# rakhimovv/lvt

Hardware: AMD Instinct MI355X
Metric: video-clips/sec/node (VQVAE+DSFVT train step, BAIR 64x64x16) (higher is better)
Workload: dtype f32

## Files before the change

include/lvt_hip.h:

```cpp
#ifndef LVT_HIP_H
#define LVT_HIP_H
#include <stddef.h>
#include <stdint.h>
#ifdef __cplusplus
extern "C" {
#endif

#define LVT_OK            0
#define LVT_EINVAL      (-1)
#define LVT_EWORKSPACE  (-2)
#define LVT_ELAUNCH     (-3)
#define LVT_ENODEVICE   (-4)

const char *lvt_last_error(void);
int lvt_version(void);
int lvt_device_info(char *name, int name_len, int *cus, int *clock_khz, long long *hbm_bytes);

#define LVT_MATH_F32   (1 << 16)
#define LVT_MATH_F16X2 (1 << 18)
typedef struct { const float *a; const float *b; float *c; } lvt_amax_io;
int lvt_amax(const float *x, long long n, float *out, void *stream);
typedef struct { const float *x; long long n; float *out; } lvt_amax_entry;
int lvt_amax_multi(const lvt_amax_entry *entries, int n, void *stream);
int lvt_amax_merge(const float *a, const float *b, float *out, void *stream);
#define LVT_VQ_COARSE  (1 << 17)
#define LVT_VQ_GENERIC (1 << 22)

#define LVT_EPI_BIAS        1
#define LVT_EPI_RESIDUAL    2
#define LVT_EPI_RELU        4
#define LVT_EPI_TANH        8
#define LVT_EPI_MASK       16
#define LVT_EPI_ACCUM      32
#define LVT_EPI_PLANES     64
#define LVT_CAUSAL_KMAX   (1 << 8)
#define LVT_CAUSAL_KMIN   (1 << 9)
#define LVT_CAUSAL_TILE   (1 << 10)

typedef struct {
    int M, N, K;
    int ta, tb;
    const float *A; long long lda; int a_kb; long long a_skb;
    const float *B; long long ldb; int b_kb; long long b_skb;
    float *C;       long long ldc;
    int batch_outer, batch_inner;
    long long sA_o, sA_i, sB_o, sB_i, sC_o, sC_i;
    float alpha;
    int flags;
    const float *bias;
    const float *res;  long long ldr;
    const float *mask; long long ldm;
    int splits;
    float *a_colsum;
    long long c_plane;
    const float *a_amax, *b_amax;
    const float *a_amax2, *b_amax2;
    float *c_amax;
} lvt_gemm_desc;
size_t lvt_gemm_workspace_bytes(const lvt_gemm_desc *d);
int lvt_gemm_f32(const lvt_gemm_desc *d, void *workspace, size_t workspace_bytes, void *stream);

int lvt_vq_argmax_scores(const float *scores, long long rows, int K, long long ld, const float *codebook, int D,
                         long long *idx, void *stream);

typedef struct {
    int M, N, K;
    const void *A; long long lda; int a_planes; int a_kb; long long a_skb;
    const void *B; long long ldb;
    float *C; long long ldc;
    int batch_outer, batch_inner;
    long long sA_o, sA_i, sB_o, sB_i, sC_o, sC_i;
    float alpha;
    int flags;
    const float *bias;
    const float *res;  long long ldr;
    const float *mask; long long ldm;
    const float *a_amax, *b_amax;
    float *c_amax;
    void *Cp; long long ldcp; const float *cp_amax;
} lvt_gemm_p2_desc;
int lvt_gemm_p2_f32(const lvt_gemm_p2_desc *d, void *stream);
typedef struct { const float *src; void *dst; int rows, cols; long long ld_src, ld_dst; int transpose; const float *amax;
                 int batch; long long bs_src, bs_dst; } lvt_p2_pack_entry;
int lvt_p2_pack_multi(const lvt_p2_pack_entry *entries, int n, void *stream);

int lvt_gemm_smallm_f32(int M, int N, int K, int tb, const float *A, long long lda, const float *B,
                        long long ldb, float *C, long long ldc, int batch, long long sB, long long sC,
                        float alpha, int flags, const float *bias, const float *res, long long ldr,
                        const int *pos, long long c_pos, long long r_pos, void *stream);
size_t lvt_gemm_smallm_splitk_workspace_bytes(int M, int N, int splits);
int lvt_gemm_smallm_splitk_f32(int M, int N, int K, int splits, const float *A, long long lda, const float *B,
                               long long ldb, float *C, long long ldc, float alpha, int flags, const float *bias,
                               const float *res, long long ldr, const int *pos, long long c_pos, long long r_pos,
                               void *workspace, size_t workspace_bytes, void *stream);
int lvt_gemm_smallm_partial_f32(int M, int N, int K, int splits, const float *A, long long lda, const float *B,
                                long long ldb, void *workspace, size_t workspace_bytes, void *stream);
int lvt_splitsum_layernorm_fwd(const float *partials, int splits, int rows, int d, const float *bias, const float *res,
                               long long ldr, float *x_out, float eps, const float *w, const float *b, float *y,
                               void *stream);

typedef struct {
    int N, Ti, Hi, Wi, Ci;
    int To, Ho, Wo, Co;
    int Kt, Kh, Kw;
    int st, sh, sw;
    int pt, ph, pw;
} lvt_conv_geom;
int lvt_conv3d_pack_weight(const lvt_conv_geom *g, const float *w, int Ci_real, int Co_real,
                           float *wp, void *stream);
typedef struct { const float *w; float *dst; int kind, taps, Ci, Co, Ci_real, Co_real; } lvt_pack_entry;
int lvt_conv3d_pack_weights_multi(const lvt_pack_entry *entries, int n, void *stream);
#define LVT_CONV_WEIGHT_IMAGE (1 << 21)
typedef struct { const float *wp; int rows, cols; const float *amax; } lvt_weight_image_entry;
size_t lvt_conv3d_weight_image_bytes(int rows, int cols);
int lvt_conv3d_weight_images(const lvt_weight_image_entry *entries, int n, void *stream);
int lvt_conv3d_pack_weight_t(const lvt_conv_geom *g, const float *w, int Ci_real, int Co_real,
                             float *wt, void *stream);
// ... 21 lines not shown
#define LVT_WGRAD_DB_OF_X (1 << 20)
int lvt_conv3d_bwd_weight(const lvt_conv_geom *g, const float *x, const float *dy, float *dw, float *db,
                          int Ci_real, int Co_real, int flags, const lvt_amax_io *ax, void *workspace,
                          size_t workspace_bytes, void *stream);
int lvt_convt4_fwd(const float *x, const float *w, const float *bias, int N, int Hi, int Wi, int Ci, int Cr,
                   int act_tanh, float *y, int flags, const lvt_amax_io *ax, void *stream);
size_t lvt_colsum_workspace_bytes(long long M, int N);
int lvt_colsum(const float *g, long long M, int N, long long ld, float *out, void *workspace,
               size_t workspace_bytes, void *stream);

size_t lvt_vq_nearest_workspace_bytes(long long rows, int num, int KC);
size_t lvt_vq_nearest_generic_workspace_bytes(int num, int D, int KC);
int lvt_vq_nearest(const float *z, long long rows, int ldz, int num, int D, int KC,
                   const float *codebooks, long long *idx, int P, int flags, void *workspace, size_t workspace_bytes,
                   void *stream);
int lvt_vq_gather(const long long *idx, const float *codebooks, long long rows, int num, int D, int KC,
                  int P, float *out, int ldo, void *stream);
size_t lvt_vq_ema_workspace_bytes(long long rows, int num, int D, int KC);
int lvt_vq_ema_accumulate(const long long *idx, const float *z, long long rows, int ldz, int num, int D,
                          int KC, int P, float *stats, void *workspace, size_t workspace_bytes,
                          void *stream);
int lvt_vq_ema_finalize(const float *stats, int num, int D, int KC, float decay, float eps,
                        float *running_size, float *running_sum, float *weight, void *stream);

int lvt_to_channels_last(const float *in, int B, int C, long long R, int ldo, int mode, const float *a,
                         const float *s, float *out, float *out_amax, void *stream);
int lvt_to_channels_first(const float *in, int B, int C, long long R, int ldi, int mode, const float *a,
                          const float *s, float lo, float hi, float *out, void *stream);

size_t lvt_reduce_workspace_bytes(void);
int lvt_mse_fwd(const float *a, const float *b, long long n, double denom, float scale, float *out,
                void *workspace, size_t workspace_bytes, void *stream);
int lvt_mse_bwd(const float *a, const float *b, long long n, double denom, float scale,
                const float *gout_dev, const float *add, int tanh_of_a, float *out, float *out_amax, void *stream);
int lvt_l1_fwd(const float *a, const float *b, long long n, double denom, float scale, float *out,
               void *workspace, size_t workspace_bytes, void *stream);
int lvt_l1_bwd(const float *a, const float *b, long long n, double denom, float scale,
               const float *gout_dev, const float *add, int tanh_of_a, float *out, float *out_amax, void *stream);
int lvt_tanh_bwd(const float *g, const float *y, long long n, float *out, float *out_amax, void *stream);
int lvt_axpy(const float *x, const float *add, long long n, const float *alpha_dev, float alpha,
             float *out, void *stream);
int lvt_add_periodic(float *x, const float *table, long long rows, int P, int d, void *stream);

int lvt_layernorm_fwd(const float *x, long long rows, int d, float eps, const float *w, const float *b,
                      float *y, float *mean, float *rstd, float *y_amax, const float *w_amax, const float *b_amax,
                      void *stream);
int lvt_layernorm_fwd_p2(const float *x, long long rows, int d, float eps, const float *w, const float *b,
                         float *y, void *yp, float *mean, float *rstd, float *y_amax, const float *w_amax,
                         const float *b_amax, void *stream);
size_t lvt_layernorm_bwd_workspace_bytes(int d);
int lvt_layernorm_bwd(const float *dy, const float *x, const float *mean, const float *rstd,
                      const float *w, long long rows, int d, const float *add, float *dx, float *dw,
                      float *db, float *dx_amax, void *workspace, size_t workspace_bytes, void *stream);

int lvt_attn_softmax_fwd(float *scores, int B, int H, int S, float temper, const float *dt,
                         const float *dh, const float *dw, int bt, int bh, int bw, int masked, float fill,
                         void *stream);
int lvt_attn_softmax_bwd(const float *P, float *dP, int B, int H, int S, float temper, int bt, int bh,
                         int bw, float *G, float *ddt, float *ddh, float *ddw, void *stream);

int lvt_attn_fwd(const float *q, const float *k, const float *v, int B, int H, int S, int da, float temper,
                 const float *dt, const float *dh, const float *dw, int bt, int bh, int bw, int masked, float fill,
                 float *P, float *o, void *stream);

int lvt_attn_planes_supported(int S, int da, int bt, int bh, int bw);
int lvt_attn_fwd_planes(const void *qkv_planes, long long plane_stride, long long operand_stride, int B, int H, int S, int da,
                        float temper, const float *dt, const float *dh, const float *dw, int bt, int bh, int bw, int masked,
                        float fill, float *P, float *o, float *o_amax, void *stream);
size_t lvt_attn_bwd_planes_workspace_bytes(int B, int H, int S, int bt, int bh, int bw);
int lvt_attn_bwd_planes(const void *qkv_planes, long long plane_stride, long long operand_stride, const void *do_planes,
                        const float *P, const float *o, int B, int H, int S, int da, float temper, int bt, int bh, int bw,
                        int masked, float *dq, float *dk, float *dv, float *ddt, float *ddh, float *ddw, float *d_amax,
                        void *workspace, size_t workspace_bytes, void *stream);

int lvt_attn_flash_supported(int S, int da, int bt, int bh, int bw);
int lvt_attn_fwd_flash(const float *q, const float *k, const float *v, long long ld, int B, int H, int S, int da,
                       float temper, const float *dt, const float *dh, const float *dw, int bt, int bh, int bw,
                       int masked, float fill, float *o, float *stats, float *o_amax, void *stream);
size_t lvt_attn_bwd_flash_workspace_bytes(int B, int H, int S, int bt, int bh, int bw);
int lvt_attn_bwd_flash(const float *q, const float *k, const float *v, const float *d_o, long long ld, const float *stats,
                       const float *o, int B, int H, int S, int da, float temper, const float *dt, const float *dh, const float *dw,
                       int bt, int bh, int bw, int masked, float fill, float *dq, float *dk, float *dv, float *ddt,
                       float *ddh, float *ddw, float *d_amax, void *workspace, size_t workspace_bytes, void *stream);

int lvt_attn_decode(const float *q, long long ldq, const float *Kc, const float *Vc, int B, int H, int S, int da, int qi,
                    float temper, const float *dt, const float *dh, const float *dw, int bt, int bh, int bw,
                    float *o, const int *pos, long long q_pos, void *stream);

int lvt_decode_gather_codes(const long long *codes, const long long *nb, const int *pos, int rows, int S1, int taps,
                            long long *out, void *stream);
int lvt_decode_commit(const long long *drawn, int rows, int S1, long long *codes, int *pos, void *stream);

int lvt_sample_categorical(const float *logits, long long rows, int V, float temp, const float *u,
                           long long *out, long long out_stride, float *probs, const int *pos, long long u_pos,
                           void *stream);

int lvt_embbag_fwd(const long long *idx, long long bstride, int P, long long rows, int nslots,
                   const int *slot_off, const int *tab_row, const float *table, int D, const float *bias,
                   const float *btable, const long long *bindex, float *out, void *stream);
#define LVT_ONEHOT_DENSE (1 << 19)
size_t lvt_onehot_tn_workspace_bytes(int nslots, int V, int N, long long rows);
int lvt_onehot_tn_is_gather(int nslots, int V, int N, long long ldb, const float *dout, int flags);
int lvt_onehot_tn_gemm(const long long *idx, int nslots, int V, const int *slot_off, long long bstride,
                       long long pstride, int P, long long rows, const float *dout, long long ldb, int N,
                       float *out, int flags, const float *dout_amax, void *workspace, size_t workspace_bytes,
                       void *stream);
int lvt_permute3(const float *in, long long s0, long long s1, long long s2, int n0, int n1, int n2,
                 float *out, void *stream);

int lvt_row_gather(const float *x, const long long *perm, long long B, int S, int d, float *out, void *stream);

int lvt_slice_context(const long long *video, int B, int T, int nc, int H, int W, const int *abc, int st, int sh,
                      int sw, int kt, int kh, int kw, int n_prime, long long pad_value, long long *ctx,
                      long long *slice, long long *slice_idx, unsigned char *ignore, void *stream);

size_t lvt_xent_workspace_bytes(void);
int lvt_xent_fwd(const float *logits, const long long *target, long long tstride_b, long long tstride_pos,
                 int P, long long rows, int V, long long ignore, float scale, float *row_loss, float *lse,
                 float *loss, float *count, void *workspace, size_t workspace_bytes, void *stream);
int lvt_xent_bwd(const float *logits, const long long *target, long long tstride_b, long long tstride_pos,
                 int P, long long rows, int V, long long ignore, const float *lse, const float *count,
                 const float *gout, float scale, float *dlogits, float *dl_amax, void *stream);

typedef struct {
    float *p; const float *g; float *s0; float *s1;
    long long n; float lr; float wd;
} lvt_opt_entry;
int lvt_adam_step(const lvt_opt_entry *entries, int n, float beta1, float beta2, float eps, int step,
                  void *stream);
int lvt_rmsprop_step(const lvt_opt_entry *entries, int n, float alpha, float eps, float momentum,
                     void *stream);

#ifdef __cplusplus
}
#endif
#endif
```

lvt_amd/csrc/attention_flash.hip:

```cpp
#include "attn_common.h"

namespace {

template <int I> struct IC { static constexpr int value = I; };
template <int N, int I = 0, class F> __device__ __forceinline__ void static_for(F &&f) {
    if constexpr (I < N) { f(IC<I>{}); static_for<N, I + 1>(f); }
}

typedef _Float16 f16x8 __attribute__((ext_vector_type(8)));
typedef _Float16 f16x2v __attribute__((ext_vector_type(2)));
typedef float f32x2 __attribute__((ext_vector_type(2)));
typedef float f32x4v __attribute__((ext_vector_type(4)));
typedef short s16x4 __attribute__((ext_vector_type(4)));
typedef __attribute__((address_space(3))) s16x4 lds_s16x4;
typedef unsigned u32x4 __attribute__((ext_vector_type(4)));

#define FA_LD 144
#define FA_PL (64 * FA_LD)
#define FA_SLOT (2 * FA_PL)
#define FA_EMIN 30
#define FA_EMAX 254
#define FA_LOG2E 1.4426950408889634f

typedef unsigned u32x2 __attribute__((ext_vector_type(2)));

__device__ __forceinline__ float fa_u2f(unsigned u) { return __uint_as_float(u); }
__device__ __forceinline__ float fa_exp_field(int e) { return e <= 0 ? 0.f : fa_u2f((unsigned)e << 23); }
__device__ __forceinline__ int fa_clamp_e(int e) { return e < FA_EMIN ? FA_EMIN : (e > FA_EMAX ? FA_EMAX : e); }
__device__ __forceinline__ int fa_ebits(float nonneg) { return fa_clamp_e((int)((__float_as_uint(nonneg) >> 23) & 0xffu)); }
template <int CTRL> __device__ __forceinline__ float fa_dpp_max(float v) {
    const int o = __builtin_amdgcn_update_dpp(0, __builtin_bit_cast(int, v), CTRL, 0xf, 0xf, false);
    return fmaxf(v, __builtin_bit_cast(float, o));
}
__device__ __forceinline__ float fa_row16_max(float v) {
    v = fa_dpp_max<0xB1>(v);
    v = fa_dpp_max<0x4E>(v);
    v = fa_dpp_max<0x141>(v);
    v = fa_dpp_max<0x140>(v);
    return v;
}
__device__ __forceinline__ float fa_kg_max(float v) {
    u32x2 r = __builtin_amdgcn_permlane16_swap(__float_as_uint(v), __float_as_uint(v), false, false);
    v = fmaxf(fa_u2f(r[0]), fa_u2f(r[1]));
    r = __builtin_amdgcn_permlane32_swap(__float_as_uint(v), __float_as_uint(v), false, false);
    return fmaxf(fa_u2f(r[0]), fa_u2f(r[1]));
}
__device__ __forceinline__ float fa_kg_sum(float v) {
    u32x2 r = __builtin_amdgcn_permlane16_swap(__float_as_uint(v), __float_as_uint(v), false, false);
    v = fa_u2f(r[0]) + fa_u2f(r[1]);
    r = __builtin_amdgcn_permlane32_swap(__float_as_uint(v), __float_as_uint(v), false, false);
    return fa_u2f(r[0]) + fa_u2f(r[1]);
}
__device__ __forceinline__ float fa_max4(const f32x4v a) { return fmaxf(fmaxf(a[0], a[1]), fmaxf(a[2], a[3])); }
__device__ __forceinline__ float fa_absmax4(const float4 a) { return fmaxf(fmaxf(fabsf(a.x), fabsf(a.y)), fmaxf(fabsf(a.z), fabsf(a.w))); }

__device__ __forceinline__ float fa_mix_lo(unsigned h, float c) {
    float r;
    asm("v_fma_mix_f32 %0, %1, %2, %3 op_sel:[0,0,0] op_sel_hi:[1,0,0]" : "=v"(r) : "v"(h), "v"(-1.f), "v"(c));
    return r;
}
__device__ __forceinline__ float fa_mix_hi(unsigned h, float c) {
    float r;
    asm("v_fma_mix_f32 %0, %1, %2, %3 op_sel:[1,0,0] op_sel_hi:[1,0,0]" : "=v"(r) : "v"(h), "v"(-1.f), "v"(c));
    return r;
}
__device__ __forceinline__ void fa_split_pair(float a, float b, float s, unsigned &ph, unsigned &pl) {
    const f32x2 t = f32x2{a, b} * s;
    ph = __builtin_bit_cast(unsigned, __builtin_convertvector(t, f16x2v));
    const f32x2 r = {fa_mix_lo(ph, t.x), fa_mix_hi(ph, t.y)};
    pl = __builtin_bit_cast(unsigned, __builtin_convertvector(r, f16x2v));
}
__device__ __forceinline__ void fa_split_pair1(float a, float b, unsigned &ph, unsigned &pl) {
    const f32x2 t = {a, b};
    ph = __builtin_bit_cast(unsigned, __builtin_convertvector(t, f16x2v));
    const f32x2 r = {fa_mix_lo(ph, a), fa_mix_hi(ph, b)};
    pl = __builtin_bit_cast(unsigned, __builtin_convertvector(r, f16x2v));
}
__device__ __forceinline__ void fa_split8(const float (&v)[8], f16x8 &h, f16x8 &l) {
    u32x4 uh, ul;
    unsigned a, b;
    fa_split_pair1(v[0], v[1], a, b); uh[0] = a; ul[0] = b;
    fa_split_pair1(v[2], v[3], a, b); uh[1] = a; ul[1] = b;
// ... 8 lines not shown
}

__device__ __forceinline__ int fa_row_scale(const float4 a, const float4 b) {
    return fa_ebits(fa_row16_max(fmaxf(fa_absmax4(a), fa_absmax4(b))));
}
__device__ __forceinline__ void fa_row_store(const float4 a, const float4 b, int eb, unsigned short *slot, float *rs_inv, int row, int c) {
    const float s = fa_u2f((unsigned)(268 - eb) << 23);
    uint2 h0, l0, h1, l1;
    fa_split_pair(a.x, a.y, s, h0.x, l0.x); fa_split_pair(a.z, a.w, s, h0.y, l0.y);
    fa_split_pair(b.x, b.y, s, h1.x, l1.x); fa_split_pair(b.z, b.w, s, h1.y, l1.y);
    unsigned short *d = slot + row * FA_LD + 4 * c;
    *reinterpret_cast<uint2 *>(d) = h0;
    *reinterpret_cast<uint2 *>(d + 64) = h1;
    *reinterpret_cast<uint2 *>(d + FA_PL) = l0;
    *reinterpret_cast<uint2 *>(d + FA_PL + 64) = l1;
    rs_inv[c == 0 ? row : 64 + c] = fa_u2f((unsigned)(eb - 14) << 23);
}
struct G4 { float4 v[4]; };
__device__ __forceinline__ void fa_load(G4 &g, const float *__restrict__ x, const float *__restrict__ y, long long ld, int tid) {
    const int r = tid >> 4, c = tid & 15;
    const float *px = x + (long long)r * ld + 4 * c, *py = y + (long long)r * ld + 4 * c;
    g.v[0] = *reinterpret_cast<const float4 *>(px);
    g.v[1] = *reinterpret_cast<const float4 *>(px + 64);
    g.v[2] = *reinterpret_cast<const float4 *>(py);
    g.v[3] = *reinterpret_cast<const float4 *>(py + 64);
}
__device__ __forceinline__ void fa_park(const G4 &g, unsigned short *slot, float *rs_inv, int tid) {
    const int r = tid >> 4, c = tid & 15;
#pragma unroll
    for (int half = 0; half < 2; ++half)
        fa_row_store(g.v[2 * half], g.v[2 * half + 1], fa_row_scale(g.v[2 * half], g.v[2 * half + 1]), slot, rs_inv, 32 * half + r, c);
}
struct G8 { float4 v[8]; };
__device__ __forceinline__ void fa_load8(G8 &g, const float *__restrict__ x, const float *__restrict__ y, long long ld, int tid) {
    const int r = tid >> 4, c = tid & 15;
    const float *px = x + (long long)r * ld + 4 * c, *py = y + (long long)r * ld + 4 * c;
    g.v[0] = *reinterpret_cast<const float4 *>(px);
    g.v[1] = *reinterpret_cast<const float4 *>(px + 64);
    g.v[2] = *reinterpret_cast<const float4 *>(px + 16 * ld);
    g.v[3] = *reinterpret_cast<const float4 *>(px + 16 * ld + 64);
    g.v[4] = *reinterpret_cast<const float4 *>(py);
    g.v[5] = *reinterpret_cast<const float4 *>(py + 64);
    g.v[6] = *reinterpret_cast<const float4 *>(py + 16 * ld);
    g.v[7] = *reinterpret_cast<const float4 *>(py + 16 * ld + 64);
}
__device__ __forceinline__ void fa_park8(const G8 &g, unsigned short *slot, float *rs_inv, int tid) {
    const int r = tid >> 4, c = tid & 15;
#pragma unroll
    for (int p = 0; p < 4; ++p)
        fa_row_store(g.v[2 * p], g.v[2 * p + 1], fa_row_scale(g.v[2 * p], g.v[2 * p + 1]), slot, rs_inv, 16 * p + r, c);
}
__device__ __forceinline__ void fa_bfrags_request(const float *__restrict__ row, int kg, float4 (&v)[8]) {
#pragma unroll
    for (int s = 0; s < 4; ++s) {
        v[2 * s] = *reinterpret_cast<const float4 *>(row + 32 * s + 8 * kg);
        v[2 * s + 1] = *reinterpret_cast<const float4 *>(row + 32 * s + 8 * kg + 4);
    }
}
__device__ __forceinline__ void fa_bfrags_split(const float4 (&v)[8], f16x8 (&fr)[4][2], float &inv) {
    float m = 0.f;
#pragma unroll
    for (int e = 0; e < 8; ++e) m = fmaxf(m, fa_absmax4(v[e]));
    m = fa_kg_max(m);
    const int eb = fa_ebits(m);
    const float sc = fa_u2f((unsigned)(268 - eb) << 23);
    inv = fa_u2f((unsigned)(eb - 14) << 23);
#pragma unroll
    for (int s = 0; s < 4; ++s) {
        u32x4 uh, ul;
        unsigned a, b;
        fa_split_pair(v[2 * s].x, v[2 * s].y, sc, a, b); uh[0] = a; ul[0] = b;
        fa_split_pair(v[2 * s].z, v[2 * s].w, sc, a, b); uh[1] = a; ul[1] = b;
        fa_split_pair(v[2 * s + 1].x, v[2 * s + 1].y, sc, a, b); uh[2] = a; ul[2] = b;
        fa_split_pair(v[2 * s + 1].z, v[2 * s + 1].w, sc, a, b); uh[3] = a; ul[3] = b;
        fr[s][0] = __builtin_bit_cast(f16x8, uh);
        fr[s][1] = __builtin_bit_cast(f16x8, ul);
    }
}
__device__ __forceinline__ void fa_load_bfrags(const float *__restrict__ row, int kg, f16x8 (&fr)[4][2], float &inv) {
    float4 v[8];
    fa_bfrags_request(row, kg, v);
    fa_bfrags_split(v, fr, inv);
}
__device__ __forceinline__ f16x8 fa_rowfrag(const unsigned short *slot, int pl, int row, int s, int kg) {
    return *reinterpret_cast<const f16x8 *>(slot + pl * FA_PL + row * FA_LD + 32 * s + 8 * kg);
}
__device__ __forceinline__ f16x8 fa_trfrag(const unsigned short *slot, int pl, int rb, int dtile, int c16, int kg) {
    const unsigned short *p = slot + pl * FA_PL + (rb + 4 * kg + (c16 >> 2)) * FA_LD + 16 * dtile + 4 * (c16 & 3);
    const s16x4 lo = __builtin_amdgcn_ds_read_tr16_b64_v4i16((lds_s16x4 *)(p));
    const s16x4 hi = __builtin_amdgcn_ds_read_tr16_b64_v4i16((lds_s16x4 *)(p + 16 * FA_LD));
    union { struct { s16x4 a, b; } s; f16x8 v; } u;
    u.s.a = lo; u.s.b = hi;
    return u.v;
}

struct FaSmem {
    unsigned short ring[2][FA_SLOT];
    float rs_inv[2][80];
    float dhs[32];
};
template <int NR> struct FaSmemA {
    unsigned short ring[2][FA_SLOT];
    float rs_inv[2][80];
    float dhs[32];
    float red[16];
    float R[128 * 4 * NR];
};
struct FaSmem3 {
    unsigned short ring[3][FA_SLOT];
    float rs_inv[3][80];
    float dhs[32];
};

__device__ __forceinline__ int fa_pair(unsigned x) { return (int)(((x >> 4) << 3) | (x & 7)); }
__device__ __forceinline__ int fa_half(unsigned x) { return (int)((x >> 3) & 1); }
__device__ __forceinline__ int fa_pair4(unsigned x) { return (int)(((x >> 5) << 3) | (x & 7)); }
__device__ __forceinline__ int fa_quarter(unsigned x) { return (int)((x >> 3) & 3); }
__device__ __forceinline__ int fa_opaque(int x) { asm volatile("" : "+s"(x)); return x; }

template <int BH, int BW> struct Geo16 {
    static_assert(BW == 16 || BW == 8, "16-wide tiles: BW is 8 or 16");
    static constexpr int HP = BW == 16 ? BH : BH / 2;
    static __device__ __forceinline__ int hj(int hslot, int kg) { return BW == 16 ? hslot : 2 * hslot + (kg >> 1); }
    static __device__ __forceinline__ int wj(int r, int kg) { return BW == 16 ? 4 * kg + r : 4 * (kg & 1) + r; }
};
template <int BT, int BH, int BW> struct BankIdx {
    static constexpr int NT = 2 * BT - 1, NH = 2 * BH - 1, NW = 2 * BW - 1, NB = NT + NH + NW;
};

struct FaArgs {
    const float *q, *k, *v, *d_o;
    long long ld;
    int H;
    float c1, fill2;
    float inv_temper;
    const float *dt, *dh, *dw;
    float *o, *m, *l;
    float *dq, *dk, *dv, *delta, *scal, *bank_partial;
};

template <int BT, int BH, int BW, int MASKED, int NCH>
__device__ __forceinline__ float fa_fwd_body(const FaArgs &A, FaSmem &sm, int bh_, int qhalf) {
    using GE = Geo16<BH, BW>;
    constexpr int HP = GE::HP;
    static_assert(BT * BH * BW == AT_S, "256 tokens");
    const int tid = threadIdx.x, lane = tid & 63, wave = tid >> 6;
    const int c16 = lane & 15, kg = lane >> 4;
    const int b = bh_ / A.H, h = bh_ % A.H;
    const long long row0 = (long long)b * AT_S;
    const int il = wave * 16 + c16, i = qhalf * 128 + il;
    const float *kbase = A.k + row0 * A.ld + h * AT_D, *vbase = A.v + row0 * A.ld + h * AT_D;
    constexpr int NIT = NCH;

    if (tid < 2 * BH - 1) sm.dhs[tid] = A.dh[h * (2 * BH - 1) + tid] * FA_LOG2E;
    G4 g0, g1;
#define FA_G(t) ((((t) & 1) == 0) ? g0 : g1)
    auto load_item = [&](int t, G4 &gg) { fa_load(gg, kbase + (long long)(32 * t) * A.ld, vbase + (long long)(32 * t) * A.ld, A.ld, tid); };
    load_item(0, g0);
    if (NIT > 1) load_item(1, g1);
    f16x8 qb[4][2];
    float qinv;
    fa_load_bfrags(A.q + (row0 + i) * A.ld + h * AT_D, kg, qb, qinv);
    const int wi = i % BW, hi = (i / BW) % BH, ti = i / (BW * BH);
    float bt_[BT], bw_[4];
#pragma unroll
    for (int x = 0; x < BT; ++x) bt_[x] = A.dt[h * (2 * BT - 1) + ti - x + BT - 1] * FA_LOG2E;
#pragma unroll
    for (int r = 0; r < 4; ++r) bw_[r] = A.dw[h * (2 * BW - 1) + wi - GE::wj(r, kg) + BW - 1] * FA_LOG2E;
    const float *dhl = sm.dhs + (hi + BH - 1 - (BW == 16 ? 0 : (kg >> 1)));
    constexpr int HSTEP = BW == 16 ? 1 : 2;
    const float qc = qinv * A.c1;
    fa_park(g0, sm.ring[0], sm.rs_inv[0], tid);
    __syncthreads();

    f32x4v oacc[AT_D / 16];
#pragma unroll
    for (int d = 0; d < AT_D / 16; ++d) oacc[d] = f32x4v{0.f, 0.f, 0.f, 0.f};
    float m_run = -3.0e38f, lsum = 0.f;
    float vmax_run = fa_u2f((unsigned)(FA_EMIN - 14) << 23);

    static_for<NIT>([&](auto tc) {
        constexpr int t = decltype(tc)::value;
        const unsigned short *cur = sm.ring[t & 1];
        const float *cinv = sm.rs_inv[t & 1];
        if constexpr (t + 2 < NIT) load_item(t + 2, FA_G(t));
        f32x4v st[2] = {f32x4v{0.f, 0.f, 0.f, 0.f}, f32x4v{0.f, 0.f, 0.f, 0.f}};
#pragma unroll
        for (int s = 0; s < 4; ++s) {
            f16x8 a[2][2];
#pragma unroll
            for (int kt = 0; kt < 2; ++kt)
#pragma unroll
                for (int pl = 0; pl < 2; ++pl) a[kt][pl] = fa_rowfrag(cur, pl, 16 * kt + c16, s, kg);
#pragma unroll
            for (int kt = 0; kt < 2; ++kt) st[kt] = fa_mfma(a[kt][1], qb[s][0], st[kt]);
#pragma unroll
            for (int kt = 0; kt < 2; ++kt) st[kt] = fa_mfma(a[kt][0], qb[s][1], st[kt]);
#pragma unroll
            for (int kt = 0; kt < 2; ++kt) st[kt] = fa_mfma(a[kt][0], qb[s][0], st[kt]);
        }
        if constexpr (t + 1 < NIT) fa_park(FA_G(t + 1), sm.ring[(t + 1) & 1], sm.rs_inv[(t + 1) & 1], tid);
        float x[8];
        f32x4v vinv[2];
#pragma unroll
        for (int kt = 0; kt < 2; ++kt) {
            const int T = 2 * t + kt;
            const f32x4v kinv = *reinterpret_cast<const f32x4v *>(cinv + 16 * kt + 4 * kg);
            vinv[kt] = *reinterpret_cast<const f32x4v *>(cinv + 32 + 16 * kt + 4 * kg);
            const float bth = bt_[T / HP] + dhl[-HSTEP * (T % HP)];
#pragma unroll
            for (int r = 0; r < 4; ++r) {
                float v = fa_score(st[kt][r], kinv[r] * qc, bth + bw_[r]);
                if (MASKED && 16 * T + 4 * kg + r > i) v = A.fill2;
                x[4 * kt + r] = v;
            }
        }
        float cmax = fmaxf(fmaxf(fmaxf(x[0], x[1]), fmaxf(x[2], x[3])), fmaxf(fmaxf(x[4], x[5]), fmaxf(x[6], x[7])));
        cmax = fa_kg_max(cmax);
        const float vmax_c = fa_kg_max(fmaxf(fa_max4(vinv[0]), fa_max4(vinv[1])));
        const float m_new = fmaxf(m_run, cmax);
        const float alpha = __builtin_amdgcn_exp2f(m_run - m_new);
        m_run = m_new;
        const float vmax_new = fmaxf(vmax_run, vmax_c);
        const float fo = alpha * (vmax_run * __builtin_amdgcn_rcpf(vmax_new));
        vmax_run = vmax_new;
        const float srun = 32768.f * __builtin_amdgcn_rcpf(vmax_new);
        float psum = 0.f, pw[8];
#pragma unroll
        for (int kt = 0; kt < 2; ++kt)
#pragma unroll
            for (int r = 0; r < 4; ++r) {
                const float p = __builtin_amdgcn_exp2f(x[4 * kt + r] - m_new);
                psum += p;
                pw[4 * kt + r] = p * (vinv[kt][r] * srun);
            }
        lsum = lsum * alpha + psum;
        f16x8 pbh, pbl;
        fa_split8(pw, pbh, pbl);
#pragma unroll
        for (int d = 0; d < AT_D / 16; ++d) oacc[d] *= fo;
#pragma unroll
        for (int dp = 0; dp < AT_D / 32; ++dp) {
            f16x8 a[2][2];
#pragma unroll
            for (int dd = 0; dd < 2; ++dd)
#pragma unroll
                for (int pl = 0; pl < 2; ++pl) a[dd][pl] = fa_trfrag(cur, pl, 32, 2 * dp + dd, c16, kg);
#pragma unroll
            for (int dd = 0; dd < 2; ++dd) oacc[2 * dp + dd] = fa_mfma(a[dd][1], pbh, oacc[2 * dp + dd]);
#pragma unroll
            for (int dd = 0; dd < 2; ++dd) oacc[2 * dp + dd] = fa_mfma(a[dd][0], pbl, oacc[2 * dp + dd]);
#pragma unroll
            for (int dd = 0; dd < 2; ++dd) oacc[2 * dp + dd] = fa_mfma(a[dd][0], pbh, oacc[2 * dp + dd]);
        }
        __syncthreads();
    });
#undef FA_G
    const float linv = 1.f / fa_kg_sum(lsum);
    const float osc = (vmax_run * (1.f / 32768.f)) * linv;
    float am = 0.f;
    {
        float *orow = A.o + (row0 + i) * A.ld + h * AT_D + 4 * kg;
#pragma unroll
        for (int d = 0; d < AT_D / 16; ++d) {
            const f32x4v ov = oacc[d] * osc;
            *reinterpret_cast<f32x4v *>(orow + 16 * d) = ov;
            am = fmaxf(am, fmaxf(fmaxf(fabsf(ov[0]), fabsf(ov[1])), fmaxf(fabsf(ov[2]), fabsf(ov[3]))));
        }
    }
    if (kg == 0) {
        const long long si = ((long long)b * A.H + h) * AT_S + i;
        A.m[si] = m_run;
        A.l[si] = linv;
    }
    return am;
}

template <int BT, int BH, int BW, int MASKED>
__global__ __launch_bounds__(512, 1) void lvt_attn_fwd_flash_kernel(const FaArgs A, float *__restrict__ o_amax) {
    __shared__ __attribute__((aligned(16))) FaSmem sm;
    if (threadIdx.x >= 256) __builtin_amdgcn_s_setprio(1);
    float am;
    if (MASKED) {
        am = fa_fwd_body<BT, BH, BW, MASKED, 8>(A, sm, blockIdx.x, 1);
        __syncthreads();
        am = fmaxf(am, fa_fwd_body<BT, BH, BW, MASKED, 4>(A, sm, fa_opaque(blockIdx.x), 0));
    } else {
        am = fa_fwd_body<BT, BH, BW, MASKED, 8>(A, sm, fa_pair(blockIdx.x), fa_half(blockIdx.x));
    }
    if (o_amax) {
        __syncthreads();
        lvt_block_amax_commit(am, o_amax, reinterpret_cast<float *>(sm.ring[0]));
    }
}

template <int BT, int BH, int BW, int MASKED, int NCH, int ONEP>
__device__ __forceinline__ float fa_bwd_a_body(const FaArgs &A, FaSmemA<BT + Geo16<BH, BW>::HP + 4> &sm, int bh_, int qhalf) {
    using GE = Geo16<BH, BW>;
    using BI = BankIdx<BT, BH, BW>;
    constexpr int HP = GE::HP;
    constexpr int NR = BT + HP + 4;
    static_assert(BT * BH * BW == AT_S, "256 tokens");
    const int tid = threadIdx.x, lane = tid & 63, wave = tid >> 6;
    const int c16 = lane & 15, kg = lane >> 4;
    const int b = bh_ / A.H, h = bh_ % A.H;
    const long long row0 = (long long)b * AT_S;
    const int il = wave * 16 + c16, i = qhalf * 128 + il;
    const float *kbase = A.k + row0 * A.ld + h * AT_D, *vbase = A.v + row0 * A.ld + h * AT_D;
    constexpr int NIT = ONEP ? NCH : 2 * NCH;

    if (tid < 2 * BH - 1) sm.dhs[tid] = A.dh[h * (2 * BH - 1) + tid] * FA_LOG2E;
    float *mine = sm.R + (il * 4 + kg) * NR;
#pragma unroll
    for (int x = 0; x < NR; ++x) mine[x] = 0.f;
    G4 g0;
    auto load_item = [&](int t, G4 &gg) {
        const int c = t < NCH ? t : t - NCH;
        fa_load(gg, kbase + (long long)(32 * c) * A.ld, vbase + (long long)(32 * c) * A.ld, A.ld, tid);
    };
    load_item(0, g0);
    f16x8 qb[4][2], dob[4][2];
    float qinv, doinv;
    float4 qraw[8], doraw[8], oraw[ONEP ? 8 : 1];
    fa_bfrags_request(A.q + (row0 + i) * A.ld + h * AT_D, kg, qraw);
    fa_bfrags_request(A.d_o + (row0 + i) * A.ld + h * AT_D, kg, doraw);
    if constexpr (ONEP) fa_bfrags_request(A.o + (row0 + i) * A.ld + h * AT_D, kg, oraw);
    fa_bfrags_split(qraw, qb, qinv);
    fa_bfrags_split(doraw, dob, doinv);
    float delta_early = 0.f;
    if constexpr (ONEP) {
        float a0 = 0.f, a1 = 0.f;
#pragma unroll
        for (int s_ = 0; s_ < 4; ++s_) {
            const float4 o0 = oraw[2 * s_], o1 = oraw[2 * s_ + 1], d0 = doraw[2 * s_], d1 = doraw[2 * s_ + 1];
            a0 = fmaf(o0.x, d0.x, a0); a0 = fmaf(o0.y, d0.y, a0); a0 = fmaf(o0.z, d0.z, a0); a0 = fmaf(o0.w, d0.w, a0);
            a1 = fmaf(o1.x, d1.x, a1); a1 = fmaf(o1.y, d1.y, a1); a1 = fmaf(o1.z, d1.z, a1); a1 = fmaf(o1.w, d1.w, a1);
        }
        delta_early = fa_kg_sum(a0 + a1);
    }
    const long long si = ((long long)b * A.H + h) * AT_S + i;
    const float m_i = A.m[si], linv = A.l[si];
    const int wi = i % BW, hi = (i / BW) % BH, ti = i / (BW * BH);
    float bt_[BT];
    f32x4v bw4;
#pragma unroll
    for (int x = 0; x < BT; ++x) bt_[x] = A.dt[h * (2 * BT - 1) + ti - x + BT - 1] * FA_LOG2E;
#pragma unroll
    for (int r = 0; r < 4; ++r) bw4[r] = A.dw[h * (2 * BW - 1) + wi - GE::wj(r, kg) + BW - 1] * FA_LOG2E;
    const float *dhl = sm.dhs + (hi + BH - 1 - (BW == 16 ? 0 : (kg >> 1)));
    constexpr int HSTEP = BW == 16 ? 1 : 2;
    const float qc = qinv * A.c1;
    fa_park(g0, sm.ring[0], sm.rs_inv[0], tid);
    load_item(1, g0);
    __syncthreads();

    float delta = 0.f, gmax = 0.f;
    float kmax = fa_u2f((unsigned)(FA_EMIN - 14) << 23);
    float sgf = 0.f, kmr = 0.f, dl = 0.f;
    int ebG = FA_EMIN;
    if constexpr (ONEP) { delta = delta_early; dl = delta * linv; }
    f32x4v qacc[AT_D / 16];
#pragma unroll
    for (int d = 0; d < AT_D / 16; ++d) qacc[d] = f32x4v{0.f, 0.f, 0.f, 0.f};
    constexpr bool CORR = ONEP;
    f32x4v cacc[CORR ? AT_D / 16 : 1];
#pragma unroll
    for (int d = 0; d < (CORR ? AT_D / 16 : 1); ++d) cacc[d] = f32x4v{0.f, 0.f, 0.f, 0.f};
    int ebC = 16;
    float rst[BT], rsw[4];
#pragma unroll
    for (int x = 0; x < BT; ++x) rst[x] = 0.f;
#pragma unroll
    for (int r = 0; r < 4; ++r) rsw[r] = 0.f;

    static_for<NIT>([&](auto tc) {
        constexpr int t = decltype(tc)::value;
        constexpr int c = t < NCH ? t : t - NCH;
        constexpr bool PASS2 = ONEP || t >= NCH;
        const unsigned short *cur = sm.ring[t & 1];
        const float *cinv = sm.rs_inv[t & 1];
        constexpr bool PARK = t + 1 < NIT;
        unsigned short *nslot = sm.ring[(t + 1) & 1];
        float *ninv = sm.rs_inv[(t + 1) & 1];
        if constexpr (!ONEP && t == NCH) {
            delta = fa_kg_sum(delta) * linv;
            gmax = fa_kg_max(gmax);
            kmax = fa_kg_max(kmax);
            const float G = gmax + fabsf(delta);
            ebG = fa_ebits(G);
            sgf = fa_u2f((unsigned)(268 - ebG) << 23);
            kmr = __builtin_amdgcn_rcpf(kmax);
            dl = delta * linv;
            float r0 = doinv, r1 = G * qinv;
#pragma unroll
            for (int dd = 32; dd > 0; dd >>= 1) { r0 = fmaxf(r0, __shfl_xor(r0, dd, 64)); r1 = fmaxf(r1, __shfl_xor(r1, dd, 64)); }
            if (lane == 0) { sm.red[wave] = r0; sm.red[8 + wave] = r1; }
        }
        f32x4v st[2] = {f32x4v{0.f, 0.f, 0.f, 0.f}, f32x4v{0.f, 0.f, 0.f, 0.f}};
        f32x4v dp[2] = {f32x4v{0.f, 0.f, 0.f, 0.f}, f32x4v{0.f, 0.f, 0.f, 0.f}};
        int eb0 = 0, eb1 = 0;
        static_for<4>([&](auto sc_) {
            constexpr int s = decltype(sc_)::value;
            f16x8 a[2][2], av[2][2];
#pragma unroll
            for (int kt = 0; kt < 2; ++kt)
#pragma unroll
                for (int pl = 0; pl < 2; ++pl) {
                    a[kt][pl] = fa_rowfrag(cur, pl, 16 * kt + c16, s, kg);
                    av[kt][pl] = fa_rowfrag(cur, pl, 32 + 16 * kt + c16, s, kg);
                }
#pragma unroll
            for (int kt = 0; kt < 2; ++kt) { st[kt] = fa_mfma(a[kt][1], qb[s][0], st[kt]); dp[kt] = fa_mfma(av[kt][1], dob[s][0], dp[kt]); }
#pragma unroll
            for (int kt = 0; kt < 2; ++kt) { st[kt] = fa_mfma(a[kt][0], qb[s][1], st[kt]); dp[kt] = fa_mfma(av[kt][0], dob[s][1], dp[kt]); }
#pragma unroll
            for (int kt = 0; kt < 2; ++kt) { st[kt] = fa_mfma(a[kt][0], qb[s][0], st[kt]); dp[kt] = fa_mfma(av[kt][0], dob[s][0], dp[kt]); }
            if constexpr (PARK) {
                if constexpr (s == 0) eb0 = fa_row_scale(g0.v[0], g0.v[1]);
                if constexpr (s == 1) fa_row_store(g0.v[0], g0.v[1], eb0, nslot, ninv, tid >> 4, tid & 15);
                if constexpr (s == 2) eb1 = fa_row_scale(g0.v[2], g0.v[3]);
                if constexpr (s == 3) fa_row_store(g0.v[2], g0.v[3], eb1, nslot, ninv, 32 + (tid >> 4), tid & 15);
                __builtin_amdgcn_sched_group_barrier(0x100, 8, 0);
#pragma unroll
                for (int e = 0; e < 12; ++e) {
                    __builtin_amdgcn_sched_group_barrier(0x008, 1, 0);
                    __builtin_amdgcn_sched_group_barrier(0x002, (s & 1) ? 3 : 2, 0);
                }
                __builtin_amdgcn_sched_barrier(0);
            }
        });
        if constexpr (t + 2 < NIT) load_item(t + 2, g0);
        float w[8];
        u32x4 pku = {0u, 0u, 0u, 0u};
        if constexpr (CORR) {
            const f32x4v k0 = *reinterpret_cast<const f32x4v *>(cinv + 4 * kg), k1 = *reinterpret_cast<const f32x4v *>(cinv + 16 + 4 * kg);
            const int ebN = max(ebC, (int)(__float_as_uint(fa_kg_max(fmaxf(fa_max4(k0), fa_max4(k1)))) >> 23));
            if (__builtin_amdgcn_ballot_w64(ebN != ebC) != 0) {
                const float f = fa_exp_field(127 + ebC - ebN);
#pragma unroll
                for (int d = 0; d < AT_D / 16; ++d) cacc[d] = cacc[d] * f;
                ebC = ebN;
            }
        }
        const float scc = CORR ? fa_u2f((unsigned)(268 - ebC) << 23) * linv : 0.f;
#pragma unroll
        for (int kt = 0; kt < 2; ++kt) {
            const int T = 2 * c + kt;
            const f32x4v kinv = *reinterpret_cast<const f32x4v *>(cinv + 16 * kt + 4 * kg);
            const f32x4v vinv = *reinterpret_cast<const f32x4v *>(cinv + 32 + 16 * kt + 4 * kg);
            const float bth = bt_[T / HP] + dhl[-HSTEP * (T % HP)];
            if constexpr (!PASS2) kmax = fmaxf(kmax, fa_max4(kinv));
            const f32x4v qk = kinv * qc, bm = bw4 + bth;
            const f32x4v dv = vinv * (PASS2 ? doinv * linv : doinv), kw = kinv * kmr;
            float gt = 0.f;
            const f32x4v ks = kinv * scc;
            f32x4v pkv = {0.f, 0.f, 0.f, 0.f};
#pragma unroll
            for (int r = 0; r < 4; ++r) {
                float x = fa_score(st[kt][r], qk[r], bm[r]);
                if (MASKED && 16 * T + 4 * kg + r > i) x = A.fill2;
                const float ex = __builtin_amdgcn_exp2f(x - m_i);
                if constexpr (!PASS2) {
                    const float dpv = dp[kt][r] * dv[r];
                    delta = fmaf(ex, dpv, delta);
                    gmax = fmaxf(gmax, fabsf(dpv));
                } else {
                    const float g = ex * fmaf(dp[kt][r], dv[r], -dl);
                    gt += g;
                    rsw[r] += g;
                    if constexpr (ONEP) { w[4 * kt + r] = g * kinv[r]; gmax = fmaxf(gmax, fabsf(g)); if constexpr (CORR) pkv[r] = ex * ks[r]; }
                    else w[4 * kt + r] = (g * sgf) * kw[r];
                }
            }
            if constexpr (PASS2) { rst[T / HP] += gt; mine[BT + T % HP] += gt; }
            if constexpr (CORR) {
                pku[2 * kt] = __builtin_bit_cast(unsigned, __builtin_convertvector(f32x2{pkv[0], pkv[1]}, f16x2v));
                pku[2 * kt + 1] = __builtin_bit_cast(unsigned, __builtin_convertvector(f32x2{pkv[2], pkv[3]}, f16x2v));
            }
        }
        if constexpr (PASS2) {
            if constexpr (ONEP) {
                float tm = 0.f;
#pragma unroll
                for (int e = 0; e < 8; ++e) tm = fmaxf(tm, fabsf(w[e]));
                const int ebN = max(ebG, fa_ebits(fa_kg_max(tm)));
                if (__builtin_amdgcn_ballot_w64(ebN != ebG) != 0) {
                    const float f = fa_exp_field(127 + ebG - ebN);
#pragma unroll
                    for (int d = 0; d < AT_D / 16; ++d) qacc[d] = qacc[d] * f;
                    ebG = ebN;
                }
                const float sct = fa_u2f((unsigned)(268 - ebG) << 23);
#pragma unroll
                for (int e = 0; e < 8; ++e) w[e] *= sct;
            }
            f16x8 wbh, wbl;
            fa_split8(w, wbh, wbl);
            const f16x8 pcb = __builtin_bit_cast(f16x8, pku);
#pragma unroll
            for (int dq_ = 0; dq_ < AT_D / 32; ++dq_) {
                f16x8 a[2][2];
#pragma unroll
                for (int dd = 0; dd < 2; ++dd)
#pragma unroll
                    for (int pl = 0; pl < 2; ++pl) a[dd][pl] = fa_trfrag(cur, pl, 0, 2 * dq_ + dd, c16, kg);
#pragma unroll
                for (int dd = 0; dd < 2; ++dd) qacc[2 * dq_ + dd] = fa_mfma(a[dd][1], wbh, qacc[2 * dq_ + dd]);
#pragma unroll
                for (int dd = 0; dd < 2; ++dd) qacc[2 * dq_ + dd] = fa_mfma(a[dd][0], wbl, qacc[2 * dq_ + dd]);
// ... 5 lines not shown
                }
            }
        }
        __syncthreads();
    });
    if constexpr (ONEP) {
        float r0 = doinv, r1 = fa_kg_max(gmax) * qinv;
#pragma unroll
        for (int dd = 32; dd > 0; dd >>= 1) { r0 = fmaxf(r0, __shfl_xor(r0, dd, 64)); r1 = fmaxf(r1, __shfl_xor(r1, dd, 64)); }
        if (lane == 0) { sm.red[wave] = r0; sm.red[8 + wave] = r1; }
        __syncthreads();
    }
    const float f1 = ONEP ? 1.f : kmax, f2 = fa_exp_field(ebG - 14) * A.inv_temper;
    float epsc = 0.f;
    if constexpr (CORR) {
        const float eps = fa_kg_sum((rsw[0] + rsw[1]) + (rsw[2] + rsw[3]));
        delta += eps;
        epsc = (eps * fa_exp_field(ebC - 14)) * A.inv_temper;
    }
    float am = 0.f;
    {
        float *qrow = A.dq + (row0 + i) * A.ld + h * AT_D + 4 * kg;
#pragma unroll
        for (int d = 0; d < AT_D / 16; ++d) {
            f32x4v ov = (qacc[d] * f1) * f2;
            if constexpr (CORR) ov = ov - cacc[d] * epsc;
            *reinterpret_cast<f32x4v *>(qrow + 16 * d) = ov;
            am = fmaxf(am, fmaxf(fmaxf(fabsf(ov[0]), fabsf(ov[1])), fmaxf(fabsf(ov[2]), fabsf(ov[3]))));
        }
    }
    if (kg == 0) A.delta[si] = delta;
    if (tid == 0) {
        float r0 = sm.red[0], r1 = sm.red[8];
#pragma unroll
        for (int x = 1; x < 8; ++x) { r0 = fmaxf(r0, sm.red[x]); r1 = fmaxf(r1, sm.red[8 + x]); }
        A.scal[(bh_ * 2 + qhalf) * 2] = r0;
        A.scal[(bh_ * 2 + qhalf) * 2 + 1] = r1;
    }
    float *R = sm.R;
    float *R2 = reinterpret_cast<float *>(sm.ring[0]);
#pragma unroll
    for (int x = 0; x < BT; ++x) mine[x] = rst[x];
#pragma unroll
    for (int r = 0; r < 4; ++r) mine[BT + HP + r] = rsw[r];
    __syncthreads();
    {
        const int e = tid & 63, part = tid >> 6;
        if (e < BI::NB) {
            float acc = 0.f;
            for (int q = 16 * part; q < 16 * part + 16; ++q) {
                const int iq = qhalf * 128 + q;
                const int wq = iq % BW, hq = (iq / BW) % BH, tq = iq / (BW * BH);
                const float *r = R + (q * 4) * NR;
                if (e < BI::NT) {
                    const int tj = tq - e + BT - 1;
                    if (tj >= 0 && tj < BT) acc += (r[tj] + r[NR + tj]) + (r[2 * NR + tj] + r[3 * NR + tj]);
                } else if (e < BI::NT + BI::NH) {
                    const int hj = hq - (e - BI::NT) + BH - 1;
                    if (hj >= 0 && hj < BH) {
                        if (BW == 16) acc += (r[BT + hj] + r[NR + BT + hj]) + (r[2 * NR + BT + hj] + r[3 * NR + BT + hj]);
                        else acc += r[(2 * (hj & 1)) * NR + BT + (hj >> 1)] + r[(2 * (hj & 1) + 1) * NR + BT + (hj >> 1)];
                    }
                } else {
                    const int wj = wq - (e - BI::NT - BI::NH) + BW - 1;
                    if (wj >= 0 && wj < BW) {
                        if (BW == 16) acc += r[(wj >> 2) * NR + BT + HP + (wj & 3)];
                        else acc += r[(wj >> 2) * NR + BT + HP + (wj & 3)] + r[((wj >> 2) + 2) * NR + BT + HP + (wj & 3)];
                    }
                }
            }
            R2[part * BI::NB + e] = acc;
        }
    }
    __syncthreads();
    if (tid < BI::NB) {
        float acc = 0.f;
#pragma unroll
        for (int part = 0; part < 8; ++part) acc += R2[part * BI::NB + tid];
        A.bank_partial[((long long)bh_ * 2 + qhalf) * BI::NB + tid] = acc;
    }
    return am;
}

template <int BT, int BH, int BW, int MASKED, int ONEP>
__global__ __launch_bounds__(512, 1) void lvt_attn_bwd_flash_a_kernel(const FaArgs A, float *__restrict__ d_amax) {
    __shared__ __attribute__((aligned(16))) FaSmemA<BT + Geo16<BH, BW>::HP + 4> sm;
    if (threadIdx.x >= 256) __builtin_amdgcn_s_setprio(1);
    float am;
    if (MASKED) {
        am = fa_bwd_a_body<BT, BH, BW, MASKED, 8, ONEP>(A, sm, blockIdx.x, 1);
        __syncthreads();
        am = fmaxf(am, fa_bwd_a_body<BT, BH, BW, MASKED, 4, ONEP>(A, sm, fa_opaque(blockIdx.x), 0));
    } else {
        am = fa_bwd_a_body<BT, BH, BW, MASKED, 8, ONEP>(A, sm, fa_pair(blockIdx.x), fa_half(blockIdx.x));
    }
    if (d_amax) {
        __syncthreads();
        lvt_block_amax_commit(am, d_amax, reinterpret_cast<float *>(sm.ring[0]));
    }
}

struct FaSmemB {
    unsigned short ring[2][FA_SLOT];
    unsigned short vres[2][FA_SLOT];
    float rs_inv[2][80];
    float vinv[2][80];
    float dhs[32];
};

template <int BT, int BH, int BW, int MASKED, int C0, int NCH>
__device__ __forceinline__ float fa_bwd_b_body(const FaArgs &A, FaSmemB &sm, int bh_, int khalf) {
    using GE = Geo16<BH, BW>;
    constexpr int HP = GE::HP;
    const int tid = threadIdx.x, lane = tid & 63, wave = tid >> 6;
    const int c16 = lane & 15, kg = lane >> 4;
    const int b = bh_ / A.H, h = bh_ % A.H;
    const long long row0 = (long long)b * AT_S;
    const int jl = wave * 16 + c16, j = khalf * 128 + jl;
    const float *qbase = A.q + row0 * A.ld + h * AT_D, *dobase = A.d_o + row0 * A.ld + h * AT_D;
    const long long sb = ((long long)b * A.H + h) * AT_S;
    constexpr int NIT = NCH;

    if (tid < 2 * BH - 1) sm.dhs[tid] = A.dh[h * (2 * BH - 1) + tid] * FA_LOG2E;
    G4 g0;
    auto load_item = [&](int t, G4 &gg) {
        fa_load(gg, qbase + (long long)(32 * (C0 + t)) * A.ld, dobase + (long long)(32 * (C0 + t)) * A.ld, A.ld, tid);
    };
    {
        const float *rows = A.v + (row0 + khalf * 128) * A.ld + h * AT_D;
        G4 a, bq;
        fa_load(a, rows, rows + 32 * A.ld, A.ld, tid);
        fa_load(bq, rows + 64 * A.ld, rows + 96 * A.ld, A.ld, tid);
        fa_park(a, sm.vres[0], sm.vinv[0], tid);
        fa_park(bq, sm.vres[1], sm.vinv[1], tid);
    }
    f16x8 kb[4][2];
    float kinv;
    load_item(0, g0);
    fa_load_bfrags(A.k + (row0 + j) * A.ld + h * AT_D, kg, kb, kinv);
    const float *sc = A.scal + (long long)bh_ * 4;
    const float domax = fmaxf(sc[0], sc[2]), umax = fmaxf(sc[1], sc[3]);
    const float srun = 32768.f * __builtin_amdgcn_rcpf(domax);
    const int zb = fa_ebits(umax);
    const float zrun = fa_u2f((unsigned)(268 - zb) << 23);
    const unsigned short *vs = sm.vres[jl >> 6];
    const int wj = j % BW, hj = (j / BW) % BH, tj = j / (BW * BH);
    float bt_[BT];
    f32x4v bw4;
#pragma unroll
    for (int x = 0; x < BT; ++x) bt_[x] = A.dt[h * (2 * BT - 1) + x - tj + BT - 1] * FA_LOG2E;
#pragma unroll
    for (int r = 0; r < 4; ++r) bw4[r] = A.dw[h * (2 * BW - 1) + GE::wj(r, kg) - wj + BW - 1] * FA_LOG2E;
    const float *dhl = sm.dhs + (BH - 1 - hj + (BW == 16 ? 0 : (kg >> 1)));
    constexpr int HSTEP = BW == 16 ? 1 : 2;
    const float kc = kinv * A.c1;
    fa_park(g0, sm.ring[0], sm.rs_inv[0], tid);
    if (NIT > 1) load_item(1, g0);
    __syncthreads();
    const float vinv = sm.vinv[jl >> 6][jl & 63];

    f32x4v accv[AT_D / 16], acck[AT_D / 16];
#pragma unroll
    for (int d = 0; d < AT_D / 16; ++d) { accv[d] = f32x4v{0.f, 0.f, 0.f, 0.f}; acck[d] = f32x4v{0.f, 0.f, 0.f, 0.f}; }

    static_for<NIT>([&](auto tc) {
        constexpr int t = decltype(tc)::value;
        constexpr int c = C0 + t;
        constexpr bool PARK = t + 1 < NIT;
        const unsigned short *cur = sm.ring[t & 1];
        const float *cinv = sm.rs_inv[t & 1];
        unsigned short *nslot = sm.ring[(t + 1) & 1];
        float *ninv = sm.rs_inv[(t + 1) & 1];
        f32x4v m4[2], l4[2], d4[2];
#pragma unroll
        for (int qt = 0; qt < 2; ++qt) {
            const long long o = sb + 32 * c + 16 * qt + 4 * kg;
            m4[qt] = *reinterpret_cast<const f32x4v *>(A.m + o);
            l4[qt] = *reinterpret_cast<const f32x4v *>(A.l + o);
            d4[qt] = *reinterpret_cast<const f32x4v *>(A.delta + o);
        }
        f32x4v st[2] = {f32x4v{0.f, 0.f, 0.f, 0.f}, f32x4v{0.f, 0.f, 0.f, 0.f}};
        f32x4v dp[2] = {f32x4v{0.f, 0.f, 0.f, 0.f}, f32x4v{0.f, 0.f, 0.f, 0.f}};
        int eb0 = 0, eb1 = 0;
        f16x8 aq[2][2][2], ad[2][2], vb[2];
        auto load_s = [&](int s_, int bf) {
#pragma unroll
            for (int qt = 0; qt < 2; ++qt)
#pragma unroll
                for (int pl = 0; pl < 2; ++pl) aq[bf][qt][pl] = fa_rowfrag(cur, pl, 16 * qt + c16, s_, kg);
        };
        auto load_p = [&](int s_) {
#pragma unroll
            for (int pl = 0; pl < 2; ++pl) vb[pl] = fa_rowfrag(vs, pl, jl & 63, s_, kg);
#pragma unroll
            for (int qt = 0; qt < 2; ++qt)
#pragma unroll
                for (int pl = 0; pl < 2; ++pl) ad[qt][pl] = fa_rowfrag(cur, pl, 32 + 16 * qt + c16, s_, kg);
        };
        load_s(0, 0);
        static_for<4>([&](auto sc_) {
            constexpr int s = decltype(sc_)::value, bf = s & 1;
            load_p(s);
#pragma unroll
            for (int qt = 0; qt < 2; ++qt) st[qt] = fa_mfma(aq[bf][qt][1], kb[s][0], st[qt]);
#pragma unroll
            for (int qt = 0; qt < 2; ++qt) st[qt] = fa_mfma(aq[bf][qt][0], kb[s][1], st[qt]);
#pragma unroll
            for (int qt = 0; qt < 2; ++qt) st[qt] = fa_mfma(aq[bf][qt][0], kb[s][0], st[qt]);
            if constexpr (s < 3) load_s(s + 1, bf ^ 1);
#pragma unroll
            for (int qt = 0; qt < 2; ++qt) dp[qt] = fa_mfma(ad[qt][1], vb[0], dp[qt]);
#pragma unroll
            for (int qt = 0; qt < 2; ++qt) dp[qt] = fa_mfma(ad[qt][0], vb[1], dp[qt]);
#pragma unroll
            for (int qt = 0; qt < 2; ++qt) dp[qt] = fa_mfma(ad[qt][0], vb[0], dp[qt]);
            if constexpr (PARK) {
                if constexpr (s == 0) eb0 = fa_row_scale(g0.v[0], g0.v[1]);
                if constexpr (s == 1) fa_row_store(g0.v[0], g0.v[1], eb0, nslot, ninv, tid >> 4, tid & 15);
                if constexpr (s == 2) eb1 = fa_row_scale(g0.v[2], g0.v[3]);
                if constexpr (s == 3) fa_row_store(g0.v[2], g0.v[3], eb1, nslot, ninv, 32 + (tid >> 4), tid & 15);
            }
            __builtin_amdgcn_sched_group_barrier(0x100, 6, 0);
#pragma unroll
            for (int e = 0; e < 6; ++e) {
                __builtin_amdgcn_sched_group_barrier(0x008, 1, 0);
                if (PARK) __builtin_amdgcn_sched_group_barrier(0x002, (s & 1) ? 3 : 2, 0);
            }
            if constexpr (s < 3) __builtin_amdgcn_sched_group_barrier(0x100, 4, 0);
#pragma unroll
            for (int e = 0; e < 6; ++e) {
                __builtin_amdgcn_sched_group_barrier(0x008, 1, 0);
                if (PARK) __builtin_amdgcn_sched_group_barrier(0x002, (s & 1) ? 3 : 2, 0);
            }
            __builtin_amdgcn_sched_barrier(0);
        });
        if constexpr (t + 2 < NIT) load_item(t + 2, g0);
        float pw[8], u[8];
#pragma unroll
        for (int qt = 0; qt < 2; ++qt) {
            const int T = 2 * c + qt;
            const f32x4v qinv = *reinterpret_cast<const f32x4v *>(cinv + 16 * qt + 4 * kg);
            const f32x4v doinv = *reinterpret_cast<const f32x4v *>(cinv + 32 + 16 * qt + 4 * kg);
            const float bth = bt_[T / HP] + dhl[HSTEP * (T % HP)];
            const f32x4v qk = qinv * kc, bm = bw4 + bth;
            const f32x4v lds = l4[qt] * (doinv * srun);
            const f32x4v qzl = l4[qt] * qinv;
            const f32x4v dvq = (doinv * vinv) * qzl, dq_ = d4[qt] * qzl;
#pragma unroll
            for (int r = 0; r < 4; ++r) {
                float x = fa_score(st[qt][r], qk[r], bm[r]);
                if (MASKED && j > 16 * T + 4 * kg + r) x = A.fill2;
                const float ex = __builtin_amdgcn_exp2f(x - m4[qt][r]);
                pw[4 * qt + r] = ex * lds[r];
                u[4 * qt + r] = (ex * fmaf(dp[qt][r], dvq[r], -dq_[r])) * zrun;
            }
        }
        f16x8 pbh, pbl, ubh, ubl;
        fa_split8(pw, pbh, pbl);
        fa_split8(u, ubh, ubl);
        f16x8 ao[2][2], aqt[2];
        auto load_o = [&](int d_, int bf) {
#pragma unroll
            for (int pl = 0; pl < 2; ++pl) ao[bf][pl] = fa_trfrag(cur, pl, 32, d_, c16, kg);
        };
        load_o(0, 0);
        static_for<AT_D / 16>([&](auto dc) {
            constexpr int d = decltype(dc)::value, bf = d & 1;
#pragma unroll
            for (int pl = 0; pl < 2; ++pl) aqt[pl] = fa_trfrag(cur, pl, 0, d, c16, kg);
            accv[d] = fa_mfma(ao[bf][1], pbh, accv[d]);
            accv[d] = fa_mfma(ao[bf][0], pbl, accv[d]);
            accv[d] = fa_mfma(ao[bf][0], pbh, accv[d]);
            if constexpr (d + 1 < AT_D / 16) load_o(d + 1, bf ^ 1);
            acck[d] = fa_mfma(aqt[1], ubh, acck[d]);
            acck[d] = fa_mfma(aqt[0], ubl, acck[d]);
            acck[d] = fa_mfma(aqt[0], ubh, acck[d]);
            __builtin_amdgcn_sched_group_barrier(0x100, 4, 0);
            __builtin_amdgcn_sched_group_barrier(0x008, 3, 0);
            if constexpr (d + 1 < AT_D / 16) __builtin_amdgcn_sched_group_barrier(0x100, 4, 0);
            __builtin_amdgcn_sched_group_barrier(0x008, 3, 0);
            __builtin_amdgcn_sched_barrier(0);
        });
        __syncthreads();
    });
    const float fvs = domax * (1.f / 32768.f), fks = fa_exp_field(zb - 14) * A.inv_temper;
    float am = 0.f;
    {
        float *vrow = A.dv + (row0 + j) * A.ld + h * AT_D + 4 * kg, *krow = A.dk + (row0 + j) * A.ld + h * AT_D + 4 * kg;
#pragma unroll
        for (int d = 0; d < AT_D / 16; ++d) {
            const f32x4v ov = accv[d] * fvs, ok = acck[d] * fks;
            *reinterpret_cast<f32x4v *>(vrow + 16 * d) = ov;
            *reinterpret_cast<f32x4v *>(krow + 16 * d) = ok;
#pragma unroll
            for (int e = 0; e < 4; ++e) am = fmaxf(am, fmaxf(fabsf(ov[e]), fabsf(ok[e])));
        }
    }
    return am;
}

template <int BT, int BH, int BW, int MASKED>
__global__ __launch_bounds__(512, 1) void lvt_attn_bwd_flash_b_kernel(const FaArgs A, float *__restrict__ d_amax) {
    __shared__ __attribute__((aligned(16))) FaSmemB sm;
    if (threadIdx.x >= 256) __builtin_amdgcn_s_setprio(1);
    float am;
    if (MASKED) {
        if (fa_half(blockIdx.x) == 0) am = fa_bwd_b_body<BT, BH, BW, MASKED, 0, 8>(A, sm, fa_pair(blockIdx.x), 0);
        else am = fa_bwd_b_body<BT, BH, BW, MASKED, 4, 4>(A, sm, fa_pair(blockIdx.x), 1);
    } else {
        am = fa_bwd_b_body<BT, BH, BW, MASKED, 0, 8>(A, sm, fa_pair(blockIdx.x), fa_half(blockIdx.x));
    }
    if (d_amax) {
        __syncthreads();
        lvt_block_amax_commit(am, d_amax, reinterpret_cast<float *>(sm.ring[0]));
    }
}

__global__ __launch_bounds__(256) void lvt_attn_flash_bank_reduce_kernel(const float *__restrict__ partial, int B, int H, int NB, int nt,
                                                                         int nh, float *__restrict__ ddt, float *__restrict__ ddh,
                                                                         float *__restrict__ ddw) {
    const int idx = blockIdx.x * 4 + (threadIdx.x >> 6), lane = threadIdx.x & 63;
    if (idx >= H * NB) return;
    const int h = idx / NB, e = idx % NB;
    float s = 0.f;
    for (int jj = lane; jj < 2 * B; jj += 64) s += partial[(((long long)(jj >> 1) * H + h) * 2 + (jj & 1)) * NB + e];
#pragma unroll
    for (int m = 32; m >= 1; m >>= 1) s += __shfl_xor(s, m, 64);
    if (lane) return;
    const int nw = NB - nt - nh;
    if (e < nt) ddt[h * nt + e] = nt == 1 ? 0.f : s;
    else if (e < nt + nh) ddh[h * nh + e - nt] = nh == 1 ? 0.f : s;
    else ddw[h * nw + e - nt - nh] = nw == 1 ? 0.f : s;
}

}

extern "C" int lvt_attn_flash_supported(int S, int da, int bt, int bh, int bw) {
    return S == AT_S && da == AT_D && ((bt == 1 && bh == 16 && bw == 16) || (bt == 4 && bh == 8 && bw == 8)) ? 1 : 0;
}

#define LVT_FA_GEOMS(X) X(1, 16, 16) X(4, 8, 8)

extern "C" int lvt_attn_fwd_flash(const float *q, const float *k, const float *v, long long ld, int B, int H, int S, int da,
                                  float temper, const float *dt, const float *dh, const float *dw, int bt, int bh, int bw,
                                  int masked, float fill, float *o, float *stats, float *o_amax, void *stream) {
    LVT_REQUIRE(q && k && v && dt && dh && dw && o && stats && B > 0 && H > 0, "attn_fwd_flash: bad args");
    LVT_REQUIRE((B * H) % 8 == 0, "attn_fwd_flash: B * H = %d must be a multiple of 8 (workgroup pairing per XCD)", B * H);
    LVT_REQUIRE(lvt_attn_flash_supported(S, da, bt, bh, bw), "attn_fwd_flash: S=%d da=%d block (%d,%d,%d) has no instantiation", S, da, bt, bh, bw);
    LVT_REQUIRE(lvt_aligned16(q) && lvt_aligned16(k) && lvt_aligned16(v) && lvt_aligned16(o) && lvt_aligned16(stats) && ld % 4 == 0 &&
                ld >= (long long)H * da, "attn_fwd_flash: alignment / row stride");
    FaArgs A = {};
    A.q = q; A.k = k; A.v = v; A.ld = ld; A.H = H; A.inv_temper = 1.f / temper; A.c1 = FA_LOG2E / temper; A.fill2 = fill * FA_LOG2E;
    A.dt = dt; A.dh = dh; A.dw = dw; A.o = o; A.m = stats; A.l = stats + (size_t)B * H * S;
    const dim3 grid((unsigned)(B * H * (masked ? 1 : 2))), blk(512);
    hipStream_t s = (hipStream_t)stream;
#define LVT_X(BT, BH, BW)                                                                                       \
    if (bt == BT && bh == BH && bw == BW) {                                                                     \
        if (masked) hipLaunchKernelGGL((lvt_attn_fwd_flash_kernel<BT, BH, BW, 1>), grid, blk, 0, s, A, o_amax); \
        else hipLaunchKernelGGL((lvt_attn_fwd_flash_kernel<BT, BH, BW, 0>), grid, blk, 0, s, A, o_amax);        \
    }
    LVT_FA_GEOMS(LVT_X)
#undef LVT_X
    LVT_CHECK_LAUNCH("lvt_attn_fwd_flash_kernel");
    return LVT_OK;
}

extern "C" size_t lvt_attn_bwd_flash_workspace_bytes(int B, int H, int S, int bt, int bh, int bw) {
    const size_t nb = (size_t)(2 * bt - 1) + (2 * bh - 1) + (2 * bw - 1);
    return (size_t)B * H * S * sizeof(float) + (size_t)B * H * 4 * sizeof(float) + (size_t)B * H * 2 * nb * sizeof(float);
}

extern "C" int lvt_attn_bwd_flash(const float *q, const float *k, const float *v, const float *d_o, long long ld, const float *stats,
                                  const float *o, int B, int H, int S, int da, float temper, const float *dt, const float *dh, const float *dw,
                                  int bt, int bh, int bw, int masked, float fill, float *dq, float *dk, float *dv, float *ddt,
                                  float *ddh, float *ddw, float *d_amax, void *workspace, size_t workspace_bytes, void *stream) {
    LVT_REQUIRE(q && k && v && d_o && stats && dt && dh && dw && dq && dk && dv && ddt && ddh && ddw && B > 0 && H > 0, "attn_bwd_flash: bad args");
    LVT_REQUIRE((B * H) % 8 == 0, "attn_bwd_flash: B * H = %d must be a multiple of 8 (workgroup pairing per XCD)", B * H);
    LVT_REQUIRE(lvt_attn_flash_supported(S, da, bt, bh, bw), "attn_bwd_flash: S=%d da=%d block (%d,%d,%d) has no instantiation", S, da, bt, bh, bw);
    LVT_REQUIRE(lvt_aligned16(q) && lvt_aligned16(k) && lvt_aligned16(v) && lvt_aligned16(d_o) && lvt_aligned16(stats) && lvt_aligned16(dq) &&
                lvt_aligned16(dk) && lvt_aligned16(dv) && ld % 4 == 0 && ld >= (long long)H * da, "attn_bwd_flash: alignment / row stride");
    if (!workspace || workspace_bytes < lvt_attn_bwd_flash_workspace_bytes(B, H, S, bt, bh, bw) || !lvt_aligned16(workspace)) {
        lvt_set_error("attn_bwd_flash: workspace too small or misaligned");
        return LVT_EWORKSPACE;
    }
    FaArgs A = {};
    A.q = q; A.k = k; A.v = v; A.d_o = d_o; A.ld = ld; A.H = H; A.inv_temper = 1.f / temper; A.c1 = FA_LOG2E / temper; A.fill2 = fill * FA_LOG2E;
    A.dt = dt; A.dh = dh; A.dw = dw; A.m = const_cast<float *>(stats); A.l = const_cast<float *>(stats) + (size_t)B * H * S;
    A.dq = dq; A.dk = dk; A.dv = dv;
    LVT_REQUIRE(!o || lvt_aligned16(o), "attn_bwd_flash: o must be 16-byte aligned");
    const bool onep = o != nullptr;
    A.o = const_cast<float *>(o);
    A.delta = (float *)workspace;
    A.scal = A.delta + (size_t)B * H * S;
    A.bank_partial = A.scal + (size_t)B * H * 4;
    const int nt = 2 * bt - 1, nh = 2 * bh - 1, nw = 2 * bw - 1, nb = nt + nh + nw;
    const dim3 grid((unsigned)(B * H * (masked ? 1 : 2))), blk(512);
    const dim3 gridb((unsigned)(B * H * 2));
    hipStream_t s = (hipStream_t)stream;
#define LVT_X(BT, BH, BW)                                                                                         \
    if (bt == BT && bh == BH && bw == BW) {                                                                       \
        if (masked && onep) hipLaunchKernelGGL((lvt_attn_bwd_flash_a_kernel<BT, BH, BW, 1, 1>), grid, blk, 0, s, A, d_amax); \
        else if (masked) hipLaunchKernelGGL((lvt_attn_bwd_flash_a_kernel<BT, BH, BW, 1, 0>), grid, blk, 0, s, A, d_amax);    \
        else if (onep) hipLaunchKernelGGL((lvt_attn_bwd_flash_a_kernel<BT, BH, BW, 0, 1>), grid, blk, 0, s, A, d_amax);      \
        else hipLaunchKernelGGL((lvt_attn_bwd_flash_a_kernel<BT, BH, BW, 0, 0>), grid, blk, 0, s, A, d_amax);                \
    }
    LVT_FA_GEOMS(LVT_X)
#undef LVT_X
    LVT_CHECK_LAUNCH("lvt_attn_bwd_flash_a_kernel");
#define LVT_X(BT, BH, BW)                                                                                         \
    if (bt == BT && bh == BH && bw == BW) {                                                                       \
        if (masked) hipLaunchKernelGGL((lvt_attn_bwd_flash_b_kernel<BT, BH, BW, 1>), gridb, blk, 0, s, A, d_amax); \
        else hipLaunchKernelGGL((lvt_attn_bwd_flash_b_kernel<BT, BH, BW, 0>), grid, blk, 0, s, A, d_amax);        \
    }
    LVT_FA_GEOMS(LVT_X)
#undef LVT_X
    LVT_CHECK_LAUNCH("lvt_attn_bwd_flash_b_kernel");
    hipLaunchKernelGGL(lvt_attn_flash_bank_reduce_kernel, dim3((unsigned)lvt_cdiv((long long)H * nb, 4)), dim3(256), 0, s,
                       A.bank_partial, B, H, nb, nt, nh, ddt, ddh, ddw);
    LVT_CHECK_LAUNCH("lvt_attn_flash_bank_reduce_kernel");
    return LVT_OK;
}
```

lvt_amd/csrc/epilogue_fast.h:

```cpp
#pragma once
#include "lvt_common.h"

typedef float lvt_f32x16 __attribute__((ext_vector_type(16)));

template <int TM, int TN>
__device__ __forceinline__ void lvt_f16x2_finish(lvt_f32x16 (&acc)[TM][TN], lvt_f32x16 (&acx)[TM][TN], int unscale) {
    if (unscale >= -100 && unscale <= 120) {
        const float s = __uint_as_float((unsigned)(unscale + 127) << 23), sx = __uint_as_float((unsigned)(unscale + 116) << 23);
#pragma unroll
        for (int i = 0; i < TM; ++i)
#pragma unroll
            for (int j = 0; j < TN; ++j) acc[i][j] = acx[i][j] * sx + acc[i][j] * s;
    } else {
#pragma unroll
        for (int i = 0; i < TM; ++i)
#pragma unroll
            for (int j = 0; j < TN; ++j)
#pragma unroll
                for (int r = 0; r < 16; ++r) acc[i][j][r] = ldexpf(fmaf(acx[i][j][r], 1.f / 2048.f, acc[i][j][r]), unscale);
    }
}

struct LvtEpi {
    int M, N;
// ... 25 lines not shown
    for (int i = 0; i < TM; ++i) {
        const int row0 = m_w + i * 32 + r0;
#pragma unroll
        for (int u = 0; u < 8; ++u) orow_all[i][u] = rm(row0 + 4 * u);
    }
    auto request = [&](int i) {
        const int row0 = m_w + i * 32 + r0;
        if (f_res) {
            const float *rp = e.res + e.coff + col;
#pragma unroll
            for (int u = 0; u < 8; ++u)
                rv_all[i][u] = (colok && row0 + 4 * u < e.M) ? *reinterpret_cast<const float4 *>(rp + orow_all[i][u] * e.ldr) : make_float4(0.f, 0.f, 0.f, 0.f);
        }
        if (f_mask) {
            const float *mp = e.mask + e.coff + col;
#pragma unroll
            for (int u = 0; u < 8; ++u)
                mv_all[i][u] = (colok && row0 + 4 * u < e.M) ? *reinterpret_cast<const float4 *>(mp + orow_all[i][u] * e.ldm) : make_float4(0.f, 0.f, 0.f, 0.f);
        }
    };
#pragma unroll
    for (int i = 0; i < TM; ++i) request(i);
#pragma unroll
    for (int i = 0; i < TM; ++i) {
#pragma unroll
        for (int j = 0; j < TN; ++j)
#pragma unroll
            for (int r = 0; r < 16; ++r) wave_tile[((r & 3) + 8 * (r >> 2) + 4 * half) * SW + 32 * j + l31] = acc[i][j][r];
        const int row0 = m_w + i * 32 + r0;
        const long long (&orow)[8] = orow_all[i];
        const float4 (&rv)[8] = rv_all[i];
        const float4 (&mv)[8] = mv_all[i];
        float *cp = e.C + e.coff + col;
#pragma unroll
        for (int u = 0; u < 8; ++u) {
            float4 v = *reinterpret_cast<const float4 *>(&wave_tile[(r0 + 4 * u) * SW + 4 * c4]);
            v.x *= e.alpha; v.y *= e.alpha; v.z *= e.alpha; v.w *= e.alpha;
            if (f_bias) { v.x += bias4.x; v.y += bias4.y; v.z += bias4.z; v.w += bias4.w; }
            if (f_res) { v.x += rv[u].x; v.y += rv[u].y; v.z += rv[u].z; v.w += rv[u].w; }
            if (f_relu) { v.x = fmaxf(v.x, 0.f); v.y = fmaxf(v.y, 0.f); v.z = fmaxf(v.z, 0.f); v.w = fmaxf(v.w, 0.f); }
            if (f_mask) { v.x = mv[u].x > 0.f ? v.x : 0.f; v.y = mv[u].y > 0.f ? v.y : 0.f; v.z = mv[u].z > 0.f ? v.z : 0.f; v.w = mv[u].w > 0.f ? v.w : 0.f; }
            if (colok && row0 + 4 * u < e.M) {
                am = fmaxf(am, fmaxf(fmaxf(lvt_absf(v.x), lvt_absf(v.y)), fmaxf(lvt_absf(v.z), lvt_absf(v.w))));
                *reinterpret_cast<float4 *>(cp + orow[u] * e.ldc) = v;
            }
        }
    }
    return am;
}

template <int TM, int TN, class RM = LvtRowIdentity>
__device__ __forceinline__ float lvt_epi_fast_dispatch(const LvtEpi &e, lvt_f32x16 (&acc)[TM][TN], float *wave_tile, int m_w, int n_w, int lane,
                                                       const RM rm = RM()) {
#define LVT_EPI_CASE(F) case (F): return lvt_epi_fast_wave<(F), TM, TN, RM>(e, acc, wave_tile, m_w, n_w, lane, rm)
    switch (e.flags & (LVT_EPI_BIAS | LVT_EPI_RESIDUAL | LVT_EPI_RELU | LVT_EPI_MASK)) {
    LVT_EPI_CASE(0);
    LVT_EPI_CASE(LVT_EPI_BIAS);
    LVT_EPI_CASE(LVT_EPI_BIAS | LVT_EPI_RELU);
    LVT_EPI_CASE(LVT_EPI_BIAS | LVT_EPI_RESIDUAL);
    LVT_EPI_CASE(LVT_EPI_BIAS | LVT_EPI_RESIDUAL | LVT_EPI_RELU);
    LVT_EPI_CASE(LVT_EPI_RESIDUAL);
    LVT_EPI_CASE(LVT_EPI_MASK);
    LVT_EPI_CASE(LVT_EPI_RESIDUAL | LVT_EPI_MASK);
    default: return lvt_epi_fast_wave<-1, TM, TN, RM>(e, acc, wave_tile, m_w, n_w, lane, rm);
    }
#undef LVT_EPI_CASE
}

__device__ __forceinline__ unsigned lvt_amax_peek(const float *dst) {
    return (dst && threadIdx.x == 0) ? __hip_atomic_load(reinterpret_cast<const unsigned *>(dst), __ATOMIC_RELAXED, __HIP_MEMORY_SCOPE_AGENT) : 0u;
}
__device__ __forceinline__ void lvt_block_amax_commit_seen(float m, float *dst, float *scratch, unsigned seen) {
#pragma unroll
    for (int d = 32; d > 0; d >>= 1) m = fmaxf(m, __shfl_xor(m, d, 64));
    const int nw = (blockDim.x + 63) >> 6;
    if ((threadIdx.x & 63) == 0) scratch[threadIdx.x >> 6] = m;
    __syncthreads();
    if (threadIdx.x == 0) {
        for (int w = 1; w < nw; ++w) m = fmaxf(m, scratch[w]);
        const unsigned bits = __float_as_uint(m);
        if (bits > seen) atomicMax(reinterpret_cast<unsigned *>(dst), bits);
    }
}
```

lvt_amd/csrc/gemm_engine.hip:

```cpp
#include "lvt_common.h"
#include "epilogue_fast.h"
#include <string.h>
#include <stdlib.h>
#include <stdint.h>
#include <type_traits>

typedef float f32x16 __attribute__((ext_vector_type(16)));

#define BK 32
#define NTHREADS 256

enum { A_KPLAIN = 0, A_MPLAIN = 1, A_CONV_K = 2, A_CONVT_K = 3, A_CONV_M = 4, A_ONEHOT_M = 5, A_PATCH = 6, A_PATCHT = 7 };
enum { B_KPLAIN = 0, B_NPLAIN = 1, B_CONVT_W = 2 };

struct KParams {
    int M, N, K;
    const float *A; long long lda; int a_kb; long long a_skb;
    const float *B; long long ldb; int b_kb; long long b_skb;
    float *C; long long ldc; long long c_plane;
    int batch_inner;
    long long sA_o, sA_i, sB_o, sB_i, sC_o, sC_i;
    float alpha; int flags;
    const float *bias; const float *res; long long ldr; const float *mask; long long ldm;
    int splits; int k_per_split; float *partial; long long partial_stride;
// ... 1378 lines not shown
    };

    f32x16 acc[TM][TN], acx[TM][TN];
#pragma unroll
    for (int i = 0; i < TM; ++i)
#pragma unroll
        for (int j = 0; j < TN; ++j)
#pragma unroll
            for (int r = 0; r < 16; ++r) { acc[i][j][r] = 0.f; acx[i][j][r] = 0.f; }

    int fa[TM], fb[TN];
#pragma unroll
    for (int i = 0; i < TM; ++i) fa[i] = hrow<BM>(wm * (TM * 32) + i * 32 + l31) + 8 * half;
#pragma unroll
    for (int j = 0; j < TN; ++j) fb[j] = 2 * PSA + hrow<BN>(wn * (TN * 32) + j * 32 + l31) + 8 * half;

    auto tile = [&](const unsigned short *cur, unsigned short *nxt, auto do_store, auto do_fetch) {
#pragma unroll
        for (int ks = 0; ks < BK; ks += 16) {
            f16x8 a[2][TM], b[2][TN];
#pragma unroll
            for (int q = 0; q < 2; ++q) {
#pragma unroll
                for (int i = 0; i < TM; ++i) a[q][i] = *reinterpret_cast<const f16x8 *>(cur + fa[i] + q * PSA + ks);
#pragma unroll
                for (int j = 0; j < TN; ++j) b[q][j] = *reinterpret_cast<const f16x8 *>(cur + fb[j] + q * PSB + ks);
            }
#pragma unroll
            for (int i = 0; i < TM; ++i)
#pragma unroll
                for (int j = 0; j < TN; ++j)
                    acx[i][j] = __builtin_amdgcn_mfma_f32_32x32x16_f16(a[0][i], b[1][j], acx[i][j], 0, 0, 0);
#pragma unroll
            for (int i = 0; i < TM; ++i)
#pragma unroll
                for (int j = 0; j < TN; ++j)
                    acc[i][j] = __builtin_amdgcn_mfma_f32_32x32x16_f16(a[0][i], b[0][j], acc[i][j], 0, 0, 0);
#pragma unroll
            for (int i = 0; i < TM; ++i)
#pragma unroll
                for (int j = 0; j < TN; ++j)
                    acx[i][j] = __builtin_amdgcn_mfma_f32_32x32x16_f16(a[1][i], b[0][j], acx[i][j], 0, 0, 0);
            if (ks == 0) {
                if constexpr (decltype(do_store)::value) store(nxt);
                if constexpr (decltype(do_fetch)::value) fetch();
            }
        }
    };
    typedef std::integral_constant<bool, true> yes_t;
    typedef std::integral_constant<bool, false> no_t;

    const int ntiles = kbeg < kend ? (kend - kbeg) / BK : 0;
    if (ntiles > 0) {
        fetch();
        store(S0);
        if (ntiles > 1) fetch();
    }
    __syncthreads();
    int kt = 0;
    for (; kt + 2 < ntiles; ++kt) {
        tile(S0 + (kt & 1) * STAGE, S0 + ((kt + 1) & 1) * STAGE, yes_t(), yes_t());
        __syncthreads();
    }
    if (kt + 1 < ntiles) {
        tile(S0 + (kt & 1) * STAGE, S0 + ((kt + 1) & 1) * STAGE, yes_t(), no_t());
        __syncthreads();
        ++kt;
    }
    if (kt < ntiles) tile(S0 + (kt & 1) * STAGE, nullptr, no_t(), no_t());
    __syncthreads();
    lvt_f16x2_finish<TM, TN>(acc, acx, unscale);

    if (TA && sum_on) {
        float *scratch = lds;
        *reinterpret_cast<float4 *>(&scratch[(kk0 * 64 + mq) * 4]) = colacc;
        __syncthreads();
        if (tid < BM) {
            float s_ = 0.f;
            for (int r = 0; r < 8; ++r) s_ += scratch[(r * 64 + tid / 4) * 4 + (tid & 3)];
            if (m0 + tid < p.M) p.colsum_partial[((long long)tc.split * gridDim.y + tc.z) * p.M + m0 + tid] = s_;
        }
        __syncthreads();
    }
    if (p.vec_epi && !(p.flags & (LVT_EPI_PLANES | LVT_EPI_ACCUM | LVT_EPI_TANH))) {
        LvtEpi e;
        e.M = p.M; e.N = p.N;
        float *wave_tile = lds + wave * (32 * TN * 32);
        if (p.splits > 1) {
            e.C = p.partial; e.ldc = p.N; e.coff = tc.split * p.partial_stride + (long long)tc.z * p.M * p.N; e.alpha = 1.f; e.flags = 0;
            e.bias = nullptr; e.res = nullptr; e.ldr = 0; e.mask = nullptr; e.ldm = 0;
            (void)lvt_epi_fast_wave<0, TM, TN>(e, acc, wave_tile, m0 + wm * (TM * 32), n0 + wn * (TN * 32), lane);
            return;
        }
        const unsigned seen = lvt_amax_peek(p.c_amax);
        e.C = p.C; e.ldc = p.ldc; e.coff = tc.coff; e.alpha = p.alpha; e.flags = p.flags;
        e.bias = p.bias; e.res = p.res; e.ldr = p.ldr; e.mask = p.mask; e.ldm = p.ldm;
        const float am_w = lvt_epi_fast_dispatch<TM, TN>(e, acc, wave_tile, m0 + wm * (TM * 32), n0 + wn * (TN * 32), lane);
        if (p.c_amax) lvt_block_amax_commit_seen(am_w, p.c_amax, lds + TURN_FLOATS, seen);
        return;
    }
    if (p.vec_epi) lvt_epilogue_vec<AMODE, BM, BN, WM, WN>(p, acc, lds, m0, n0, wm, wn, lane, 0, tc.coff, tc.z, tc.split);
    else lvt_epilogue<AMODE, BM, BN, WM, WN>(p, acc, m0, n0, wm, wn, l31, half, 0, tc.coff, tc.z, tc.split);
}

__global__ void lvt_reduce_splits_kernel(const float *__restrict__ partial, long long n4, long long stride,
                                         int splits, float *__restrict__ out, int accumulate) {
    long long i = (long long)blockIdx.x * blockDim.x + threadIdx.x;
    const long long step = (long long)gridDim.x * blockDim.x;
    for (; i < n4; i += step) {
        float4 s0 = ldg4(partial + i * 4), s1 = zero4(), s2 = zero4(), s3 = zero4();
        int k = 1;
        for (; k + 3 < splits; k += 4) {
            const float4 t0 = ldg4(partial + k * stride + i * 4), t1 = ldg4(partial + (k + 1) * stride + i * 4);
            const float4 t2 = ldg4(partial + (k + 2) * stride + i * 4), t3 = ldg4(partial + (k + 3) * stride + i * 4);
            s0.x += t0.x; s0.y += t0.y; s0.z += t0.z; s0.w += t0.w;
            s1.x += t1.x; s1.y += t1.y; s1.z += t1.z; s1.w += t1.w;
            s2.x += t2.x; s2.y += t2.y; s2.z += t2.z; s2.w += t2.w;
            s3.x += t3.x; s3.y += t3.y; s3.z += t3.z; s3.w += t3.w;
        }
        for (; k < splits; ++k) {
            const float4 t = ldg4(partial + k * stride + i * 4);
            s0.x += t.x; s0.y += t.y; s0.z += t.z; s0.w += t.w;
        }
        float4 s;
        s.x = (s0.x + s1.x) + (s2.x + s3.x); s.y = (s0.y + s1.y) + (s2.y + s3.y);
        s.z = (s0.z + s1.z) + (s2.z + s3.z); s.w = (s0.w + s1.w) + (s2.w + s3.w);
        float4 *o = reinterpret_cast<float4 *>(out + i * 4);
        if (accumulate) { const float4 c = *o; s.x += c.x; s.y += c.y; s.z += c.z; s.w += c.w; }
        *o = s;
    }
}

__global__ void lvt_pack_weight_kernel(const float *__restrict__ w, float *__restrict__ wp, int taps, int Ci,
                                       int Co, int Ci_real, int Co_real) {
    const long long total = (long long)taps * Ci * Co;
    for (long long i = (long long)blockIdx.x * blockDim.x + threadIdx.x; i < total;
         i += (long long)gridDim.x * blockDim.x) {
        const int co = i % Co; long long t = i / Co;
        const int ci = t % Ci; const int tap = t / Ci;
        float v = 0.f;
        if (co < Co_real && ci < Ci_real) v = w[((long long)co * Ci_real + ci) * taps + tap];
        wp[i] = v;
    }
}
__global__ void lvt_pack_weight_t_kernel(const float *__restrict__ w, float *__restrict__ wt, int taps, int Ci,
                                         int Co, int Ci_real, int Co_real) {
    const long long total = (long long)taps * Co * Ci;
    for (long long i = (long long)blockIdx.x * blockDim.x + threadIdx.x; i < total;
         i += (long long)gridDim.x * blockDim.x) {
        const int ci = i % Ci; long long t = i / Ci;
        const int co = t % Co; const int tr = t / Co;
        float v = 0.f;
        if (co < Co_real && ci < Ci_real) v = w[((long long)co * Ci_real + ci) * taps + (taps - 1 - tr)];
        wt[i] = v;
    }
}
__global__ void lvt_pack_weight_phases_kernel(const float *__restrict__ w, float *__restrict__ wph, int Ci, int Co,
                                              int Ci_real, int Co_real) {
    const long long total = 16LL * Co * Ci;
    for (long long i = (long long)blockIdx.x * blockDim.x + threadIdx.x; i < total; i += (long long)gridDim.x * blockDim.x) {
        const int ci = i % Ci; long long t = i / Ci;
        const int co = t % Co; const int pt = t / Co;
        const int ph = pt >> 2, tap = pt & 3;
        const int ky = 3 - (ph >> 1) - 2 * (tap >> 1), kx = 3 - (ph & 1) - 2 * (tap & 1);
        float v = 0.f;
        if (co < Co_real && ci < Ci_real) v = w[(((long long)co * Ci_real + ci) * 4 + ky) * 4 + kx];
// ... 150 lines not shown

template <int TA, int TB>
static int launch_wide(const KParams &p, int zcount, hipStream_t s) {
    const long long ntm = lvt_cdiv(p.M, 256), ntn = lvt_cdiv(p.N, 128);
    if (ntm * ntn > 0x7fffffffLL || zcount > 65535 || p.splits > 65535) {
        lvt_set_error("gemm: grid too large (%lld tiles, z=%d, splits=%d)", ntm * ntn, zcount, p.splits);
        return LVT_EINVAL;
    }
    dim3 grid((unsigned)(ntm * ntn), (unsigned)zcount, (unsigned)(p.splits > 1 ? p.splits : 1));
    KParams pv = p;
    {
        auto al16 = [](const void *q) { return ((uintptr_t)q & 15) == 0; };
        bool ok = p.N % 4 == 0;
        if (p.splits > 1) ok = ok && al16(p.partial) && p.partial_stride % 4 == 0 && ((long long)p.M * p.N) % 4 == 0;
        else {
            ok = ok && al16(p.C) && p.ldc % 4 == 0 && p.sC_o % 4 == 0 && p.sC_i % 4 == 0;
            if (p.flags & LVT_EPI_BIAS) ok = ok && al16(p.bias);
            if (p.flags & LVT_EPI_RESIDUAL) ok = ok && al16(p.res) && p.ldr % 4 == 0;
            if (p.flags & LVT_EPI_MASK) ok = ok && al16(p.mask) && p.ldm % 4 == 0;
        }
        pv.vec_epi = ok ? 1 : 0;
    }
    if ((p.flags & LVT_EPI_PLANES) && !pv.vec_epi) {
        lvt_set_error("gemm: LVT_EPI_PLANES needs 16-byte aligned bias / res / mask and ldr, ldm %% 4 == 0");
        return LVT_EINVAL;
    }
    hipLaunchKernelGGL((lvt_gemm_wide_kernel<TA, TB>), grid, dim3(WIDE_THREADS), 0, s, pv);
    LVT_CHECK_LAUNCH("lvt_gemm_wide_kernel");
    return LVT_OK;
}

static int choose_splits(long long tiles, int K, int min_k) {
    int s = (int)((2 * LVT_NUM_CU) / (tiles > 0 ? tiles : 1));
    const int maxs = K / min_k > 0 ? K / min_k : 1;
    if (s > maxs) s = maxs;
    if (s < 1) s = 1;
    return s;
}

static void kparams_from_desc(const lvt_gemm_desc *d, KParams &p) {
    memset(&p, 0, sizeof(p));
    p.M = d->M; p.N = d->N; p.K = d->K;
    p.A = d->A; p.lda = d->lda; p.a_kb = d->a_kb > 0 ? d->a_kb : d->K; p.a_skb = d->a_skb;
    p.B = d->B; p.ldb = d->ldb; p.b_kb = d->b_kb > 0 ? d->b_kb : d->K; p.b_skb = d->b_skb;
    p.C = d->C; p.ldc = d->ldc; p.c_plane = d->c_plane;
    p.batch_inner = d->batch_inner > 0 ? d->batch_inner : 1;
    p.sA_o = d->sA_o; p.sA_i = d->sA_i; p.sB_o = d->sB_o; p.sB_i = d->sB_i; p.sC_o = d->sC_o; p.sC_i = d->sC_i;
    p.alpha = d->alpha; p.flags = d->flags; p.bias = d->bias; p.res = d->res; p.ldr = d->ldr;
    p.mask = d->mask; p.ldm = d->ldm;
    p.splits = d->splits > 1 ? d->splits : 1;
    p.a_amax = d->a_amax; p.b_amax = d->b_amax; p.c_amax = d->c_amax;
    p.a_amax2 = d->a_amax2; p.b_amax2 = d->b_amax2;
}

static int gemm_batch(const lvt_gemm_desc *d) {
    return (d->batch_outer > 0 ? d->batch_outer : 1) * (d->batch_inner > 0 ? d->batch_inner : 1);
}

extern "C" size_t lvt_gemm_workspace_bytes(const lvt_gemm_desc *d) {
    if (!d || d->splits <= 1) return 0;
    return (size_t)d->splits * gemm_batch(d) * ((size_t)d->M * d->N + (d->a_colsum ? (size_t)d->M : 0)) * sizeof(float);
}

extern "C" int lvt_gemm_f32(const lvt_gemm_desc *d, void *workspace, size_t workspace_bytes, void *stream) {
    LVT_REQUIRE(d && d->A && d->B && d->C, "gemm: null pointer");
    LVT_REQUIRE(d->M > 0 && d->N > 0 && d->K > 0, "gemm: bad shape %d %d %d", d->M, d->N, d->K);
    LVT_REQUIRE(d->K % 4 == 0, "gemm: K=%d must be a multiple of 4", d->K);
    LVT_REQUIRE(d->lda % 4 == 0 && d->ldb % 4 == 0, "gemm: lda/ldb must be multiples of 4");
    LVT_REQUIRE(lvt_aligned16(d->A) && lvt_aligned16(d->B), "gemm: A/B must be 16-byte aligned");
    LVT_REQUIRE(d->ta == 0 || d->M % 4 == 0, "gemm: ta=1 needs M %% 4 == 0");
    LVT_REQUIRE(d->tb == 0 || d->N % 4 == 0, "gemm: tb=1 needs N %% 4 == 0");
    LVT_REQUIRE(d->a_kb <= 0 || (d->a_kb % 4 == 0 && d->a_skb % 4 == 0), "gemm: a_kb/a_skb %% 4");
    LVT_REQUIRE(d->b_kb <= 0 || (d->b_kb % 4 == 0 && d->b_skb % 4 == 0), "gemm: b_kb/b_skb %% 4");
    LVT_REQUIRE(!(d->ta == 1 && d->tb == 0), "gemm: (ta=1, tb=0) is not instantiated");
    LVT_REQUIRE(!(d->flags & LVT_EPI_BIAS) || d->bias, "gemm: BIAS flag without bias");
    LVT_REQUIRE(!(d->flags & LVT_EPI_RESIDUAL) || d->res, "gemm: RESIDUAL flag without res");
    LVT_REQUIRE(!(d->flags & LVT_EPI_MASK) || d->mask, "gemm: MASK flag without mask");
    LVT_REQUIRE(math_of(d->flags) != 2 || (d->a_amax && d->b_amax), "gemm: LVT_MATH_F16X2 needs a_amax and b_amax");
    LVT_REQUIRE(!d->c_amax || d->splits <= 1, "gemm: c_amax is not produced by split-K launches");
    if (d->flags & LVT_EPI_PLANES)
        LVT_REQUIRE(d->splits <= 1 && !(d->flags & LVT_EPI_ACCUM) && d->N % 4 == 0 && d->ldc % 4 == 0 && d->c_plane % 4 == 0 &&
                    d->sC_o % 4 == 0 && d->sC_i % 4 == 0 && lvt_aligned16(d->C) && !(d->flags & LVT_MATH_F32),
                    "gemm: PLANES needs the bf16x3 arithmetic, no split-K / ACCUM, N, ldc, c_plane, sC %% 4 == 0 and an aligned C");
    hipStream_t s = (hipStream_t)stream;
    KParams p; kparams_from_desc(d, p);
    const int zc = gemm_batch(d);
    if (p.splits > 1) {
        LVT_REQUIRE((d->flags & ~(LVT_EPI_ACCUM | LVT_MATH_F32 | LVT_MATH_F16X2)) == 0 && d->alpha == 1.0f, "gemm: split-K allows only ACCUM");
        LVT_REQUIRE(d->ldc == d->N && (zc == 1 || (d->sC_i == (long long)d->M * d->N)),
                    "gemm: split-K needs a dense C (ldc == N)");
        LVT_REQUIRE(((long long)d->M * d->N) % 4 == 0 && lvt_aligned16(d->C), "gemm: split-K C alignment");
        const size_t need = lvt_gemm_workspace_bytes(d);
        if (workspace_bytes < need || !workspace) {
            lvt_set_error("gemm: workspace %zu < %zu", workspace_bytes, need);
            return LVT_EWORKSPACE;
        }
        p.k_per_split = (int)(lvt_cdiv(lvt_cdiv(p.K, p.splits), BK) * BK);
        p.partial = (float *)workspace;
        p.partial_stride = (long long)zc * d->M * d->N;
        if (d->a_colsum) {
            LVT_REQUIRE(d->ta == 1 && d->M % 4 == 0, "gemm: a_colsum needs ta == 1 and M %% 4 == 0");
            p.colsum_partial = p.partial + (long long)p.splits * p.partial_stride;
        }
    } else {
        LVT_REQUIRE(!d->a_colsum, "gemm: a_colsum needs splits > 1");
    }
    int rc;
    const long long a_span = d->ta ? (long long)d->K * d->lda : (long long)d->M * d->lda + (long long)(d->K / p.a_kb) * d->a_skb;
    const long long b_span = d->tb ? (long long)d->K * d->ldb : (long long)d->N * d->ldb + (long long)(d->K / p.b_kb) * d->b_skb;
    const bool wide = math_of(d->flags) == 2 && d->M > 128 && d->K % BK == 0 && p.a_kb % BK == 0 &&
                      p.b_kb % BK == 0 && a_span < (1LL << 30) && b_span < (1LL << 30) &&
                      !(d->flags & (LVT_CAUSAL_KMAX | LVT_CAUSAL_KMIN | LVT_CAUSAL_TILE));
    if (wide && d->ta == 0 && d->tb == 0) rc = launch_wide<0, 0>(p, zc, s);
    else if (wide && d->ta == 0 && d->tb == 1) rc = launch_wide<0, 1>(p, zc, s);
    else if (wide) rc = launch_wide<1, 1>(p, zc, s);
    else if (d->ta == 0 && d->tb == 0) rc = launch_tile<A_KPLAIN, B_KPLAIN, 128, 128, 2, 2>(p, zc, s);
    else if (d->ta == 0 && d->tb == 1) rc = launch_tile<A_KPLAIN, B_NPLAIN, 128, 128, 2, 2>(p, zc, s);
    else rc = launch_tile<A_MPLAIN, B_NPLAIN, 128, 128, 2, 2>(p, zc, s);
    if (rc != LVT_OK) return rc;
    if (p.splits > 1) {
        const long long n4 = p.partial_stride / 4;
        const int blocks = (int)(lvt_cdiv(n4, 256) < 2048 ? lvt_cdiv(n4, 256) : 2048);
        hipLaunchKernelGGL(lvt_reduce_splits_kernel, dim3(blocks), dim3(256), 0, s, p.partial, n4,
                           p.partial_stride, p.splits, d->C, (d->flags & LVT_EPI_ACCUM) ? 1 : 0);
        LVT_CHECK_LAUNCH("lvt_reduce_splits_kernel");
        if (p.colsum_partial) {
            hipLaunchKernelGGL(lvt_reduce_splits_kernel, dim3((unsigned)lvt_cdiv((long long)zc * d->M / 4, 256)), dim3(256), 0, s,
                               (const float *)p.colsum_partial, (long long)zc * d->M / 4, (long long)zc * d->M, p.splits,
                               d->a_colsum, 0);
            LVT_CHECK_LAUNCH("lvt_reduce_splits_kernel");
        }
    }
    return LVT_OK;
}

struct PackTable { const float *w[64]; float *dst[64]; int kind[64], taps[64], Ci[64], Co[64], Ci_real[64], Co_real[64]; };
__global__ void lvt_pack_weights_multi_kernel(const PackTable t) {
    const int e = blockIdx.y;
    const float *__restrict__ w = t.w[e];
    float *__restrict__ dst = t.dst[e];
    const int kind = t.kind[e], taps = t.taps[e], Ci = t.Ci[e], Co = t.Co[e], Ci_real = t.Ci_real[e], Co_real = t.Co_real[e];
    const long long total = (long long)(kind >= 2 ? 16 : taps) * Ci * Co;
    for (long long i = (long long)blockIdx.x * blockDim.x + threadIdx.x; i < total; i += (long long)gridDim.x * blockDim.x) {
        int co, ci, tap;
        if (kind == 0 || kind == 3) { co = i % Co; const long long q = i / Co; ci = q % Ci; tap = (int)(q / Ci); }
        else { ci = i % Ci; const long long q = i / Ci; co = q % Co; tap = (int)(q / Co); }
        int src_tap = tap;
        if (kind == 1) src_tap = taps - 1 - tap;
        else if (kind == 2) { const int ph = tap >> 2, tp = tap & 3; src_tap = (3 - (ph >> 1) - 2 * (tp >> 1)) * 4 + 3 - (ph & 1) - 2 * (tp & 1); }
        else if (kind == 3) { const int cls = tap >> 2, tp = tap & 3; src_tap = (2 * (tp >> 1) + (cls >> 1)) * 4 + 2 * (tp & 1) + (cls & 1); }
        float v = 0.f;
        if (co < Co_real && ci < Ci_real) v = w[((long long)co * Ci_real + ci) * (kind >= 2 ? 16 : taps) + src_tap];
        dst[i] = v;
    }
}
extern "C" int lvt_conv3d_pack_weights_multi(const lvt_pack_entry *entries, int n, void *stream) {
    LVT_REQUIRE(entries && n > 0, "pack_weights_multi: bad args");
    for (int base = 0; base < n; base += 64) {
        const int cnt = n - base < 64 ? n - base : 64;
        PackTable t;
        long long biggest = 0;
        for (int i = 0; i < cnt; ++i) {
            const lvt_pack_entry &e = entries[base + i];
            LVT_REQUIRE(e.w && e.dst && e.kind >= 0 && e.kind <= 3 && e.taps > 0 && e.Ci > 0 && e.Co > 0 && e.Ci_real <= e.Ci &&
                            e.Co_real <= e.Co && (e.kind < 2 || e.taps == 16), "pack_weights_multi: bad entry %d", base + i);
            t.w[i] = e.w; t.dst[i] = e.dst; t.kind[i] = e.kind; t.taps[i] = e.taps; t.Ci[i] = e.Ci; t.Co[i] = e.Co;
            t.Ci_real[i] = e.Ci_real; t.Co_real[i] = e.Co_real;
            const long long total = (long long)e.taps * e.Ci * e.Co;
            if (total > biggest) biggest = total;
        }
        const unsigned bx = (unsigned)(lvt_cdiv(biggest, 256) < 1024 ? lvt_cdiv(biggest, 256) : 1024);
        hipLaunchKernelGGL(lvt_pack_weights_multi_kernel, dim3(bx, (unsigned)cnt), dim3(256), 0, (hipStream_t)stream, t);
        LVT_CHECK_LAUNCH("lvt_pack_weights_multi_kernel");
    }
    return LVT_OK;
}

struct WImgTable { const float *wp[64]; char *img[64]; const float *amax[64]; int rows[64], cols[64]; };
__global__ __launch_bounds__(256) void lvt_weight_images_kernel(const WImgTable t) {
    const int e = blockIdx.y;
    const float *__restrict__ wp = t.wp[e];
    const int rows = t.rows[e], cols = t.cols[e];
    const int ntn = cols / 128, ntiles = (rows / 32) * ntn;
    int unscale = 0;
    const float sb = lvt_f16_scale(t.amax[e], unscale);
    const int n = threadIdx.x & 127, q0 = threadIdx.x >> 7;
    for (int tile = blockIdx.x; tile < ntiles; tile += gridDim.x) {
        const int kt = tile / ntn, nt = tile - kt * ntn;
        unsigned short *img = reinterpret_cast<unsigned short *>(t.img[e] + (long long)tile * PT_BIMG_BYTES);
        const float *src = wp + (long long)(kt * 32) * cols + nt * 128 + n;
#pragma unroll
        for (int kq = q0; kq < 8; kq += 2) {
            const float4 v = make_float4(src[(long long)(4 * kq) * cols], src[(long long)(4 * kq + 1) * cols],
                                         src[(long long)(4 * kq + 2) * cols], src[(long long)(4 * kq + 3) * cols]);
            store_split2_k<128>(img, n, 4 * kq, v, sb);
// ... 464 lines not shown
```

lvt_amd/csrc/lvt_core.hip:

```cpp
#include "lvt_common.h"
#include <string.h>

static thread_local char g_err[512] = "";

void lvt_set_error(const char *fmt, ...) {
    va_list ap;
    va_start(ap, fmt);
    vsnprintf(g_err, sizeof(g_err), fmt, ap);
    va_end(ap);
}

extern "C" const char *lvt_last_error(void) { return g_err; }
extern "C" int lvt_version(void) { return 620; }

extern "C" int lvt_device_info(char *name, int name_len, int *cus, int *clock_khz, long long *hbm_bytes) {
    int n = 0;
    if (hipGetDeviceCount(&n) != hipSuccess || n == 0) {
        lvt_set_error("no HIP device visible");
        return LVT_ENODEVICE;
    }
    int dev = 0;
    (void)hipGetDevice(&dev);
    hipDeviceProp_t prop;
    if (hipGetDeviceProperties(&prop, dev) != hipSuccess) {
        lvt_set_error("hipGetDeviceProperties failed");
        return LVT_ENODEVICE;
    }
    if (name && name_len > 0) {
        snprintf(name, name_len, "%s (%s)", prop.name, prop.gcnArchName);
    }
    if (cus) *cus = prop.multiProcessorCount;
    if (clock_khz) *clock_khz = prop.clockRate;
    if (hbm_bytes) *hbm_bytes = (long long)prop.totalGlobalMem;
    return LVT_OK;
}
```

lvt_amd/hip/binding.py:

```python
import ctypes as C
import os

import torch

_HERE = os.path.dirname(os.path.abspath(__file__))
_LIB_PATH = os.environ.get("LVT_HIP_LIB") or os.path.join(os.path.dirname(_HERE), "liblvt_hip.so")

EPI_BIAS, EPI_RESIDUAL, EPI_RELU, EPI_TANH, EPI_MASK, EPI_ACCUM, EPI_PLANES = 1, 2, 4, 8, 16, 32, 64
CAUSAL_KMAX, CAUSAL_KMIN, CAUSAL_TILE = 1 << 8, 1 << 9, 1 << 10
ABI_VERSION = 620
MATH_F32 = 1 << 16
MATH_F16X2 = 1 << 18
ONEHOT_DENSE = 1 << 19
WGRAD_DB_OF_X = 1 << 20
CONV_WEIGHT_IMAGE = 1 << 21


class LvtError(RuntimeError):
    pass


class GemmDesc(C.Structure):
    _fields_ = [
        ("M", C.c_int), ("N", C.c_int), ("K", C.c_int), ("ta", C.c_int), ("tb", C.c_int),
        ("A", C.c_void_p), ("lda", C.c_longlong), ("a_kb", C.c_int), ("a_skb", C.c_longlong),
        ("B", C.c_void_p), ("ldb", C.c_longlong), ("b_kb", C.c_int), ("b_skb", C.c_longlong),
        ("C", C.c_void_p), ("ldc", C.c_longlong),
        ("batch_outer", C.c_int), ("batch_inner", C.c_int),
        ("sA_o", C.c_longlong), ("sA_i", C.c_longlong), ("sB_o", C.c_longlong), ("sB_i", C.c_longlong),
        ("sC_o", C.c_longlong), ("sC_i", C.c_longlong),
        ("alpha", C.c_float), ("flags", C.c_int),
        ("bias", C.c_void_p), ("res", C.c_void_p), ("ldr", C.c_longlong),
        ("mask", C.c_void_p), ("ldm", C.c_longlong), ("splits", C.c_int),
        ("a_colsum", C.c_void_p), ("c_plane", C.c_longlong),
        ("a_amax", C.c_void_p), ("b_amax", C.c_void_p), ("a_amax2", C.c_void_p), ("b_amax2", C.c_void_p), ("c_amax", C.c_void_p),
    ]


class GemmP2Desc(C.Structure):
    _fields_ = [
        ("M", C.c_int), ("N", C.c_int), ("K", C.c_int),
        ("A", C.c_void_p), ("lda", C.c_longlong), ("a_planes", C.c_int), ("a_kb", C.c_int), ("a_skb", C.c_longlong),
        ("B", C.c_void_p), ("ldb", C.c_longlong),
        ("C", C.c_void_p), ("ldc", C.c_longlong),
        ("batch_outer", C.c_int), ("batch_inner", C.c_int),
        ("sA_o", C.c_longlong), ("sA_i", C.c_longlong), ("sB_o", C.c_longlong), ("sB_i", C.c_longlong),
        ("sC_o", C.c_longlong), ("sC_i", C.c_longlong),
        ("alpha", C.c_float), ("flags", C.c_int),
        ("bias", C.c_void_p), ("res", C.c_void_p), ("ldr", C.c_longlong),
        ("mask", C.c_void_p), ("ldm", C.c_longlong),
        ("a_amax", C.c_void_p), ("b_amax", C.c_void_p), ("c_amax", C.c_void_p),
        ("Cp", C.c_void_p), ("ldcp", C.c_longlong), ("cp_amax", C.c_void_p),
    ]


class P2PackEntry(C.Structure):
    _fields_ = [("src", C.c_void_p), ("dst", C.c_void_p), ("rows", C.c_int), ("cols", C.c_int), ("ld_src", C.c_longlong),
                ("ld_dst", C.c_longlong), ("transpose", C.c_int), ("amax", C.c_void_p),
                ("batch", C.c_int), ("bs_src", C.c_longlong), ("bs_dst", C.c_longlong)]


class AmaxEntry(C.Structure):
    _fields_ = [("x", C.c_void_p), ("n", C.c_longlong), ("out", C.c_void_p)]


class PackEntry(C.Structure):
    _fields_ = [("w", C.c_void_p), ("dst", C.c_void_p), ("kind", C.c_int), ("taps", C.c_int), ("Ci", C.c_int), ("Co", C.c_int),
                ("Ci_real", C.c_int), ("Co_real", C.c_int)]


class WeightImageEntry(C.Structure):
    _fields_ = [("wp", C.c_void_p), ("rows", C.c_int), ("cols", C.c_int), ("amax", C.c_void_p)]


class AmaxIO(C.Structure):
    _fields_ = [("a", C.c_void_p), ("b", C.c_void_p), ("c", C.c_void_p)]


class OptEntry(C.Structure):
    _fields_ = [("p", C.c_void_p), ("g", C.c_void_p), ("s0", C.c_void_p), ("s1", C.c_void_p),
                ("n", C.c_longlong), ("lr", C.c_float), ("wd", C.c_float)]


class ConvGeom(C.Structure):
    _fields_ = [(n, C.c_int) for n in
                ("N", "Ti", "Hi", "Wi", "Ci", "To", "Ho", "Wo", "Co", "Kt", "Kh", "Kw",
                 "st", "sh", "sw", "pt", "ph", "pw")]

    def key(self):
        return tuple(getattr(self, n) for n, _ in self._fields_)


_lib = None


def _declare(lib):
    vp, ci, cll, cf, sz = C.c_void_p, C.c_int, C.c_longlong, C.c_float, C.c_size_t
    P = C.POINTER
    sigs = {
        "lvt_last_error": (C.c_char_p, []),
        "lvt_version": (ci, []),
        "lvt_device_info": (ci, [C.c_char_p, ci, P(ci), P(ci), P(cll)]),
        "lvt_gemm_workspace_bytes": (sz, [P(GemmDesc)]),
        "lvt_gemm_f32": (ci, [P(GemmDesc), vp, sz, vp]),
        "lvt_vq_argmax_scores": (ci, [vp, cll, ci, cll, vp, ci, vp, vp]),
        "lvt_gemm_p2_f32": (ci, [P(GemmP2Desc), vp]),
        "lvt_p2_pack_multi": (ci, [P(P2PackEntry), ci, vp]),
        "lvt_layernorm_fwd_p2": (ci, [vp, cll, ci, cf, vp, vp, vp, vp, vp, vp, vp, vp, vp, vp]),
        "lvt_gemm_smallm_f32": (ci, [ci, ci, ci, ci, vp, cll, vp, cll, vp, cll, ci, cll, cll, cf, ci, vp, vp, cll, vp, cll, cll, vp]),
        "lvt_gemm_smallm_splitk_workspace_bytes": (sz, [ci, ci, ci]),
        "lvt_gemm_smallm_splitk_f32": (ci, [ci, ci, ci, ci, vp, cll, vp, cll, vp, cll, cf, ci, vp, vp, cll, vp, cll, cll, vp, sz, vp]),
        "lvt_gemm_smallm_partial_f32": (ci, [ci, ci, ci, ci, vp, cll, vp, cll, vp, sz, vp]),
        "lvt_splitsum_layernorm_fwd": (ci, [vp, ci, ci, ci, vp, vp, cll, vp, cf, vp, vp, vp, vp]),
        "lvt_conv3d_pack_weight": (ci, [P(ConvGeom), vp, ci, ci, vp, vp]),
        "lvt_conv3d_pack_weight_t": (ci, [P(ConvGeom), vp, ci, ci, vp, vp]),
        "lvt_conv3d_uses_patch_kernel": (ci, [P(ConvGeom), ci]),
        "lvt_conv3d_fwd_uses_parity_kernel": (ci, [P(ConvGeom), ci]),
        "lvt_conv3d_pack_weight_parity": (ci, [P(ConvGeom), vp, ci, ci, vp, vp]),
        "lvt_amax": (ci, [vp, cll, vp, vp]),
        "lvt_amax_multi": (ci, [P(AmaxEntry), ci, vp]),
        "lvt_conv3d_pack_weights_multi": (ci, [P(PackEntry), ci, vp]),
        "lvt_conv3d_weight_image_bytes": (sz, [ci, ci]),
        "lvt_conv3d_weight_images": (ci, [P(WeightImageEntry), ci, vp]),
        "lvt_amax_merge": (ci, [vp, vp, vp, vp]),
        "lvt_conv3d_fwd_parity": (ci, [P(ConvGeom), vp, vp, vp, vp, vp, vp, ci, P(AmaxIO), vp]),
        "lvt_conv3d_fwd": (ci, [P(ConvGeom), vp, vp, vp, vp, vp, vp, ci, P(AmaxIO), vp]),
        "lvt_conv3d_bwd_data_uses_phase_kernel": (ci, [P(ConvGeom), ci]),
        "lvt_conv3d_pack_weight_phases": (ci, [P(ConvGeom), vp, ci, ci, vp, vp]),
        "lvt_conv3d_bwd_data_phases": (ci, [P(ConvGeom), vp, vp, vp, vp, vp, vp, ci, P(AmaxIO), vp]),
        "lvt_conv3d_bwd_data": (ci, [P(ConvGeom), vp, vp, vp, vp, vp, vp, ci, P(AmaxIO), vp]),
        "lvt_conv3d_bwd_weight_workspace_bytes": (sz, [P(ConvGeom)]),
        "lvt_conv3d_bwd_weight_fuses_bias": (ci, [P(ConvGeom), ci]),
        "lvt_conv3d_bwd_weight": (ci, [P(ConvGeom), vp, vp, vp, vp, ci, ci, ci, P(AmaxIO), vp, sz, vp]),
        "lvt_convt4_fwd": (ci, [vp, vp, vp, ci, ci, ci, ci, ci, ci, vp, ci, vp, vp]),
        "lvt_colsum_workspace_bytes": (sz, [cll, ci]),
        "lvt_colsum": (ci, [vp, cll, ci, cll, vp, vp, sz, vp]),
        "lvt_vq_nearest_workspace_bytes": (sz, [cll, ci, ci]),
        "lvt_vq_nearest_generic_workspace_bytes": (sz, [ci, ci, ci]),
        "lvt_vq_nearest": (ci, [vp, cll, ci, ci, ci, ci, vp, vp, ci, ci, vp, sz, vp]),
        "lvt_vq_gather": (ci, [vp, vp, cll, ci, ci, ci, ci, vp, ci, vp]),
        "lvt_vq_ema_workspace_bytes": (sz, [cll, ci, ci, ci]),
        "lvt_vq_ema_accumulate": (ci, [vp, vp, cll, ci, ci, ci, ci, ci, vp, vp, sz, vp]),
        "lvt_vq_ema_finalize": (ci, [vp, ci, ci, ci, cf, cf, vp, vp, vp, vp]),
        "lvt_to_channels_last": (ci, [vp, ci, ci, cll, ci, ci, vp, vp, vp, vp, vp]),
        "lvt_to_channels_first": (ci, [vp, ci, ci, cll, ci, ci, vp, vp, cf, cf, vp, vp]),
        "lvt_reduce_workspace_bytes": (sz, []),
        "lvt_mse_fwd": (ci, [vp, vp, cll, C.c_double, cf, vp, vp, sz, vp]),
        "lvt_mse_bwd": (ci, [vp, vp, cll, C.c_double, cf, vp, vp, ci, vp, vp, vp]),
        "lvt_l1_fwd": (ci, [vp, vp, cll, C.c_double, cf, vp, vp, sz, vp]),
        "lvt_l1_bwd": (ci, [vp, vp, cll, C.c_double, cf, vp, vp, ci, vp, vp, vp]),
        "lvt_tanh_bwd": (ci, [vp, vp, cll, vp, vp, vp]),
        "lvt_axpy": (ci, [vp, vp, cll, vp, cf, vp, vp]),
        "lvt_add_periodic": (ci, [vp, vp, cll, ci, ci, vp]),
        "lvt_layernorm_fwd": (ci, [vp, cll, ci, cf, vp, vp, vp, vp, vp, vp, vp, vp, vp]),
        "lvt_layernorm_bwd_workspace_bytes": (sz, [ci]),
        "lvt_layernorm_bwd": (ci, [vp, vp, vp, vp, vp, cll, ci, vp, vp, vp, vp, vp, vp, sz, vp]),
        "lvt_attn_softmax_fwd": (ci, [vp, ci, ci, ci, cf, vp, vp, vp, ci, ci, ci, ci, cf, vp]),
        "lvt_attn_softmax_bwd": (ci, [vp, vp, ci, ci, ci, cf, ci, ci, ci, vp, vp, vp, vp, vp]),
        "lvt_attn_fwd": (ci, [vp, vp, vp, ci, ci, ci, ci, cf, vp, vp, vp, ci, ci, ci, ci, cf, vp, vp, vp]),
        "lvt_attn_planes_supported": (ci, [ci, ci, ci, ci, ci]),
        "lvt_attn_fwd_planes": (ci, [vp, cll, cll, ci, ci, ci, ci, cf, vp, vp, vp, ci, ci, ci, ci, cf, vp, vp, vp, vp]),
        "lvt_attn_bwd_planes_workspace_bytes": (sz, [ci, ci, ci, ci, ci, ci]),
        "lvt_attn_bwd_planes": (ci, [vp, cll, cll, vp, vp, vp, ci, ci, ci, ci, cf, ci, ci, ci, ci, vp, vp, vp, vp, vp, vp, vp, vp, sz, vp]),
        "lvt_attn_flash_supported": (ci, [ci, ci, ci, ci, ci]),
        "lvt_attn_fwd_flash": (ci, [vp, vp, vp, cll, ci, ci, ci, ci, cf, vp, vp, vp, ci, ci, ci, ci, cf, vp, vp, vp, vp]),
        "lvt_attn_bwd_flash_workspace_bytes": (sz, [ci, ci, ci, ci, ci, ci]),
        "lvt_attn_bwd_flash": (ci, [vp, vp, vp, vp, cll, vp, vp, ci, ci, ci, ci, cf, vp, vp, vp, ci, ci, ci, ci, cf, vp, vp, vp, vp,
                                    vp, vp, vp, vp, sz, vp]),
        "lvt_attn_decode": (ci, [vp, cll, vp, vp, ci, ci, ci, ci, ci, cf, vp, vp, vp, ci, ci, ci, vp, vp, cll, vp]),
        "lvt_decode_gather_codes": (ci, [vp, vp, vp, ci, ci, ci, vp, vp]),
        "lvt_decode_commit": (ci, [vp, ci, ci, vp, vp, vp]),
        "lvt_sample_categorical": (ci, [vp, cll, ci, cf, vp, vp, cll, vp, vp, cll, vp]),
        "lvt_embbag_fwd": (ci, [vp, cll, ci, cll, ci, P(ci), P(ci), vp, ci, vp, vp, vp, vp, vp]),
        "lvt_onehot_tn_workspace_bytes": (sz, [ci, ci, ci, cll]),
        "lvt_onehot_tn_is_gather": (ci, [ci, ci, ci, cll, vp, ci]),
        "lvt_onehot_tn_gemm": (ci, [vp, ci, ci, P(ci), cll, cll, ci, cll, vp, cll, ci, vp, ci, vp, vp, sz, vp]),
        "lvt_permute3": (ci, [vp, cll, cll, cll, ci, ci, ci, vp, vp]),
        "lvt_row_gather": (ci, [vp, vp, cll, ci, ci, vp, vp]),
        "lvt_slice_context": (ci, [vp, ci, ci, ci, ci, ci, vp, ci, ci, ci, ci, ci, ci, ci, cll, vp, vp, vp, vp, vp]),
        "lvt_xent_workspace_bytes": (sz, []),
        "lvt_xent_fwd": (ci, [vp, vp, cll, cll, ci, cll, ci, cll, cf, vp, vp, vp, vp, vp, sz, vp]),
        "lvt_xent_bwd": (ci, [vp, vp, cll, cll, ci, cll, ci, cll, vp, vp, vp, cf, vp, vp, vp]),
        "lvt_adam_step": (ci, [P(OptEntry), ci, cf, cf, cf, ci, vp]),
        "lvt_rmsprop_step": (ci, [P(OptEntry), ci, cf, cf, cf, vp]),
    }
    for name, (res, args) in sigs.items():
        fn = getattr(lib, name)
        fn.restype = res
        fn.argtypes = args
    return sigs


def available():
    return os.path.exists(_LIB_PATH)


def lib():
    global _lib
    if _lib is None:
        if not os.path.exists(_LIB_PATH):
            raise LvtError("liblvt_hip.so not found at %s -- run `python -c 'import __graft_entry__ as g; "
                           "g.build()'` (or `make -C lvt_amd/csrc`); there is no CPU fallback" % _LIB_PATH)
        handle = C.CDLL(_LIB_PATH)
        handle.lvt_version.restype = C.c_int
        if handle.lvt_version() != ABI_VERSION:
            raise LvtError("liblvt_hip.so at %s has ABI version %d, this package binds version %d -- rebuild it "
                           "(`make -C lvt_amd/csrc`)" % (_LIB_PATH, handle.lvt_version(), ABI_VERSION))
        handle._lvt_sigs = _declare(handle)
        _lib = handle
    return _lib


MATH_MODES = ("f32", "bf16x3", "f16x2")
_math_mode = os.environ.get("LVT_MATH", "f16x2")
if _math_mode not in MATH_MODES:
    raise LvtError("LVT_MATH must be one of %s (got %r)" % (MATH_MODES, _math_mode))


def set_math_mode(mode):
    global _math_mode
    if mode not in MATH_MODES:
        raise LvtError("math mode must be one of %s (got %r)" % (MATH_MODES, mode))
    _math_mode = mode


def get_math_mode():
    return _math_mode


def math_flag():
    return MATH_F32 if _math_mode == "f32" else (MATH_F16X2 if _math_mode == "f16x2" else 0)


def f16x2():
    return _math_mode == "f16x2"


_amax_pool, _amax_pos, _epoch = None, 0, 0


def bump_epoch():
    global _epoch
    _epoch += 1


def amax_slot(device):
    global _amax_pool, _amax_pos
    if _amax_pool is None or _amax_pos >= _amax_pool.numel() or _amax_pool.device != device:
        _amax_pool, _amax_pos = torch.zeros(4096, dtype=torch.float32, device=device), 0
    s = _amax_pool[_amax_pos:_amax_pos + 1]
    _amax_pos += 1
# ... 214 lines not shown
```

lvt_amd/hip/gemm.py:

```python
import ctypes as C
import os

import torch

from . import binding as L


def gemm(A, B, C_out, M, N, K, ta=0, tb=0, lda=None, ldb=None, ldc=None, a_kb=0, a_skb=0, b_kb=0,
         b_skb=0, batch_outer=1, batch_inner=1, sA=(0, 0), sB=(0, 0), sC=(0, 0), alpha=1.0, flags=0,
         bias=None, res=None, ldr=0, mask=None, ldm=0, splits=1, a_colsum=None, c_plane=0, a_also=None, b_also=None):
    L.require(A, B, C_out, bias, res, mask)
    d = L.GemmDesc()
    d.M, d.N, d.K, d.ta, d.tb = M, N, K, ta, tb
    d.A, d.lda, d.a_kb, d.a_skb = A.data_ptr(), (lda if lda is not None else (K if ta == 0 else M)), a_kb, a_skb
    d.B, d.ldb, d.b_kb, d.b_skb = B.data_ptr(), (ldb if ldb is not None else (K if tb == 0 else N)), b_kb, b_skb
    d.C, d.ldc = C_out.data_ptr(), (ldc if ldc is not None else N)
    d.batch_outer, d.batch_inner = batch_outer, batch_inner
    d.sA_o, d.sA_i = sA
    d.sB_o, d.sB_i = sB
    d.sC_o, d.sC_i = sC
    d.alpha, d.flags = alpha, flags | L.math_flag()
    d.bias = bias.data_ptr() if bias is not None else None
    d.res = res.data_ptr() if res is not None else None
    d.ldr = ldr if res is not None and ldr else d.ldc
    d.mask = mask.data_ptr() if mask is not None else None
    d.ldm = ldm if mask is not None and ldm else d.ldc
    d.splits = splits
    d.a_colsum = a_colsum.data_ptr() if a_colsum is not None else None
    d.c_plane = c_plane
    if L.f16x2():
        d.a_amax, d.b_amax = L.amax_of(A).data_ptr(), L.amax_of(B).data_ptr()
        d.a_amax2 = L.amax_of(a_also).data_ptr() if a_also is not None else None
        d.b_amax2 = L.amax_of(b_also).data_ptr() if b_also is not None else None
        if splits <= 1 and C_out.dtype == torch.float32:
            d.c_amax = L.new_amax(C_out).data_ptr()
    lib = L.lib()
    ws, nws = None, 0
    if splits > 1:
        nws = lib.lvt_gemm_workspace_bytes(C.byref(d))
        ws = L.workspace(nws, A.device, "gemm")
    t0 = L.TIMER.begin() if L.TIMER is not None else None
    L.check(lib.lvt_gemm_f32(C.byref(d), L.ptr(ws), nws, L.stream_ptr()), "lvt_gemm_f32")
    if t0 is not None:
        causal = 0.75 if flags & (L.CAUSAL_KMAX | L.CAUSAL_KMIN | L.CAUSAL_TILE) and M == 256 and N % 128 == 0 else 1.0
        L.TIMER.end("gemm_%s%s" % ("nt"[ta], "tn"[tb]), 2.0 * M * N * K * batch_outer * batch_inner * causal, t0)
    return C_out


class P2Image:
    __slots__ = ("data", "amax")

    def __init__(self, data, amax):
        self.data, self.amax = data, amax


def p2_mode(force=None):
    if not L.f16x2():
        return "off"
    if force is not None:
        return "full" if force else "off"
    env = os.environ.get("LVT_P2", "")
    if env == "qkv":
        return "qkv"
    return "full" if env not in ("", "0") else "off"


def p2_supported(force=None):
    return p2_mode(force) == "full"


def p2_pack(specs):
    arr = (L.P2PackEntry * len(specs))()
    for e, sp in zip(arr, specs):
        src, transpose, dst, amax = sp[:4]
        if src.dim() != 2 or dst.dim() != 2 or src.stride(1) != 1 or dst.stride(1) != 1 or not src.is_cuda:
            raise L.LvtError("p2_pack: 2-D device views with unit column stride expected")
        e.src, e.dst, e.rows, e.cols = src.data_ptr(), dst.data_ptr(), src.shape[0], src.shape[1]
        e.ld_src, e.ld_dst, e.transpose, e.amax = src.stride(0), dst.stride(0), int(bool(transpose)), amax.data_ptr()
        e.batch, e.bs_src, e.bs_dst = sp[4:7] if len(sp) > 4 else (1, 0, 0)
    L.check(L.lib().lvt_p2_pack_multi(arr, len(specs), L.stream_ptr()), "lvt_p2_pack_multi")


def gemm_p2(A, Bimg, C_out, M, N, K, lda=None, a_kb=0, a_skb=0, ldb=None, ldc=None, batch_outer=1, batch_inner=1, sA=(0, 0),
            sB=(0, 0), sC=(0, 0), alpha=1.0, flags=0, bias=None, res=None, ldr=0, mask=None, ldm=0, out_image=None, out_bound=None):
    a_img = isinstance(A, P2Image)
    At = A.data if a_img else A
    L.require(C_out, bias, res, mask)
    d = L.GemmP2Desc()
    d.M, d.N, d.K = M, N, K
    d.A, d.lda, d.a_planes, d.a_kb, d.a_skb = At.data_ptr(), (lda if lda is not None else K), int(a_img), a_kb, a_skb
    d.B, d.ldb = Bimg.data.data_ptr(), (ldb if ldb is not None else K)
    d.C, d.ldc = C_out.data_ptr(), (ldc if ldc is not None else N)
    d.batch_outer, d.batch_inner = batch_outer, batch_inner
    d.sA_o, d.sA_i = sA
    d.sB_o, d.sB_i = sB
    d.sC_o, d.sC_i = sC
    d.alpha, d.flags = alpha, flags | L.MATH_F16X2
    d.bias = bias.data_ptr() if bias is not None else None
    d.res = res.data_ptr() if res is not None else None
    d.ldr = ldr if res is not None and ldr else d.ldc
    d.mask = mask.data_ptr() if mask is not None else None
    d.ldm = ldm if mask is not None and ldm else d.ldc
    d.a_amax = (A.amax if a_img else L.amax_of(A)).data_ptr()
    d.b_amax = Bimg.amax.data_ptr()
    d.c_amax = L.new_amax(C_out).data_ptr()
    img = None
    if out_image is not None:
        d.Cp, d.ldcp, d.cp_amax = out_image.data_ptr(), d.ldc, out_bound.data_ptr()
        img = P2Image(out_image, out_bound)
    t0 = L.TIMER.begin() if L.TIMER is not None else None
    L.check(L.lib().lvt_gemm_p2_f32(C.byref(d), L.stream_ptr()), "lvt_gemm_p2_f32")
    if t0 is not None:
        L.TIMER.end("gemm_p2a" if a_img else "gemm_p2", 2.0 * M * N * K * batch_outer * batch_inner, t0)
    return C_out, img


def _smallm_splits(N, K):
# ... 299 lines not shown
```

lvt_amd/hip/tx.py:

```python
import ctypes as C

import torch

from . import binding as L
from . import ew


def _iarr(vals):
    return (C.c_int * len(vals))(*[int(v) for v in vals])


def attn_softmax_fwd_(scores, temper, dt, dh, dw, block, masked, fill=-1e4):
    L.require(scores, dt, dh, dw)
    B, H, S, _ = scores.shape
    L.check(L.lib().lvt_attn_softmax_fwd(L.ptr(scores), B, H, S, temper, L.ptr(dt), L.ptr(dh), L.ptr(dw),
                                         block[0], block[1], block[2], 1 if masked else 0, fill, L.stream_ptr()),
            "lvt_attn_softmax_fwd")
    L.drop_amax(scores)
    return scores


def attn_fwd_supported(S, da):
    return S == 256 and da == 128


def attn_fwd(q, k, v, B, H, S, da, temper, dt, dh, dw, block, masked, fill=-1e4):
    L.require(q, k, v, dt, dh, dw)
    P = torch.empty(B, H, S, S, dtype=torch.float32, device=q.device)
    o = torch.empty(B * S, H * da, dtype=torch.float32, device=q.device)
    t0 = L.TIMER.begin() if L.TIMER is not None else None
    L.check(L.lib().lvt_attn_fwd(L.ptr(q), L.ptr(k), L.ptr(v), B, H, S, da, temper, L.ptr(dt), L.ptr(dh), L.ptr(dw),
                                 block[0], block[1], block[2], 1 if masked else 0, fill, L.ptr(P), L.ptr(o),
                                 L.stream_ptr()), "lvt_attn_fwd")
    if t0 is not None:
        L.TIMER.end("attn_fwd", 4.0 * B * H * S * S * da, t0)
    return P, o


def attn_planes_supported(S, da, block, bh_pairs=8):
    return bh_pairs % 8 == 0 and bool(L.lib().lvt_attn_planes_supported(S, da, block[0], block[1], block[2])) and L.get_math_mode() != "f32"


def attn_fwd_planes(qkvp, B, H, S, da, temper, dt, dh, dw, block, masked, fill=-1e4):
    L.require(qkvp, dt, dh, dw)
    M, hd = B * S, H * da
    P = torch.empty(B, H, S, S, dtype=torch.float32, device=qkvp.device)
    o = torch.empty(M, hd, dtype=torch.float32, device=qkvp.device)
    t0 = L.TIMER.begin() if L.TIMER is not None else None
    L.check(L.lib().lvt_attn_fwd_planes(L.ptr(qkvp), M * hd, 3 * M * hd, B, H, S, da, temper, L.ptr(dt), L.ptr(dh), L.ptr(dw),
                                        block[0], block[1], block[2], 1 if masked else 0, fill, L.ptr(P), L.ptr(o),
                                        L.out_amax(o), L.stream_ptr()), "lvt_attn_fwd_planes")
    if t0 is not None:
        L.TIMER.end("attn_fwd", 4.0 * B * H * S * S * da, t0)
    return P, o


def attn_bwd_planes(qkvp, dop, P, o, B, H, S, da, temper, block, masked):
    L.require(qkvp, dop, P, o)
    M, hd = B * S, H * da
    dev = P.device
    dqkv = torch.empty(3, M, hd, dtype=torch.float32, device=dev)
    ddt = torch.empty(H, 2 * block[0] - 1, dtype=torch.float32, device=dev)
    ddh = torch.empty(H, 2 * block[1] - 1, dtype=torch.float32, device=dev)
    ddw = torch.empty(H, 2 * block[2] - 1, dtype=torch.float32, device=dev)
    lib = L.lib()
    nws = lib.lvt_attn_bwd_planes_workspace_bytes(B, H, S, block[0], block[1], block[2])
    ws = L.workspace(nws, dev, "attn_bwd")
    t0 = L.TIMER.begin() if L.TIMER is not None else None
    L.check(lib.lvt_attn_bwd_planes(L.ptr(qkvp), M * hd, 3 * M * hd, L.ptr(dop), L.ptr(P), L.ptr(o), B, H, S, da, temper,
                                    block[0], block[1], block[2], 1 if masked else 0, L.ptr(dqkv[0]), L.ptr(dqkv[1]),
                                    L.ptr(dqkv[2]), L.ptr(ddt), L.ptr(ddh), L.ptr(ddw), L.out_amax(dqkv), L.ptr(ws), nws,
                                    L.stream_ptr()),
            "lvt_attn_bwd_planes")
    if t0 is not None:
        L.TIMER.end("attn_bwd", 8.0 * B * H * S * S * da, t0)
    return dqkv, ddt, ddh, ddw


def attn_flash_supported(S, da, block, bh_pairs=8):
    return (bh_pairs % 8 == 0 and L.get_math_mode() == "f16x2" and
            bool(L.lib().lvt_attn_flash_supported(S, da, block[0], block[1], block[2])))


def attn_fwd_flash(qkv, B, H, S, da, temper, dt, dh, dw, block, masked, fill=-1e4):
    L.require(qkv, dt, dh, dw)
    M, hd = B * S, H * da
    o = torch.empty(M, hd, dtype=torch.float32, device=qkv.device)
    stats = torch.empty(2, B * H * S, dtype=torch.float32, device=qkv.device)
    t0 = L.TIMER.begin() if L.TIMER is not None else None
    L.check(L.lib().lvt_attn_fwd_flash(L.ptr(qkv[0]), L.ptr(qkv[1]), L.ptr(qkv[2]), hd, B, H, S, da, temper, L.ptr(dt), L.ptr(dh),
                                       L.ptr(dw), block[0], block[1], block[2], 1 if masked else 0, fill, L.ptr(o), L.ptr(stats),
                                       L.out_amax(o), L.stream_ptr()), "lvt_attn_fwd_flash")
    if t0 is not None:
        L.TIMER.end("attn_fwd", 4.0 * B * H * S * S * da, t0)
    return o, stats


def attn_bwd_flash(qkv, do, stats, B, H, S, da, temper, dt, dh, dw, block, masked, fill=-1e4, o=None):
    L.require(qkv, do, stats, dt, dh, dw, o)
    M, hd = B * S, H * da
    dev = qkv.device
    dqkv = torch.empty(3, M, hd, dtype=torch.float32, device=dev)
    ddt = torch.empty(H, 2 * block[0] - 1, dtype=torch.float32, device=dev)
    ddh = torch.empty(H, 2 * block[1] - 1, dtype=torch.float32, device=dev)
    ddw = torch.empty(H, 2 * block[2] - 1, dtype=torch.float32, device=dev)
    lib = L.lib()
    nws = lib.lvt_attn_bwd_flash_workspace_bytes(B, H, S, block[0], block[1], block[2])
    ws = L.workspace(nws, dev, "attn_bwd")
    t0 = L.TIMER.begin() if L.TIMER is not None else None
    L.check(lib.lvt_attn_bwd_flash(L.ptr(qkv[0]), L.ptr(qkv[1]), L.ptr(qkv[2]), L.ptr(do), hd, L.ptr(stats), L.ptr(o), B, H, S, da, temper,
                                   L.ptr(dt), L.ptr(dh), L.ptr(dw), block[0], block[1], block[2], 1 if masked else 0, fill,
                                   L.ptr(dqkv[0]), L.ptr(dqkv[1]), L.ptr(dqkv[2]), L.ptr(ddt), L.ptr(ddh), L.ptr(ddw),
                                   L.out_amax(dqkv), L.ptr(ws), nws, L.stream_ptr()), "lvt_attn_bwd_flash")
    if t0 is not None:
        L.TIMER.end("attn_bwd", 8.0 * B * H * S * S * da, t0)
    return dqkv, ddt, ddh, ddw


def attn_softmax_bwd_(P, dP, temper, block):
    L.require(P, dP)
    B, H, S, _ = P.shape
    G = torch.empty(H, S, S, dtype=torch.float32, device=P.device)
    ddt = torch.empty(H, 2 * block[0] - 1, dtype=torch.float32, device=P.device)
    ddh = torch.empty(H, 2 * block[1] - 1, dtype=torch.float32, device=P.device)
    ddw = torch.empty(H, 2 * block[2] - 1, dtype=torch.float32, device=P.device)
    L.check(L.lib().lvt_attn_softmax_bwd(L.ptr(P), L.ptr(dP), B, H, S, temper, block[0], block[1], block[2], L.ptr(G),
                                         L.ptr(ddt), L.ptr(ddh), L.ptr(ddw), L.stream_ptr()), "lvt_attn_softmax_bwd")
    L.drop_amax(dP)
    return ddt, ddh, ddw


MAX_SLOTS = 32


def _embbag_once(idx, bstride, P, rows, slot_off, tab_row, table, D, bias, btable, bindex):
    out = torch.empty(rows, D, dtype=torch.float32, device=idx.device)
    L.check(L.lib().lvt_embbag_fwd(L.ptr(idx), bstride, P, rows, len(slot_off), _iarr(slot_off), _iarr(tab_row),
                                   L.ptr(table), D, L.ptr(bias), L.ptr(btable), L.ptr(bindex), L.ptr(out),
                                   L.stream_ptr()), "lvt_embbag_fwd")
    return out


def embbag_fwd(idx, bstride, P, rows, slot_off, tab_row, table, D, bias=None, btable=None, bindex=None):
    L.require(idx, table, bias, btable, bindex)
    out = _embbag_once(idx, bstride, P, rows, slot_off[:MAX_SLOTS], tab_row[:MAX_SLOTS], table, D, bias, btable, bindex)
    for s in range(MAX_SLOTS, len(slot_off), MAX_SLOTS):
        part = _embbag_once(idx, bstride, P, rows, slot_off[s:s + MAX_SLOTS], tab_row[s:s + MAX_SLOTS], table, D,
                            None, None, None)
        out = ew.axpy(part, add=out)
    return out


def _onehot_once(idx, V, slot_off, bstride, pstride, P, rows, dout, N, ldb, dense):
    lib = L.lib()
    ns = len(slot_off)
    out = torch.empty(ns * V, N, dtype=torch.float32, device=dout.device)
    nws = lib.lvt_onehot_tn_workspace_bytes(ns, V, N, rows)
    ws = L.workspace(nws, dout.device, "onehot")
    ldb = ldb if ldb is not None else N
    flags = L.math_flag() | (L.ONEHOT_DENSE if dense else 0)
    gather = bool(lib.lvt_onehot_tn_is_gather(ns, V, N, ldb, L.ptr(dout), flags))
    t0 = L.TIMER.begin() if L.TIMER is not None else None
    L.check(lib.lvt_onehot_tn_gemm(L.ptr(idx), ns, V, _iarr(slot_off), bstride, pstride, P, rows, L.ptr(dout), ldb, N,
                                   L.ptr(out), flags, L.ptr(L.amax_of(dout)) if (L.f16x2() and not gather) else None,
                                   L.ptr(ws), nws, L.stream_ptr()),
            "lvt_onehot_tn_gemm")
    if t0 is not None:
        if gather:
            L.TIMER.end("embbag_wgrad_gather", 0.0, t0)
        else:
            L.TIMER.end("gemm_onehot_tn", 2.0 * ns * V * N * rows, t0)
    return out


def onehot_tn_gemm(idx, V, slot_off, bstride, pstride, P, rows, dout, N, ldb=None, dense=False):
    L.require(idx, dout)
    if len(slot_off) <= MAX_SLOTS:
        return _onehot_once(idx, V, slot_off, bstride, pstride, P, rows, dout, N, ldb, dense)
# ... 77 lines not shown
```

lvt_amd/modeling/autoregressive/vt_attention.py:

```python
import math
import os

import numpy as np
import torch
from torch import nn
from torch.nn import init

from ...hip import binding as L
from ...hip import ew, tx
from ...hip import gemm as G


class PositionalEncoding(nn.Module):

    def __init__(self, d_model, num_dims=3, min_timescale=1.0, max_timescale=1.0e4):
        super().__init__()
        assert d_model >= num_dims * 2, "d_model should be >= then 2*num_dims"
        self.d_model, self.num_dims = d_model, num_dims
        self.num_timescales = d_model // (num_dims * 2)
        inc = np.log(max_timescale / min_timescale) / self.num_timescales
        self.register_buffer("inv_timescales",
                             min_timescale * torch.exp(torch.arange(self.num_timescales).float() * -inc))
        self._tables = {}

# ... 92 lines not shown
    for m, iq, i1 in layers:
        m._p2 = (iq, i1)


def linear_wgrad(dy, x, n_out, k_in, rows, want_bias=False):
    dw = torch.empty(n_out, k_in, dtype=torch.float32, device=dy.device)
    tiles = -(-n_out // 128) * -(-k_in // 128)
    splits = _splits(tiles, rows)
    if not want_bias:
        G.gemm(dy, x, dw, n_out, k_in, rows, ta=1, tb=1, lda=dy.shape[-1], ldb=x.shape[-1], splits=splits)
        return dw
    if splits < 2:
        G.gemm(dy, x, dw, n_out, k_in, rows, ta=1, tb=1, lda=dy.shape[-1], ldb=x.shape[-1], splits=splits)
        return dw, G.colsum(dy, rows, n_out)
    db = torch.empty(n_out, dtype=torch.float32, device=dy.device)
    G.gemm(dy, x, dw, n_out, k_in, rows, ta=1, tb=1, lda=dy.shape[-1], ldb=x.shape[-1], splits=splits, a_colsum=db)
    return dw, db


def linear_wgrad_pair(dy0, x0, dy1, x1, n_out, k_in, rows):
    es = dy0.element_size()
    da, dx = dy1.data_ptr() - dy0.data_ptr(), x1.data_ptr() - x0.data_ptr()
    if (da % (4 * es) or dx % (4 * es) or dy0.shape != dy1.shape or x0.shape != x1.shape or not
            (dy0.is_contiguous() and dy1.is_contiguous() and x0.is_contiguous() and x1.is_contiguous())):
        a, ab = linear_wgrad(dy0, x0, n_out, k_in, rows, want_bias=True)
        b, bb = linear_wgrad(dy1, x1, n_out, k_in, rows, want_bias=True)
        return torch.stack([a, b]), torch.stack([ab, bb])
    dw = torch.empty(2, n_out, k_in, dtype=torch.float32, device=dy0.device)
    db = torch.empty(2, n_out, dtype=torch.float32, device=dy0.device)
    tiles = 2 * -(-n_out // 128) * -(-k_in // 128)
    splits = _splits(tiles, rows)
    if splits < 2:
        a, ab = linear_wgrad(dy0, x0, n_out, k_in, rows, want_bias=True)
        b, bb = linear_wgrad(dy1, x1, n_out, k_in, rows, want_bias=True)
        return torch.stack([a, b]), torch.stack([ab, bb])
    G.gemm(dy0, x0, dw, n_out, k_in, rows, ta=1, tb=1, lda=n_out, ldb=k_in, batch_inner=2, sA=(0, da // es), sB=(0, dx // es),
           sC=(0, n_out * k_in), splits=splits, a_colsum=db, a_also=dy1, b_also=x1)
    return dw, db


FUSED_ATTENTION = True
PLANE_ATTENTION = None
FLASH_ATTENTION = None


def _use_flash(S, da, block, pairs):
    if os.environ.get("LVT_NO_FLASH_ATTENTION") or FLASH_ATTENTION is False:
        return False
    return tx.attn_flash_supported(S, da, block, pairs)


def _use_planes(S, da, block, pairs):
    if os.environ.get("LVT_NO_PLANE_ATTENTION") or PLANE_ATTENTION is False:
        return False
    return tx.attn_planes_supported(S, da, block, pairs)


class _BlockLocalAttentionFn(torch.autograd.Function):
    @staticmethod
    def forward(ctx, x, block, masked, dt, dh, dw, ln_w, ln_b, w_q, w_k, w_v, proj_w, f0w, f0b, f1w, f1b, f3w, f3b,
                wqkv, p2=None):
        L.require(x)
        M, d = x.shape
        S = block[0] * block[1] * block[2]
        b = M // S
        na, _, da = w_q.shape
        hd = na * da
        temper = math.sqrt(da)
        dev = x.device
        flash = FUSED_ATTENTION and _use_flash(S, da, block, b * na)
        planes = FUSED_ATTENTION and not flash and _use_planes(S, da, block, b * na)
        p2 = p2 if (p2 is not None and not planes and L.f16x2()) else None
        p2_full = p2 is not None and p2[1] is not None
        if p2_full:
            xn, xn_img, mean1, rstd1 = ew.layernorm_fwd_p2(x, ln_w, ln_b)
        else:
            xn, mean1, rstd1 = ew.layernorm_fwd(x, ln_w, ln_b)
        if planes:
            qkv = torch.empty(3, 3, M, hd, dtype=torch.bfloat16, device=dev)
            G.gemm(xn, wqkv, qkv, M, da, d, ta=0, tb=1, lda=d, ldb=da, ldc=hd, batch_outer=3, batch_inner=na,
                   sB=(na * d * da, d * da), sC=(3 * M * hd, da), flags=L.EPI_PLANES, c_plane=M * hd)
            P, o = tx.attn_fwd_planes(qkv, b, na, S, da, temper, dt, dh, dw, block, masked)
        else:
            qkv = torch.empty(3, M, hd, dtype=torch.float32, device=dev)
            if p2 is not None:
                G.gemm_p2(G.P2Image(xn_img, L.amax_of(xn)) if p2_full else xn, p2[0], qkv, M, hd, d, lda=d, ldb=d, ldc=hd,
                          batch_outer=3, batch_inner=1, sB=(hd * d, 0), sC=(M * hd, 0))
                if p2_full:
                    del xn_img
            else:
                G.gemm(xn, wqkv, qkv, M, da, d, ta=0, tb=1, lda=d, ldb=da, ldc=hd, batch_outer=3, batch_inner=na,
                       sB=(na * d * da, d * da), sC=(M * hd, da))
            q, k, v = qkv[0], qkv[1], qkv[2]
        if planes:
            pass
        elif flash:
            o, P = tx.attn_fwd_flash(qkv, b, na, S, da, temper, dt, dh, dw, block, masked)
        elif FUSED_ATTENTION and tx.attn_fwd_supported(S, da):
            P, o = tx.attn_fwd(q, k, v, b, na, S, da, temper, dt, dh, dw, block, masked)
        else:
            P = torch.empty(b, na, S, S, dtype=torch.float32, device=dev)
            G.gemm(q, k, P, S, S, da, ta=0, tb=0, lda=hd, ldb=hd, ldc=S, batch_outer=b, batch_inner=na,
                   sA=(S * hd, da), sB=(S * hd, da), sC=(na * S * S, S * S))
            tx.attn_softmax_fwd_(P, temper, dt, dh, dw, block, masked)
            o = torch.empty(M, hd, dtype=torch.float32, device=dev)
            G.gemm(P, v, o, S, da, S, ta=0, tb=1, lda=S, ldb=hd, ldc=hd, batch_outer=b, batch_inner=na,
                   sA=(na * S * S, S * S), sB=(S * hd, da), sC=(S * hd, da))
        y1 = torch.empty(M, d, dtype=torch.float32, device=dev)
        G.gemm(o, proj_w, y1, M, d, hd, flags=L.EPI_RESIDUAL, res=x)
        h1 = torch.empty(M, f1w.shape[0], dtype=torch.float32, device=dev)
        if p2_full:
            fn, fn_img, mean2, rstd2 = ew.layernorm_fwd_p2(y1, f0w, f0b)
            G.gemm_p2(G.P2Image(fn_img, L.amax_of(fn)), p2[1], h1, M, f1w.shape[0], d, flags=L.EPI_BIAS | L.EPI_RELU, bias=f1b)
            del fn_img
        else:
            fn, mean2, rstd2 = ew.layernorm_fwd(y1, f0w, f0b)
            G.gemm(fn, f1w, h1, M, f1w.shape[0], d, flags=L.EPI_BIAS | L.EPI_RELU, bias=f1b)
        if L.RELU_TRACE is not None:
            L.RELU_TRACE.append(h1 > 0)
        y2 = torch.empty(M, d, dtype=torch.float32, device=dev)
        G.gemm(h1, f3w, y2, M, d, f3w.shape[1], flags=L.EPI_BIAS | L.EPI_RESIDUAL, bias=f3b, res=y1)
        ctx.save_for_backward(x, mean1, rstd1, xn, qkv, P, o, y1, mean2, rstd2, fn, h1,
                              ln_w, wqkv, proj_w, f0w, f1w, f3w, dt, dh, dw)
        ctx.block, ctx.dims, ctx.masked, ctx.planes, ctx.flash = block, (M, d, S, b, na, da), bool(masked), bool(planes), bool(flash)
        return y2

    @staticmethod
    def backward(ctx, dy2):
        (x, mean1, rstd1, xn, qkv, P, o, y1, mean2, rstd2, fn, h1,
         ln_w, wqkv, proj_w, f0w, f1w, f3w, dt, dh, dw) = ctx.saved_tensors
        M, d, S, b, na, da = ctx.dims
        hd = na * da
        temper = math.sqrt(da)
        dev = x.device
        dy2 = dy2.contiguous()
        dff = f1w.shape[0]
        dh1 = torch.empty(M, dff, dtype=torch.float32, device=dev)
        G.gemm(dy2, f3w, dh1, M, dff, d, ta=0, tb=1, ldb=dff, flags=L.EPI_MASK, mask=h1)
        dfn = torch.empty(M, d, dtype=torch.float32, device=dev)
        G.gemm(dh1, f1w, dfn, M, d, dff, ta=0, tb=1, ldb=d)
        if d == dff:
            dwp, dbp = linear_wgrad_pair(dy2, h1, dh1, fn, d, dff, M)
            df3w, df3b, df1w, df1b = dwp[0], dbp[0], dwp[1], dbp[1]
        else:
            df3w, df3b = linear_wgrad(dy2, h1, d, dff, M, want_bias=True)
            df1w, df1b = linear_wgrad(dh1, fn, dff, d, M, want_bias=True)
        dy1, df0w, df0b = ew.layernorm_bwd(dfn, y1, mean2, rstd2, f0w, add=dy2)
        if ctx.planes:
            do = torch.empty(3, M, hd, dtype=torch.bfloat16, device=dev)
            G.gemm(dy1, proj_w, do, M, hd, d, ta=0, tb=1, ldb=hd, flags=L.EPI_PLANES, c_plane=M * hd)
            dproj = linear_wgrad(dy1, o, d, hd, M)
            dqkv, ddt, ddh, ddw = tx.attn_bwd_planes(qkv, do, P, o, b, na, S, da, temper, ctx.block, ctx.masked)
            return _BlockLocalAttentionFn._finish_backward(ctx, dqkv, ddt, ddh, ddw, dy1, dproj, df0w, df0b, df1w, df1b,
                                                            df3w, df3b)
        do = torch.empty(M, hd, dtype=torch.float32, device=dev)
        G.gemm(dy1, proj_w, do, M, hd, d, ta=0, tb=1, ldb=hd)
        dproj = linear_wgrad(dy1, o, d, hd, M)
        if ctx.flash:
            dqkv, ddt, ddh, ddw = tx.attn_bwd_flash(qkv, do, P, b, na, S, da, temper, dt, dh, dw, ctx.block, ctx.masked, o=o)
            return _BlockLocalAttentionFn._finish_backward(ctx, dqkv, ddt, ddh, ddw, dy1, dproj, df0w, df0b, df1w, df1b,
                                                            df3w, df3b)
        q, k, v = qkv[0], qkv[1], qkv[2]
        bh = dict(batch_outer=b, batch_inner=na)
        dqkv = torch.empty(3, M, hd, dtype=torch.float32, device=dev)
        dq, dk, dv = dqkv[0], dqkv[1], dqkv[2]
        G.gemm(P, do, dv, S, da, S, ta=1, tb=1, lda=S, ldb=hd, ldc=hd, sA=(na * S * S, S * S), sB=(S * hd, da),
               sC=(S * hd, da), flags=L.CAUSAL_KMIN if ctx.masked else 0, **bh)
        dP = torch.empty(b, na, S, S, dtype=torch.float32, device=dev)
        G.gemm(do, v, dP, S, S, da, ta=0, tb=0, lda=hd, ldb=hd, ldc=S, sA=(S * hd, da), sB=(S * hd, da),
               sC=(na * S * S, S * S), flags=L.CAUSAL_TILE if ctx.masked else 0, **bh)
        ddt, ddh, ddw = tx.attn_softmax_bwd_(P, dP, temper, ctx.block)
        G.gemm(dP, k, dq, S, da, S, ta=0, tb=1, lda=S, ldb=hd, ldc=hd, sA=(na * S * S, S * S), sB=(S * hd, da),
               sC=(S * hd, da), flags=L.CAUSAL_KMAX if ctx.masked else 0, **bh)
        G.gemm(dP, q, dk, S, da, S, ta=1, tb=1, lda=S, ldb=hd, ldc=hd, sA=(na * S * S, S * S), sB=(S * hd, da),
               sC=(S * hd, da), flags=L.CAUSAL_KMIN if ctx.masked else 0, **bh)
        del dP
        return _BlockLocalAttentionFn._finish_backward(ctx, dqkv, ddt, ddh, ddw, dy1, dproj, df0w, df0b, df1w, df1b, df3w, df3b)

    @staticmethod
    def _finish_backward(ctx, dqkv, ddt, ddh, ddw, dy1, dproj, df0w, df0b, df1w, df1b, df3w, df3b):
        x, mean1, rstd1, xn = ctx.saved_tensors[:4]
        ln_w, wqkv = ctx.saved_tensors[12], ctx.saved_tensors[13]
        M, d, S, b, na, da = ctx.dims
        hd = na * da
        dev = x.device
        dxn = torch.empty(M, d, dtype=torch.float32, device=dev)
        G.gemm(dqkv, wqkv, dxn, M, d, 3 * hd, ta=0, tb=0, lda=hd, a_kb=hd, a_skb=M * hd, ldb=da, b_kb=da, b_skb=d * da)
        dws = torch.empty(3, na, d, da, dtype=torch.float32, device=dev)
        G.gemm(xn, dqkv, dws, d, da, M, ta=1, tb=1, lda=d, ldb=hd, ldc=da, batch_outer=3, batch_inner=na,
               sB=(M * hd, da), sC=(na * d * da, d * da), splits=_splits(3 * na * -(-d // 128), M))
        dx, dlnw, dlnb = ew.layernorm_bwd(dxn, x, mean1, rstd1, ln_w, add=dy1)
        return (dx, None, None, ddt, ddh, ddw, dlnw, dlnb, dws[0], dws[1], dws[2], dproj, df0w, df0b,
                df1w, df1b, df3w, df3b, None, None)


class BlockLocalAttention(nn.Module):
    def __init__(self, block_size, da, d, n_head, masked=False):
        super().__init__()
        self.block_size = tuple(block_size)
        self.n_head, self.masked = n_head, masked
        self.mha = MultiHeadAttention(n_head, d, da)
        self.ffn = nn.Sequential(nn.LayerNorm(d), nn.Linear(d, d), nn.ReLU(True), nn.Linear(d, d))
        t, h, w = self.block_size
        self.dt_bank = nn.Parameter(torch.zeros(n_head, 2 * t - 1))
        self.dh_bank = nn.Parameter(torch.zeros(n_head, 2 * h - 1))
        self.dw_bank = nn.Parameter(torch.zeros(n_head, 2 * w - 1))
        it = torch.arange(t).view(t, 1, 1).expand(t, h, w).reshape(-1, 1)
        ih = torch.arange(h).view(1, h, 1).expand(t, h, w).reshape(-1, 1)
        iw = torch.arange(w).view(1, 1, w).expand(t, h, w).reshape(-1, 1)
        for name, ix, n in (("dt", it, t), ("dh", ih, h), ("dw", iw, w)):
            self.register_buffer(name, (ix - ix.t() + (n - 1)).reshape(-1))
        if masked:
            s = t * h * w
            self.register_buffer("mask", torch.triu(torch.ones(1, 1, s, s), diagonal=1))
        else:
            self.register_buffer("mask", None)

    def get_B(self):
        t, h, w = self.block_size
        s = t * h * w
        return (self.dt_bank.index_select(1, self.dt) + self.dh_bank.index_select(1, self.dh)
                + self.dw_bank.index_select(1, self.dw)).view(self.n_head, 1, s, s)

    def forward_tokens(self, x_tok, thw=None):
        m, f = self.mha, self.ffn
        split = thw is not None and tuple(thw) != self.block_size
        if split:
            perm, inv = _block_permutation(tuple(thw), self.block_size, x_tok.device)
            S = perm.numel()
            x_tok = _RowPermuteFn.apply(x_tok, perm, inv, S)
        y = _BlockLocalAttentionFn.apply(
            x_tok, self.block_size, self.masked, self.dt_bank, self.dh_bank, self.dw_bank,
            m.layer_norm.weight, m.layer_norm.bias, m.w_q, m.w_k, m.w_v, m.proj.weight,
            f[0].weight, f[0].bias, f[1].weight, f[1].bias, f[3].weight, f[3].bias, m.packed_qkv(), getattr(self, "_p2", None))
        if split:
            y = _RowPermuteFn.apply(y, inv, perm, S)
        return y

    def forward(self, x):
        from .. import convstack
        B, C, T, H, W = x.shape
        tok = convstack._TokensIn.apply(x)
# ... 35 lines not shown
```

Baseline: 1361.

## Emit QKV as pre-split fp16 row planes from GEMM epilogue for flash attention

Adds an EPI_ROWPLANES GEMM epilogue that writes Q/K/V as pre-split fp16 hi/lo planes plus a per-row exponent scale. New flash forward and backward kernel variants (PL template) consume these planes directly instead of loading fp32 and doing the row-scale/split in every attention tile. This removes the repeated conversion work and the fp32 reads from the attention inner loops, including the scheduling slots reserved for that conversion. In exchange the QKV GEMM epilogue does extra work, the saved tensor changes layout, and more kernel instantiations are compiled.

Result: no change. 1365, median of 6 (+0.3%).

```diff
diff --git a/include/lvt_hip.h b/include/lvt_hip.h
--- a/include/lvt_hip.h
+++ b/include/lvt_hip.h
@@ -33,6 +33,7 @@
 #define LVT_EPI_MASK       16
 #define LVT_EPI_ACCUM      32
 #define LVT_EPI_PLANES     64
+#define LVT_EPI_ROWPLANES 128
 #define LVT_CAUSAL_KMAX   (1 << 8)
 #define LVT_CAUSAL_KMIN   (1 << 9)
 #define LVT_CAUSAL_TILE   (1 << 10)
@@ -220,6 +221,15 @@
                        const float *o, int B, int H, int S, int da, float temper, const float *dt, const float *dh, const float *dw,
                        int bt, int bh, int bw, int masked, float fill, float *dq, float *dk, float *dv, float *ddt,
                        float *ddh, float *ddw, float *d_amax, void *workspace, size_t workspace_bytes, void *stream);
+int lvt_attn_fwd_flash_qkvp(const void *qp, const void *kp, const void *vp, const float *qe, const float *ke, const float *ve,
+                            long long ld, int B, int H, int S, int da, float temper, const float *dt, const float *dh,
+                            const float *dw, int bt, int bh, int bw, int masked, float fill, float *o, float *stats,
+                            float *o_amax, void *stream);
+int lvt_attn_bwd_flash_qkvp(const void *qp, const void *kp, const void *vp, const float *qe, const float *ke, const float *ve,
+                            const float *d_o, long long ld, const float *stats, const float *o, int B, int H, int S, int da,
+                            float temper, const float *dt, const float *dh, const float *dw, int bt, int bh, int bw, int masked,
+                            float fill, float *dq, float *dk, float *dv, float *ddt, float *ddh, float *ddw, float *d_amax,
+                            void *workspace, size_t workspace_bytes, void *stream);
 
 int lvt_attn_decode(const float *q, long long ldq, const float *Kc, const float *Vc, int B, int H, int S, int da, int qi,
                     float temper, const float *dt, const float *dh, const float *dw, int bt, int bh, int bw,
diff --git a/lvt_amd/csrc/attention_flash.hip b/lvt_amd/csrc/attention_flash.hip
--- a/lvt_amd/csrc/attention_flash.hip
+++ b/lvt_amd/csrc/attention_flash.hip
@@ -1,3 +1,4 @@
+#include <type_traits>
 #include "attn_common.h"
 
 namespace {
@@ -172,6 +173,73 @@
     fa_bfrags_request(row, kg, v);
     fa_bfrags_split(v, fr, inv);
 }
+struct P4 { uint4 v[4]; float e[2]; };
+__device__ __forceinline__ void fa_load_p(P4 &g, const float *__restrict__ x, const float *__restrict__ y, const float *__restrict__ ex,
+                                          const float *__restrict__ ey, long long ld, int tid) {
+    const int r = tid >> 4, c = tid & 15;
+    const uint4 *px = reinterpret_cast<const uint4 *>(x + (long long)r * ld) + c, *py = reinterpret_cast<const uint4 *>(y + (long long)r * ld) + c;
+    g.v[0] = px[0];
+    g.v[1] = px[16];
+    g.v[2] = py[0];
+    g.v[3] = py[16];
+    g.e[0] = ex[r];
+    g.e[1] = ey[r];
+}
+__device__ __forceinline__ void fa_store_p(uint4 h, uint4 l, float e, unsigned short *slot, float *rs_inv, int row, int c) {
+    unsigned short *d = slot + row * FA_LD + 8 * c;
+    *reinterpret_cast<uint4 *>(d) = h;
+    *reinterpret_cast<uint4 *>(d + FA_PL) = l;
+    rs_inv[c == 0 ? row : 64 + c] = e;
+}
+__device__ __forceinline__ void fa_park_p(const P4 &g, unsigned short *slot, float *rs_inv, int tid) {
+    const int r = tid >> 4, c = tid & 15;
+    fa_store_p(g.v[0], g.v[1], g.e[0], slot, rs_inv, r, c);
+    fa_store_p(g.v[2], g.v[3], g.e[1], slot, rs_inv, 32 + r, c);
+}
+__device__ __forceinline__ void fa_load_bfrags_p(const float *__restrict__ row, const float *__restrict__ e, int kg, f16x8 (&fr)[4][2], float &inv) {
+    const uint4 *p = reinterpret_cast<const uint4 *>(row);
+#pragma unroll
+    for (int s = 0; s < 4; ++s) {
+        fr[s][0] = __builtin_bit_cast(f16x8, p[4 * s + kg]);
+        fr[s][1] = __builtin_bit_cast(f16x8, p[16 + 4 * s + kg]);
+    }
+    inv = *e;
+}
+struct PQ { uint4 q[2]; float4 d[2]; float e; };
+__device__ __forceinline__ void fa_load_pq(PQ &g, const float *__restrict__ x, const float *__restrict__ ex, const float *__restrict__ y,
+                                           long long ld, int tid) {
+    const int r = tid >> 4, c = tid & 15;
+    const uint4 *px = reinterpret_cast<const uint4 *>(x + (long long)r * ld) + c;
+    const float *py = y + (long long)r * ld + 4 * c;
+    g.q[0] = px[0];
+    g.q[1] = px[16];
+    g.d[0] = *reinterpret_cast<const float4 *>(py);
+    g.d[1] = *reinterpret_cast<const float4 *>(py + 64);
+    g.e = ex[r];
+}
+
+template <int S_> __device__ __forceinline__ void fa_stage_piece(const G4 &g, int &eb0, int &eb1, unsigned short *slot, float *ri, int tid) {
+    if constexpr (S_ == 0) eb0 = fa_row_scale(g.v[0], g.v[1]);
+    if constexpr (S_ == 1) fa_row_store(g.v[0], g.v[1], eb0, slot, ri, tid >> 4, tid & 15);
+    if constexpr (S_ == 2) eb1 = fa_row_scale(g.v[2], g.v[3]);
+    if constexpr (S_ == 3) fa_row_store(g.v[2], g.v[3], eb1, slot, ri, 32 + (tid >> 4), tid & 15);
+}
+template <int S_> __device__ __forceinline__ void fa_stage_piece(const P4 &g, int &, int &, unsigned short *slot, float *ri, int tid) {
+    if constexpr (S_ == 1) fa_store_p(g.v[0], g.v[1], g.e[0], slot, ri, tid >> 4, tid & 15);
+    if constexpr (S_ == 3) fa_store_p(g.v[2], g.v[3], g.e[1], slot, ri, 32 + (tid >> 4), tid & 15);
+}
+template <int S_> __device__ __forceinline__ void fa_stage_piece(const PQ &g, int &, int &eb1, unsigned short *slot, float *ri, int tid) {
+    if constexpr (S_ == 1) fa_store_p(g.q[0], g.q[1], g.e, slot, ri, tid >> 4, tid & 15);
+    if constexpr (S_ == 2) eb1 = fa_row_scale(g.d[0], g.d[1]);
+    if constexpr (S_ == 3) fa_row_store(g.d[0], g.d[1], eb1, slot, ri, 32 + (tid >> 4), tid & 15);
+}
+__device__ __forceinline__ void fa_stage_all(const G4 &g, unsigned short *slot, float *ri, int tid) { fa_park(g, slot, ri, tid); }
+__device__ __forceinline__ void fa_stage_all(const P4 &g, unsigned short *slot, float *ri, int tid) { fa_park_p(g, slot, ri, tid); }
+__device__ __forceinline__ void fa_stage_all(const PQ &g, unsigned short *slot, float *ri, int tid) {
+    fa_store_p(g.q[0], g.q[1], g.e, slot, ri, tid >> 4, tid & 15);
+    fa_row_store(g.d[0], g.d[1], fa_row_scale(g.d[0], g.d[1]), slot, ri, 32 + (tid >> 4), tid & 15);
+}
+
 __device__ __forceinline__ f16x8 fa_rowfrag(const unsigned short *slot, int pl, int row, int s, int kg) {
     return *reinterpret_cast<const f16x8 *>(slot + pl * FA_PL + row * FA_LD + 32 * s + 8 * kg);
 }
@@ -227,9 +295,11 @@
     const float *dt, *dh, *dw;
     float *o, *m, *l;
     float *dq, *dk, *dv, *delta, *scal, *bank_partial;
+    const float *qe, *ke, *ve;
+    long long em;
 };
 
-template <int BT, int BH, int BW, int MASKED, int NCH>
+template <int BT, int BH, int BW, int MASKED, int NCH, int PL>
 __device__ __forceinline__ float fa_fwd_body(const FaArgs &A, FaSmem &sm, int bh_, int qhalf) {
     using GE = Geo16<BH, BW>;
     constexpr int HP = GE::HP;
@@ -243,14 +313,21 @@
     constexpr int NIT = NCH;
 
     if (tid < 2 * BH - 1) sm.dhs[tid] = A.dh[h * (2 * BH - 1) + tid] * FA_LOG2E;
-    G4 g0, g1;
+    using GT = typename std::conditional<PL != 0, P4, G4>::type;
+    const long long eo = h * A.em + row0;
+    GT g0, g1;
 #define FA_G(t) ((((t) & 1) == 0) ? g0 : g1)
-    auto load_item = [&](int t, G4 &gg) { fa_load(gg, kbase + (long long)(32 * t) * A.ld, vbase + (long long)(32 * t) * A.ld, A.ld, tid); };
+    auto load_item = [&](int t, GT &gg) {
+        if constexpr (PL) fa_load_p(gg, kbase + (long long)(32 * t) * A.ld, vbase + (long long)(32 * t) * A.ld, A.ke + eo + 32 * t, A.ve + eo + 32 * t, A.ld, tid);
+        else fa_load(gg, kbase + (long long)(32 * t) * A.ld, vbase + (long long)(32 * t) * A.ld, A.ld, tid);
+    };
+    auto park = [&](const GT &gg, unsigned short *slot, float *ri) { fa_stage_all(gg, slot, ri, tid); };
     load_item(0, g0);
     if (NIT > 1) load_item(1, g1);
     f16x8 qb[4][2];
     float qinv;
-    fa_load_bfrags(A.q + (row0 + i) * A.ld + h * AT_D, kg, qb, qinv);
+    if constexpr (PL) fa_load_bfrags_p(A.q + (row0 + i) * A.ld + h * AT_D, A.qe + eo + i, kg, qb, qinv);
+    else fa_load_bfrags(A.q + (row0 + i) * A.ld + h * AT_D, kg, qb, qinv);
     const int wi = i % BW, hi = (i / BW) % BH, ti = i / (BW * BH);
     float bt_[BT], bw_[4];
 #pragma unroll
@@ -260,7 +337,7 @@
     const float *dhl = sm.dhs + (hi + BH - 1 - (BW == 16 ? 0 : (kg >> 1)));
     constexpr int HSTEP = BW == 16 ? 1 : 2;
     const float qc = qinv * A.c1;
-    fa_park(g0, sm.ring[0], sm.rs_inv[0], tid);
+    park(g0, sm.ring[0], sm.rs_inv[0]);
     __syncthreads();
 
     f32x4v oacc[AT_D / 16];
@@ -289,7 +366,7 @@
 #pragma unroll
             for (int kt = 0; kt < 2; ++kt) st[kt] = fa_mfma(a[kt][0], qb[s][0], st[kt]);
         }
-        if constexpr (t + 1 < NIT) fa_park(FA_G(t + 1), sm.ring[(t + 1) & 1], sm.rs_inv[(t + 1) & 1], tid);
+        if constexpr (t + 1 < NIT) park(FA_G(t + 1), sm.ring[(t + 1) & 1], sm.rs_inv[(t + 1) & 1]);
         float x[8];
         f32x4v vinv[2];
 #pragma unroll
@@ -366,17 +443,17 @@
     return am;
 }
 
-template <int BT, int BH, int BW, int MASKED>
+template <int BT, int BH, int BW, int MASKED, int PL>
 __global__ __launch_bounds__(512, 1) void lvt_attn_fwd_flash_kernel(const FaArgs A, float *__restrict__ o_amax) {
     __shared__ __attribute__((aligned(16))) FaSmem sm;
     if (threadIdx.x >= 256) __builtin_amdgcn_s_setprio(1);
     float am;
     if (MASKED) {
-        am = fa_fwd_body<BT, BH, BW, MASKED, 8>(A, sm, blockIdx.x, 1);
+        am = fa_fwd_body<BT, BH, BW, MASKED, 8, PL>(A, sm, blockIdx.x, 1);
         __syncthreads();
-        am = fmaxf(am, fa_fwd_body<BT, BH, BW, MASKED, 4>(A, sm, fa_opaque(blockIdx.x), 0));
+        am = fmaxf(am, fa_fwd_body<BT, BH, BW, MASKED, 4, PL>(A, sm, fa_opaque(blockIdx.x), 0));
     } else {
-        am = fa_fwd_body<BT, BH, BW, MASKED, 8>(A, sm, fa_pair(blockIdx.x), fa_half(blockIdx.x));
+        am = fa_fwd_body<BT, BH, BW, MASKED, 8, PL>(A, sm, fa_pair(blockIdx.x), fa_half(blockIdx.x));
     }
     if (o_amax) {
         __syncthreads();
@@ -384,7 +461,7 @@
     }
 }
 
-template <int BT, int BH, int BW, int MASKED, int NCH, int ONEP>
+template <int BT, int BH, int BW, int MASKED, int NCH, int ONEP, int PL>
 __device__ __forceinline__ float fa_bwd_a_body(const FaArgs &A, FaSmemA<BT + Geo16<BH, BW>::HP + 4> &sm, int bh_, int qhalf) {
     using GE = Geo16<BH, BW>;
     using BI = BankIdx<BT, BH, BW>;
@@ -403,19 +480,23 @@
     float *mine = sm.R + (il * 4 + kg) * NR;
 #pragma unroll
     for (int x = 0; x < NR; ++x) mine[x] = 0.f;
-    G4 g0;
-    auto load_item = [&](int t, G4 &gg) {
+    using GT = typename std::conditional<PL != 0, P4, G4>::type;
+    const long long eo = h * A.em + row0;
+    GT g0;
+    auto load_item = [&](int t, GT &gg) {
         const int c = t < NCH ? t : t - NCH;
-        fa_load(gg, kbase + (long long)(32 * c) * A.ld, vbase + (long long)(32 * c) * A.ld, A.ld, tid);
+        if constexpr (PL) fa_load_p(gg, kbase + (long long)(32 * c) * A.ld, vbase + (long long)(32 * c) * A.ld, A.ke + eo + 32 * c, A.ve + eo + 32 * c, A.ld, tid);
+        else fa_load(gg, kbase + (long long)(32 * c) * A.ld, vbase + (long long)(32 * c) * A.ld, A.ld, tid);
     };
     load_item(0, g0);
     f16x8 qb[4][2], dob[4][2];
     float qinv, doinv;
-    float4 qraw[8], doraw[8], oraw[ONEP ? 8 : 1];
-    fa_bfrags_request(A.q + (row0 + i) * A.ld + h * AT_D, kg, qraw);
+    float4 qraw[PL ? 1 : 8], doraw[8], oraw[ONEP ? 8 : 1];
+    if constexpr (PL) fa_load_bfrags_p(A.q + (row0 + i) * A.ld + h * AT_D, A.qe + eo + i, kg, qb, qinv);
+    else fa_bfrags_request(A.q + (row0 + i) * A.ld + h * AT_D, kg, qraw);
     fa_bfrags_request(A.d_o + (row0 + i) * A.ld + h * AT_D, kg, doraw);
     if constexpr (ONEP) fa_bfrags_request(A.o + (row0 + i) * A.ld + h * AT_D, kg, oraw);
-    fa_bfrags_split(qraw, qb, qinv);
+    if constexpr (!PL) fa_bfrags_split(qraw, qb, qinv);
     fa_bfrags_split(doraw, dob, doinv);
     float delta_early = 0.f;
     if constexpr (ONEP) {
@@ -440,7 +521,7 @@
     const float *dhl = sm.dhs + (hi + BH - 1 - (BW == 16 ? 0 : (kg >> 1)));
     constexpr int HSTEP = BW == 16 ? 1 : 2;
     const float qc = qinv * A.c1;
-    fa_park(g0, sm.ring[0], sm.rs_inv[0], tid);
+    fa_stage_all(g0, sm.ring[0], sm.rs_inv[0], tid);
     load_item(1, g0);
     __syncthreads();
 
@@ -506,15 +587,12 @@
 #pragma unroll
             for (int kt = 0; kt < 2; ++kt) { st[kt] = fa_mfma(a[kt][0], qb[s][0], st[kt]); dp[kt] = fa_mfma(av[kt][0], dob[s][0], dp[kt]); }
             if constexpr (PARK) {
-                if constexpr (s == 0) eb0 = fa_row_scale(g0.v[0], g0.v[1]);
-                if constexpr (s == 1) fa_row_store(g0.v[0], g0.v[1], eb0, nslot, ninv, tid >> 4, tid & 15);
-                if constexpr (s == 2) eb1 = fa_row_scale(g0.v[2], g0.v[3]);
-                if constexpr (s == 3) fa_row_store(g0.v[2], g0.v[3], eb1, nslot, ninv, 32 + (tid >> 4), tid & 15);
+                fa_stage_piece<s>(g0, eb0, eb1, nslot, ninv, tid);
                 __builtin_amdgcn_sched_group_barrier(0x100, 8, 0);
 #pragma unroll
                 for (int e = 0; e < 12; ++e) {
                     __builtin_amdgcn_sched_group_barrier(0x008, 1, 0);
-                    __builtin_amdgcn_sched_group_barrier(0x002, (s & 1) ? 3 : 2, 0);
+                    if (!PL) __builtin_amdgcn_sched_group_barrier(0x002, (s & 1) ? 3 : 2, 0);
                 }
                 __builtin_amdgcn_sched_barrier(0);
             }
@@ -686,17 +764,17 @@
     return am;
 }
 
-template <int BT, int BH, int BW, int MASKED, int ONEP>
+template <int BT, int BH, int BW, int MASKED, int ONEP, int PL>
 __global__ __launch_bounds__(512, 1) void lvt_attn_bwd_flash_a_kernel(const FaArgs A, float *__restrict__ d_amax) {
     __shared__ __attribute__((aligned(16))) FaSmemA<BT + Geo16<BH, BW>::HP + 4> sm;
     if (threadIdx.x >= 256) __builtin_amdgcn_s_setprio(1);
     float am;
     if (MASKED) {
-        am = fa_bwd_a_body<BT, BH, BW, MASKED, 8, ONEP>(A, sm, blockIdx.x, 1);
+        am = fa_bwd_a_body<BT, BH, BW, MASKED, 8, ONEP, PL>(A, sm, blockIdx.x, 1);
         __syncthreads();
-        am = fmaxf(am, fa_bwd_a_body<BT, BH, BW, MASKED, 4, ONEP>(A, sm, fa_opaque(blockIdx.x), 0));
+        am = fmaxf(am, fa_bwd_a_body<BT, BH, BW, MASKED, 4, ONEP, PL>(A, sm, fa_opaque(blockIdx.x), 0));
     } else {
-        am = fa_bwd_a_body<BT, BH, BW, MASKED, 8, ONEP>(A, sm, fa_pair(blockIdx.x), fa_half(blockIdx.x));
+        am = fa_bwd_a_body<BT, BH, BW, MASKED, 8, ONEP, PL>(A, sm, fa_pair(blockIdx.x), fa_half(blockIdx.x));
     }
     if (d_amax) {
         __syncthreads();
@@ -712,7 +790,7 @@
     float dhs[32];
 };
 
-template <int BT, int BH, int BW, int MASKED, int C0, int NCH>
+template <int BT, int BH, int BW, int MASKED, int C0, int NCH, int PL>
 __device__ __forceinline__ float fa_bwd_b_body(const FaArgs &A, FaSmemB &sm, int bh_, int khalf) {
     using GE = Geo16<BH, BW>;
     constexpr int HP = GE::HP;
@@ -726,11 +804,22 @@
     constexpr int NIT = NCH;
 
     if (tid < 2 * BH - 1) sm.dhs[tid] = A.dh[h * (2 * BH - 1) + tid] * FA_LOG2E;
-    G4 g0;
-    auto load_item = [&](int t, G4 &gg) {
-        fa_load(gg, qbase + (long long)(32 * (C0 + t)) * A.ld, dobase + (long long)(32 * (C0 + t)) * A.ld, A.ld, tid);
+    using GT = typename std::conditional<PL != 0, PQ, G4>::type;
+    const long long eo = h * A.em + row0;
+    GT g0;
+    auto load_item = [&](int t, GT &gg) {
+        if constexpr (PL) fa_load_pq(gg, qbase + (long long)(32 * (C0 + t)) * A.ld, A.qe + eo + 32 * (C0 + t), dobase + (long long)(32 * (C0 + t)) * A.ld, A.ld, tid);
+        else fa_load(gg, qbase + (long long)(32 * (C0 + t)) * A.ld, dobase + (long long)(32 * (C0 + t)) * A.ld, A.ld, tid);
     };
-    {
+    if constexpr (PL) {
+        const float *rows = A.v + (row0 + khalf * 128) * A.ld + h * AT_D;
+        const float *er = A.ve + eo + khalf * 128;
+        P4 a, bq;
+        fa_load_p(a, rows, rows + 32 * A.ld, er, er + 32, A.ld, tid);
+        fa_load_p(bq, rows + 64 * A.ld, rows + 96 * A.ld, er + 64, er + 96, A.ld, tid);
+        fa_park_p(a, sm.vres[0], sm.vinv[0], tid);
+        fa_park_p(bq, sm.vres[1], sm.vinv[1], tid);
+    } else {
         const float *rows = A.v + (row0 + khalf * 128) * A.ld + h * AT_D;
         G4 a, bq;
         fa_load(a, rows, rows + 32 * A.ld, A.ld, tid);
@@ -741,7 +830,8 @@
     f16x8 kb[4][2];
     float kinv;
     load_item(0, g0);
-    fa_load_bfrags(A.k + (row0 + j) * A.ld + h * AT_D, kg, kb, kinv);
+    if constexpr (PL) fa_load_bfrags_p(A.k + (row0 + j) * A.ld + h * AT_D, A.ke + eo + j, kg, kb, kinv);
+    else fa_load_bfrags(A.k + (row0 + j) * A.ld + h * AT_D, kg, kb, kinv);
     const float *sc = A.scal + (long long)bh_ * 4;
     const float domax = fmaxf(sc[0], sc[2]), umax = fmaxf(sc[1], sc[3]);
     const float srun = 32768.f * __builtin_amdgcn_rcpf(domax);
@@ -758,7 +848,7 @@
     const float *dhl = sm.dhs + (BH - 1 - hj + (BW == 16 ? 0 : (kg >> 1)));
     constexpr int HSTEP = BW == 16 ? 1 : 2;
     const float kc = kinv * A.c1;
-    fa_park(g0, sm.ring[0], sm.rs_inv[0], tid);
+    fa_stage_all(g0, sm.ring[0], sm.rs_inv[0], tid);
     if (NIT > 1) load_item(1, g0);
     __syncthreads();
     const float vinv = sm.vinv[jl >> 6][jl & 63];
@@ -818,12 +908,7 @@
             for (int qt = 0; qt < 2; ++qt) dp[qt] = fa_mfma(ad[qt][0], vb[1], dp[qt]);
 #pragma unroll
             for (int qt = 0; qt < 2; ++qt) dp[qt] = fa_mfma(ad[qt][0], vb[0], dp[qt]);
-            if constexpr (PARK) {
-                if constexpr (s == 0) eb0 = fa_row_scale(g0.v[0], g0.v[1]);
-                if constexpr (s == 1) fa_row_store(g0.v[0], g0.v[1], eb0, nslot, ninv, tid >> 4, tid & 15);
-                if constexpr (s == 2) eb1 = fa_row_scale(g0.v[2], g0.v[3]);
-                if constexpr (s == 3) fa_row_store(g0.v[2], g0.v[3], eb1, nslot, ninv, 32 + (tid >> 4), tid & 15);
-            }
+            if constexpr (PARK) fa_stage_piece<s>(g0, eb0, eb1, nslot, ninv, tid);
             __builtin_amdgcn_sched_group_barrier(0x100, 6, 0);
 #pragma unroll
             for (int e = 0; e < 6; ++e) {
@@ -903,16 +988,16 @@
     return am;
 }
 
-template <int BT, int BH, int BW, int MASKED>
+template <int BT, int BH, int BW, int MASKED, int PL>
 __global__ __launch_bounds__(512, 1) void lvt_attn_bwd_flash_b_kernel(const FaArgs A, float *__restrict__ d_amax) {
     __shared__ __attribute__((aligned(16))) FaSmemB sm;
     if (threadIdx.x >= 256) __builtin_amdgcn_s_setprio(1);
     float am;
     if (MASKED) {
-        if (fa_half(blockIdx.x) == 0) am = fa_bwd_b_body<BT, BH, BW, MASKED, 0, 8>(A, sm, fa_pair(blockIdx.x), 0);
-        else am = fa_bwd_b_body<BT, BH, BW, MASKED, 4, 4>(A, sm, fa_pair(blockIdx.x), 1);
+        if (fa_half(blockIdx.x) == 0) am = fa_bwd_b_body<BT, BH, BW, MASKED, 0, 8, PL>(A, sm, fa_pair(blockIdx.x), 0);
+        else am = fa_bwd_b_body<BT, BH, BW, MASKED, 4, 4, PL>(A, sm, fa_pair(blockIdx.x), 1);
     } else {
-        am = fa_bwd_b_body<BT, BH, BW, MASKED, 0, 8>(A, sm, fa_pair(blockIdx.x), fa_half(blockIdx.x));
+        am = fa_bwd_b_body<BT, BH, BW, MASKED, 0, 8, PL>(A, sm, fa_pair(blockIdx.x), fa_half(blockIdx.x));
     }
     if (d_amax) {
         __syncthreads();
@@ -945,28 +1030,47 @@
 
 #define LVT_FA_GEOMS(X) X(1, 16, 16) X(4, 8, 8)
 
+static int fa_fwd_launch(FaArgs &A, long long ld, int B, int H, int S, int da, float temper, int bt, int bh, int bw, int masked,
+                         float fill, float *o, float *stats, float *o_amax, void *stream, int pl) {
+    LVT_REQUIRE(A.q && A.k && A.v && A.dt && A.dh && A.dw && o && stats && B > 0 && H > 0, "attn_fwd_flash: bad args");
+    LVT_REQUIRE((B * H) % 8 == 0, "attn_fwd_flash: B * H = %d must be a multiple of 8 (workgroup pairing per XCD)", B * H);
+    LVT_REQUIRE(lvt_attn_flash_supported(S, da, bt, bh, bw), "attn_fwd_flash: S=%d da=%d block (%d,%d,%d) has no instantiation", S, da, bt, bh, bw);
+    LVT_REQUIRE(lvt_aligned16(A.q) && lvt_aligned16(A.k) && lvt_aligned16(A.v) && lvt_aligned16(o) && lvt_aligned16(stats) && ld % 4 == 0 &&
+                ld >= (long long)H * da, "attn_fwd_flash: alignment / row stride");
+    LVT_REQUIRE(!pl || (A.qe && A.ke && A.ve), "attn_fwd_flash_qkvp: scale arrays missing");
+    A.ld = ld; A.H = H; A.inv_temper = 1.f / temper; A.c1 = FA_LOG2E / temper; A.fill2 = fill * FA_LOG2E;
+    A.o = o; A.m = stats; A.l = stats + (size_t)B * H * S; A.em = (long long)B * S;
+    const dim3 grid((unsigned)(B * H * (masked ? 1 : 2))), blk(512);
+    hipStream_t s = (hipStream_t)stream;
+#define LVT_X2(BT, BH, BW, PL)                                                                                      \
+    if (bt == BT && bh == BH && bw == BW && pl == PL) {                                                             \
+        if (masked) hipLaunchKernelGGL((lvt_attn_fwd_flash_kernel<BT, BH, BW, 1, PL>), grid, blk, 0, s, A, o_amax); \
+        else hipLaunchKernelGGL((lvt_attn_fwd_flash_kernel<BT, BH, BW, 0, PL>), grid, blk, 0, s, A, o_amax);        \
+    }
+#define LVT_X(BT, BH, BW) LVT_X2(BT, BH, BW, 0) LVT_X2(BT, BH, BW, 1)
+    LVT_FA_GEOMS(LVT_X)
+#undef LVT_X
+#undef LVT_X2
+    LVT_CHECK_LAUNCH("lvt_attn_fwd_flash_kernel");
+    return LVT_OK;
+}
+
 extern "C" int lvt_attn_fwd_flash(const float *q, const float *k, const float *v, long long ld, int B, int H, int S, int da,
                                   float temper, const float *dt, const float *dh, const float *dw, int bt, int bh, int bw,
                                   int masked, float fill, float *o, float *stats, float *o_amax, void *stream) {
-    LVT_REQUIRE(q && k && v && dt && dh && dw && o && stats && B > 0 && H > 0, "attn_fwd_flash: bad args");
-    LVT_REQUIRE((B * H) % 8 == 0, "attn_fwd_flash: B * H = %d must be a multiple of 8 (workgroup pairing per XCD)", B * H);
-    LVT_REQUIRE(lvt_attn_flash_supported(S, da, bt, bh, bw), "attn_fwd_flash: S=%d da=%d block (%d,%d,%d) has no instantiation", S, da, bt, bh, bw);
-    LVT_REQUIRE(lvt_aligned16(q) && lvt_aligned16(k) && lvt_aligned16(v) && lvt_aligned16(o) && lvt_aligned16(stats) && ld % 4 == 0 &&
-                ld >= (long long)H * da, "attn_fwd_flash: alignment / row stride");
     FaArgs A = {};
-    A.q = q; A.k = k; A.v = v; A.ld = ld; A.H = H; A.inv_temper = 1.f / temper; A.c1 = FA_LOG2E / temper; A.fill2 = fill * FA_LOG2E;
-    A.dt = dt; A.dh = dh; A.dw = dw; A.o = o; A.m = stats; A.l = stats + (size_t)B * H * S;
-    const dim3 grid((unsigned)(B * H * (masked ? 1 : 2))), blk(512);
-    hipStream_t s = (hipStream_t)stream;
-#define LVT_X(BT, BH, BW)                                                                                       \
-    if (bt == BT && bh == BH && bw == BW) {                                                                     \
-        if (masked) hipLaunchKernelGGL((lvt_attn_fwd_flash_kernel<BT, BH, BW, 1>), grid, blk, 0, s, A, o_amax); \
-        else hipLaunchKernelGGL((lvt_attn_fwd_flash_kernel<BT, BH, BW, 0>), grid, blk, 0, s, A, o_amax);        \
-    }
-    LVT_FA_GEOMS(LVT_X)
-#undef LVT_X
-    LVT_CHECK_LAUNCH("lvt_attn_fwd_flash_kernel");
-    return LVT_OK;
+    A.q = q; A.k = k; A.v = v; A.dt = dt; A.dh = dh; A.dw = dw;
+    return fa_fwd_launch(A, ld, B, H, S, da, temper, bt, bh, bw, masked, fill, o, stats, o_amax, stream, 0);
+}
+
+extern "C" int lvt_attn_fwd_flash_qkvp(const void *qp, const void *kp, const void *vp, const float *qe, const float *ke, const float *ve,
+                                       long long ld, int B, int H, int S, int da, float temper, const float *dt, const float *dh,
+                                       const float *dw, int bt, int bh, int bw, int masked, float fill, float *o, float *stats,
+                                       float *o_amax, void *stream) {
+    FaArgs A = {};
+    A.q = (const float *)qp; A.k = (const float *)kp; A.v = (const float *)vp; A.qe = qe; A.ke = ke; A.ve = ve;
+    A.dt = dt; A.dh = dh; A.dw = dw;
+    return fa_fwd_launch(A, ld, B, H, S, da, temper, bt, bh, bw, masked, fill, o, stats, o_amax, stream, 1);
 }
 
 extern "C" size_t lvt_attn_bwd_flash_workspace_bytes(int B, int H, int S, int bt, int bh, int bw) {
@@ -974,23 +1078,23 @@
     return (size_t)B * H * S * sizeof(float) + (size_t)B * H * 4 * sizeof(float) + (size_t)B * H * 2 * nb * sizeof(float);
 }
 
-extern "C" int lvt_attn_bwd_flash(const float *q, const float *k, const float *v, const float *d_o, long long ld, const float *stats,
-                                  const float *o, int B, int H, int S, int da, float temper, const float *dt, const float *dh, const float *dw,
-                                  int bt, int bh, int bw, int masked, float fill, float *dq, float *dk, float *dv, float *ddt,
-                                  float *ddh, float *ddw, float *d_amax, void *workspace, size_t workspace_bytes, void *stream) {
-    LVT_REQUIRE(q && k && v && d_o && stats && dt && dh && dw && dq && dk && dv && ddt && ddh && ddw && B > 0 && H > 0, "attn_bwd_flash: bad args");
+static int fa_bwd_launch(FaArgs &A, long long ld, const float *stats, const float *o, int B, int H, int S, int da, float temper,
+                         int bt, int bh, int bw, int masked, float fill, float *ddt, float *ddh, float *ddw, float *d_amax,
+                         void *workspace, size_t workspace_bytes, void *stream, int pl) {
+    LVT_REQUIRE(A.q && A.k && A.v && A.d_o && stats && A.dt && A.dh && A.dw && A.dq && A.dk && A.dv && ddt && ddh && ddw && B > 0 && H > 0,
+                "attn_bwd_flash: bad args");
     LVT_REQUIRE((B * H) % 8 == 0, "attn_bwd_flash: B * H = %d must be a multiple of 8 (workgroup pairing per XCD)", B * H);
     LVT_REQUIRE(lvt_attn_flash_supported(S, da, bt, bh, bw), "attn_bwd_flash: S=%d da=%d block (%d,%d,%d) has no instantiation", S, da, bt, bh, bw);
-    LVT_REQUIRE(lvt_aligned16(q) && lvt_aligned16(k) && lvt_aligned16(v) && lvt_aligned16(d_o) && lvt_aligned16(stats) && lvt_aligned16(dq) &&
-                lvt_aligned16(dk) && lvt_aligned16(dv) && ld % 4 == 0 && ld >= (long long)H * da, "attn_bwd_flash: alignment / row stride");
+    LVT_REQUIRE(lvt_aligned16(A.q) && lvt_aligned16(A.k) && lvt_aligned16(A.v) && lvt_aligned16(A.d_o) && lvt_aligned16(stats) &&
+                lvt_aligned16(A.dq) && lvt_aligned16(A.dk) && lvt_aligned16(A.dv) && ld % 4 == 0 && ld >= (long long)H * da,
+                "attn_bwd_flash: alignment / row stride");
+    LVT_REQUIRE(!pl || (A.qe && A.ke && A.ve && o), "attn_bwd_flash_qkvp: needs the scale arrays and o");
     if (!workspace || workspace_bytes < lvt_attn_bwd_flash_workspace_bytes(B, H, S, bt, bh, bw) || !lvt_aligned16(workspace)) {
         lvt_set_error("attn_bwd_flash: workspace too small or misaligned");
         return LVT_EWORKSPACE;
     }
-    FaArgs A = {};
-    A.q = q; A.k = k; A.v = v; A.d_o = d_o; A.ld = ld; A.H = H; A.inv_temper = 1.f / temper; A.c1 = FA_LOG2E / temper; A.fill2 = fill * FA_LOG2E;
-    A.dt = dt; A.dh = dh; A.dw = dw; A.m = const_cast<float *>(stats); A.l = const_cast<float *>(stats) + (size_t)B * H * S;
-    A.dq = dq; A.dk = dk; A.dv = dv;
+    A.ld = ld; A.H = H; A.inv_temper = 1.f / temper; A.c1 = FA_LOG2E / temper; A.fill2 = fill * FA_LOG2E;
+    A.m = const_cast<float *>(stats); A.l = const_cast<float *>(stats) + (size_t)B * H * S; A.em = (long long)B * S;
     LVT_REQUIRE(!o || lvt_aligned16(o), "attn_bwd_flash: o must be 16-byte aligned");
     const bool onep = o != nullptr;
     A.o = const_cast<float *>(o);
@@ -1003,24 +1107,50 @@
     hipStream_t s = (hipStream_t)stream;
 #define LVT_X(BT, BH, BW)                                                                                         \
     if (bt == BT && bh == BH && bw == BW) {                                                                       \
-        if (masked && onep) hipLaunchKernelGGL((lvt_attn_bwd_flash_a_kernel<BT, BH, BW, 1, 1>), grid, blk, 0, s, A, d_amax); \
-        else if (masked) hipLaunchKernelGGL((lvt_attn_bwd_flash_a_kernel<BT, BH, BW, 1, 0>), grid, blk, 0, s, A, d_amax);    \
-        else if (onep) hipLaunchKernelGGL((lvt_attn_bwd_flash_a_kernel<BT, BH, BW, 0, 1>), grid, blk, 0, s, A, d_amax);      \
-        else hipLaunchKernelGGL((lvt_attn_bwd_flash_a_kernel<BT, BH, BW, 0, 0>), grid, blk, 0, s, A, d_amax);                \
+        if (pl && masked) hipLaunchKernelGGL((lvt_attn_bwd_flash_a_kernel<BT, BH, BW, 1, 1, 1>), grid, blk, 0, s, A, d_amax); \
+        else if (pl) hipLaunchKernelGGL((lvt_attn_bwd_flash_a_kernel<BT, BH, BW, 0, 1, 1>), grid, blk, 0, s, A, d_amax);      \
+        else if (masked && onep) hipLaunchKernelGGL((lvt_attn_bwd_flash_a_kernel<BT, BH, BW, 1, 1, 0>), grid, blk, 0, s, A, d_amax); \
+        else if (masked) hipLaunchKernelGGL((lvt_attn_bwd_flash_a_kernel<BT, BH, BW, 1, 0, 0>), grid, blk, 0, s, A, d_amax);    \
+        else if (onep) hipLaunchKernelGGL((lvt_attn_bwd_flash_a_kernel<BT, BH, BW, 0, 1, 0>), grid, blk, 0, s, A, d_amax);      \
+        else hipLaunchKernelGGL((lvt_attn_bwd_flash_a_kernel<BT, BH, BW, 0, 0, 0>), grid, blk, 0, s, A, d_amax);                \
     }
     LVT_FA_GEOMS(LVT_X)
 #undef LVT_X
     LVT_CHECK_LAUNCH("lvt_attn_bwd_flash_a_kernel");
-#define LVT_X(BT, BH, BW)                                                                                         \
-    if (bt == BT && bh == BH && bw == BW) {                                                                       \
-        if (masked) hipLaunchKernelGGL((lvt_attn_bwd_flash_b_kernel<BT, BH, BW, 1>), gridb, blk, 0, s, A, d_amax); \
-        else hipLaunchKernelGGL((lvt_attn_bwd_flash_b_kernel<BT, BH, BW, 0>), grid, blk, 0, s, A, d_amax);        \
-    }
+#define LVT_X2(BT, BH, BW, PL)                                                                                        \
+    if (bt == BT && bh == BH && bw == BW && pl == PL) {                                                               \
+        if (masked) hipLaunchKernelGGL((lvt_attn_bwd_flash_b_kernel<BT, BH, BW, 1, PL>), gridb, blk, 0, s, A, d_amax); \
+        else hipLaunchKernelGGL((lvt_attn_bwd_flash_b_kernel<BT, BH, BW, 0, PL>), grid, blk, 0, s, A, d_amax);        \
+    }
+#define LVT_X(BT, BH, BW) LVT_X2(BT, BH, BW, 0) LVT_X2(BT, BH, BW, 1)
     LVT_FA_GEOMS(LVT_X)
 #undef LVT_X
+#undef LVT_X2
     LVT_CHECK_LAUNCH("lvt_attn_bwd_flash_b_kernel");
     hipLaunchKernelGGL(lvt_attn_flash_bank_reduce_kernel, dim3((unsigned)lvt_cdiv((long long)H * nb, 4)), dim3(256), 0, s,
                        A.bank_partial, B, H, nb, nt, nh, ddt, ddh, ddw);
     LVT_CHECK_LAUNCH("lvt_attn_flash_bank_reduce_kernel");
     return LVT_OK;
 }
+
+extern "C" int lvt_attn_bwd_flash(const float *q, const float *k, const float *v, const float *d_o, long long ld, const float *stats,
+                                  const float *o, int B, int H, int S, int da, float temper, const float *dt, const float *dh, const float *dw,
+                                  int bt, int bh, int bw, int masked, float fill, float *dq, float *dk, float *dv, float *ddt,
+                                  float *ddh, float *ddw, float *d_amax, void *workspace, size_t workspace_bytes, void *stream) {
+    FaArgs A = {};
+    A.q = q; A.k = k; A.v = v; A.d_o = d_o; A.dt = dt; A.dh = dh; A.dw = dw; A.dq = dq; A.dk = dk; A.dv = dv;
+    return fa_bwd_launch(A, ld, stats, o, B, H, S, da, temper, bt, bh, bw, masked, fill, ddt, ddh, ddw, d_amax, workspace,
+                         workspace_bytes, stream, 0);
+}
+
+extern "C" int lvt_attn_bwd_flash_qkvp(const void *qp, const void *kp, const void *vp, const float *qe, const float *ke, const float *ve,
+                                       const float *d_o, long long ld, const float *stats, const float *o, int B, int H, int S, int da,
+                                       float temper, const float *dt, const float *dh, const float *dw, int bt, int bh, int bw, int masked,
+                                       float fill, float *dq, float *dk, float *dv, float *ddt, float *ddh, float *ddw, float *d_amax,
+                                       void *workspace, size_t workspace_bytes, void *stream) {
+    FaArgs A = {};
+    A.q = (const float *)qp; A.k = (const float *)kp; A.v = (const float *)vp; A.qe = qe; A.ke = ke; A.ve = ve;
+    A.d_o = d_o; A.dt = dt; A.dh = dh; A.dw = dw; A.dq = dq; A.dk = dk; A.dv = dv;
+    return fa_bwd_launch(A, ld, stats, o, B, H, S, da, temper, bt, bh, bw, masked, fill, ddt, ddh, ddw, d_amax, workspace,
+                         workspace_bytes, stream, 1);
+}
diff --git a/lvt_amd/csrc/epilogue_fast.h b/lvt_amd/csrc/epilogue_fast.h
--- a/lvt_amd/csrc/epilogue_fast.h
+++ b/lvt_amd/csrc/epilogue_fast.h
@@ -131,3 +131,79 @@
         if (bits > seen) atomicMax(reinterpret_cast<unsigned *>(dst), bits);
     }
 }
+
+#define LVT_RP_EMIN 30
+#define LVT_RP_EMAX 254
+template <int CTRL> __device__ __forceinline__ float lvt_rp_dpp_max(float v) {
+    const int o = __builtin_amdgcn_update_dpp(0, __builtin_bit_cast(int, v), CTRL, 0xf, 0xf, false);
+    return fmaxf(v, __builtin_bit_cast(float, o));
+}
+__device__ __forceinline__ float lvt_rp_row16_max(float v) {
+    v = lvt_rp_dpp_max<0xB1>(v);
+    v = lvt_rp_dpp_max<0x4E>(v);
+    v = lvt_rp_dpp_max<0x141>(v);
+    v = lvt_rp_dpp_max<0x140>(v);
+    return v;
+}
+__device__ __forceinline__ unsigned lvt_rp_split_pair(float a, float b, float s, unsigned &pl) {
+    typedef _Float16 h2 __attribute__((ext_vector_type(2)));
+    typedef float f2 __attribute__((ext_vector_type(2)));
+    const f2 t = f2{a, b} * s;
+    const unsigned ph = __builtin_bit_cast(unsigned, __builtin_convertvector(t, h2));
+    float r0, r1;
+    asm("v_fma_mix_f32 %0, %1, %2, %3 op_sel:[0,0,0] op_sel_hi:[1,0,0]" : "=v"(r0) : "v"(ph), "v"(-1.f), "v"(t.x));
+    asm("v_fma_mix_f32 %0, %1, %2, %3 op_sel:[1,0,0] op_sel_hi:[1,0,0]" : "=v"(r1) : "v"(ph), "v"(-1.f), "v"(t.y));
+    pl = __builtin_bit_cast(unsigned, __builtin_convertvector(f2{r0, r1}, h2));
+    return ph;
+}
+template <int TM, int TN>
+__device__ __forceinline__ void lvt_epi_rowplanes_wave(const LvtEpi &e, lvt_f32x16 (&acc)[TM][TN], float *wave_tile, float *xch,
+                                                       float *expo, int m_w, int n_t, int wm, int wn, int lane) {
+    static_assert(TM == 2 && TN == 2, "64 x 64 sub-tiles");
+    constexpr int SW = TN * 32;
+    const int l31 = lane & 31, half = lane >> 5;
+    const int c4 = lane & 15, r0 = lane >> 4;
+    float4 v[TM][8];
+    float mx[TM][8];
+#pragma unroll
+    for (int i = 0; i < TM; ++i) {
+#pragma unroll
+        for (int j = 0; j < TN; ++j)
+#pragma unroll
+            for (int r = 0; r < 16; ++r) wave_tile[((r & 3) + 8 * (r >> 2) + 4 * half) * SW + 32 * j + l31] = acc[i][j][r];
+#pragma unroll
+        for (int u = 0; u < 8; ++u) {
+            float4 w = *reinterpret_cast<const float4 *>(&wave_tile[(r0 + 4 * u) * SW + 4 * c4]);
+            w.x *= e.alpha; w.y *= e.alpha; w.z *= e.alpha; w.w *= e.alpha;
+            v[i][u] = w;
+            mx[i][u] = lvt_rp_row16_max(fmaxf(fmaxf(lvt_absf(w.x), lvt_absf(w.y)), fmaxf(lvt_absf(w.z), lvt_absf(w.w))));
+        }
+    }
+    if (c4 == 0) {
+#pragma unroll
+        for (int i = 0; i < TM; ++i)
+#pragma unroll
+            for (int u = 0; u < 8; ++u) xch[wn * 256 + wm * 64 + i * 32 + r0 + 4 * u] = mx[i][u];
+    }
+    __syncthreads();
+#pragma unroll
+    for (int i = 0; i < TM; ++i) {
+#pragma unroll
+        for (int u = 0; u < 8; ++u) {
+            const int rl = i * 32 + r0 + 4 * u, row = m_w + rl;
+            const float m = fmaxf(mx[i][u], xch[(wn ^ 1) * 256 + wm * 64 + rl]);
+            int eb = (int)((__float_as_uint(m) >> 23) & 0xffu);
+            eb = eb < LVT_RP_EMIN ? LVT_RP_EMIN : (eb > LVT_RP_EMAX ? LVT_RP_EMAX : eb);
+            const float s = __uint_as_float((unsigned)(268 - eb) << 23);
+            uint2 hi, lo;
+            hi.x = lvt_rp_split_pair(v[i][u].x, v[i][u].y, s, lo.x);
+            hi.y = lvt_rp_split_pair(v[i][u].z, v[i][u].w, s, lo.y);
+            if (row < e.M) {
+                unsigned short *cp = reinterpret_cast<unsigned short *>(e.C + e.coff + (long long)row * e.ldc + n_t) + 64 * wn + 4 * c4;
+                *reinterpret_cast<uint2 *>(cp) = hi;
+                *reinterpret_cast<uint2 *>(cp + 128) = lo;
+                if (wn == 0 && c4 == 0) expo[row] = __uint_as_float((unsigned)(eb - 14) << 23);
+            }
+        }
+    }
+}
diff --git a/lvt_amd/csrc/gemm_engine.hip b/lvt_amd/csrc/gemm_engine.hip
--- a/lvt_amd/csrc/gemm_engine.hip
+++ b/lvt_amd/csrc/gemm_engine.hip
@@ -1484,6 +1484,14 @@
         }
         __syncthreads();
     }
+    if (p.flags & LVT_EPI_ROWPLANES) {
+        static_assert(LDS_FLOATS >= TURN_FLOATS + 512, "row-max exchange beside the turn-tables");
+        LvtEpi e;
+        e.M = p.M; e.N = p.N; e.C = p.C; e.ldc = p.ldc; e.coff = tc.coff; e.alpha = p.alpha; e.flags = p.flags;
+        float *expo = p.C + p.c_plane + ((long long)tc.z * (p.N / BN) + n0 / BN) * p.M;
+        lvt_epi_rowplanes_wave<TM, TN>(e, acc, lds + wave * (32 * TN * 32), lds + TURN_FLOATS, expo, m0 + wm * (TM * 32), n0, wm, wn, lane);
+        return;
+    }
     if (p.vec_epi && !(p.flags & (LVT_EPI_PLANES | LVT_EPI_ACCUM | LVT_EPI_TANH))) {
         LvtEpi e;
         e.M = p.M; e.N = p.N;
@@ -1800,6 +1808,11 @@
         LVT_REQUIRE(d->splits <= 1 && !(d->flags & LVT_EPI_ACCUM) && d->N % 4 == 0 && d->ldc % 4 == 0 && d->c_plane % 4 == 0 &&
                     d->sC_o % 4 == 0 && d->sC_i % 4 == 0 && lvt_aligned16(d->C) && !(d->flags & LVT_MATH_F32),
                     "gemm: PLANES needs the bf16x3 arithmetic, no split-K / ACCUM, N, ldc, c_plane, sC %% 4 == 0 and an aligned C");
+    if (d->flags & LVT_EPI_ROWPLANES)
+        LVT_REQUIRE(d->splits <= 1 && (d->flags & ~(LVT_EPI_ROWPLANES | LVT_MATH_F16X2)) == 0 && d->N % 128 == 0 && d->ldc % 4 == 0 &&
+                    d->sC_o % 4 == 0 && d->sC_i % 4 == 0 && lvt_aligned16(d->C) && !d->c_amax && d->c_plane > 0,
+                    "gemm: ROWPLANES needs the f16x2 arithmetic and no other epilogue flag, no split-K / c_amax, N %% 128 == 0, "
+                    "ldc, sC %% 4 == 0, an aligned C and the scale array at c_plane > 0");
     hipStream_t s = (hipStream_t)stream;
     KParams p; kparams_from_desc(d, p);
     const int zc = gemm_batch(d);
@@ -1829,6 +1842,7 @@
     const bool wide = math_of(d->flags) == 2 && d->M > 128 && d->K % BK == 0 && p.a_kb % BK == 0 &&
                       p.b_kb % BK == 0 && a_span < (1LL << 30) && b_span < (1LL << 30) &&
                       !(d->flags & (LVT_CAUSAL_KMAX | LVT_CAUSAL_KMIN | LVT_CAUSAL_TILE));
+    LVT_REQUIRE(wide || !(d->flags & LVT_EPI_ROWPLANES), "gemm: ROWPLANES is a form of the wide kernel (M > 128, K %% 32 == 0, no causal flag)");
     if (wide && d->ta == 0 && d->tb == 0) rc = launch_wide<0, 0>(p, zc, s);
     else if (wide && d->ta == 0 && d->tb == 1) rc = launch_wide<0, 1>(p, zc, s);
     else if (wide) rc = launch_wide<1, 1>(p, zc, s);
diff --git a/lvt_amd/csrc/lvt_core.hip b/lvt_amd/csrc/lvt_core.hip
--- a/lvt_amd/csrc/lvt_core.hip
+++ b/lvt_amd/csrc/lvt_core.hip
@@ -11,7 +11,7 @@
 }
 
 extern "C" const char *lvt_last_error(void) { return g_err; }
-extern "C" int lvt_version(void) { return 620; }
+extern "C" int lvt_version(void) { return 630; }
 
 extern "C" int lvt_device_info(char *name, int name_len, int *cus, int *clock_khz, long long *hbm_bytes) {
     int n = 0;
diff --git a/lvt_amd/hip/binding.py b/lvt_amd/hip/binding.py
--- a/lvt_amd/hip/binding.py
+++ b/lvt_amd/hip/binding.py
@@ -6,9 +6,9 @@
 _HERE = os.path.dirname(os.path.abspath(__file__))
 _LIB_PATH = os.environ.get("LVT_HIP_LIB") or os.path.join(os.path.dirname(_HERE), "liblvt_hip.so")
 
-EPI_BIAS, EPI_RESIDUAL, EPI_RELU, EPI_TANH, EPI_MASK, EPI_ACCUM, EPI_PLANES = 1, 2, 4, 8, 16, 32, 64
+EPI_BIAS, EPI_RESIDUAL, EPI_RELU, EPI_TANH, EPI_MASK, EPI_ACCUM, EPI_PLANES, EPI_ROWPLANES = 1, 2, 4, 8, 16, 32, 64, 128
 CAUSAL_KMAX, CAUSAL_KMIN, CAUSAL_TILE = 1 << 8, 1 << 9, 1 << 10
-ABI_VERSION = 620
+ABI_VERSION = 630
 MATH_F32 = 1 << 16
 MATH_F16X2 = 1 << 18
 ONEHOT_DENSE = 1 << 19
@@ -167,6 +167,10 @@
         "lvt_attn_bwd_flash_workspace_bytes": (sz, [ci, ci, ci, ci, ci, ci]),
         "lvt_attn_bwd_flash": (ci, [vp, vp, vp, vp, cll, vp, vp, ci, ci, ci, ci, cf, vp, vp, vp, ci, ci, ci, ci, cf, vp, vp, vp, vp,
                                     vp, vp, vp, vp, sz, vp]),
+        "lvt_attn_fwd_flash_qkvp": (ci, [vp, vp, vp, vp, vp, vp, cll, ci, ci, ci, ci, cf, vp, vp, vp, ci, ci, ci, ci, cf, vp, vp,
+                                         vp, vp]),
+        "lvt_attn_bwd_flash_qkvp": (ci, [vp, vp, vp, vp, vp, vp, vp, cll, vp, vp, ci, ci, ci, ci, cf, vp, vp, vp, ci, ci, ci, ci,
+                                         cf, vp, vp, vp, vp, vp, vp, vp, vp, sz, vp]),
         "lvt_attn_decode": (ci, [vp, cll, vp, vp, ci, ci, ci, ci, ci, cf, vp, vp, vp, ci, ci, ci, vp, vp, cll, vp]),
         "lvt_decode_gather_codes": (ci, [vp, vp, vp, ci, ci, ci, vp, vp]),
         "lvt_decode_commit": (ci, [vp, ci, ci, vp, vp, vp]),
diff --git a/lvt_amd/hip/gemm.py b/lvt_amd/hip/gemm.py
--- a/lvt_amd/hip/gemm.py
+++ b/lvt_amd/hip/gemm.py
@@ -32,7 +32,7 @@
         d.a_amax, d.b_amax = L.amax_of(A).data_ptr(), L.amax_of(B).data_ptr()
         d.a_amax2 = L.amax_of(a_also).data_ptr() if a_also is not None else None
         d.b_amax2 = L.amax_of(b_also).data_ptr() if b_also is not None else None
-        if splits <= 1 and C_out.dtype == torch.float32:
+        if splits <= 1 and C_out.dtype == torch.float32 and not flags & L.EPI_ROWPLANES:
             d.c_amax = L.new_amax(C_out).data_ptr()
     lib = L.lib()
     ws, nws = None, 0
diff --git a/lvt_amd/hip/tx.py b/lvt_amd/hip/tx.py
--- a/lvt_amd/hip/tx.py
+++ b/lvt_amd/hip/tx.py
@@ -94,6 +94,49 @@
     if t0 is not None:
         L.TIMER.end("attn_fwd", 4.0 * B * H * S * S * da, t0)
     return o, stats
+
+
+def qkv_rowplanes(M, H, da, device):
+    hd = H * da
+    buf = torch.empty(3 * M * hd + 3 * H * M, dtype=torch.float32, device=device)
+    return buf, buf[:3 * M * hd].view(3, M, hd), buf[3 * M * hd:].view(3, H, M), 3 * M * hd
+
+
+def attn_fwd_flash_qkvp(qkvp, qkve, B, H, S, da, temper, dt, dh, dw, block, masked, fill=-1e4):
+    L.require(qkvp, qkve, dt, dh, dw)
+    M, hd = B * S, H * da
+    o = torch.empty(M, hd, dtype=torch.float32, device=qkvp.device)
+    stats = torch.empty(2, B * H * S, dtype=torch.float32, device=qkvp.device)
+    t0 = L.TIMER.begin() if L.TIMER is not None else None
+    L.check(L.lib().lvt_attn_fwd_flash_qkvp(L.ptr(qkvp[0]), L.ptr(qkvp[1]), L.ptr(qkvp[2]), L.ptr(qkve[0]), L.ptr(qkve[1]),
+                                            L.ptr(qkve[2]), hd, B, H, S, da, temper, L.ptr(dt), L.ptr(dh), L.ptr(dw), block[0],
+                                            block[1], block[2], 1 if masked else 0, fill, L.ptr(o), L.ptr(stats), L.out_amax(o),
+                                            L.stream_ptr()), "lvt_attn_fwd_flash_qkvp")
+    if t0 is not None:
+        L.TIMER.end("attn_fwd", 4.0 * B * H * S * S * da, t0)
+    return o, stats
+
+
+def attn_bwd_flash_qkvp(qkvp, qkve, do, stats, o, B, H, S, da, temper, dt, dh, dw, block, masked, fill=-1e4):
+    L.require(qkvp, qkve, do, stats, dt, dh, dw, o)
+    M, hd = B * S, H * da
+    dev = qkvp.device
+    dqkv = torch.empty(3, M, hd, dtype=torch.float32, device=dev)
+    ddt = torch.empty(H, 2 * block[0] - 1, dtype=torch.float32, device=dev)
+    ddh = torch.empty(H, 2 * block[1] - 1, dtype=torch.float32, device=dev)
+    ddw = torch.empty(H, 2 * block[2] - 1, dtype=torch.float32, device=dev)
+    lib = L.lib()
+    nws = lib.lvt_attn_bwd_flash_workspace_bytes(B, H, S, block[0], block[1], block[2])
+    ws = L.workspace(nws, dev, "attn_bwd")
+    t0 = L.TIMER.begin() if L.TIMER is not None else None
+    L.check(lib.lvt_attn_bwd_flash_qkvp(L.ptr(qkvp[0]), L.ptr(qkvp[1]), L.ptr(qkvp[2]), L.ptr(qkve[0]), L.ptr(qkve[1]),
+                                        L.ptr(qkve[2]), L.ptr(do), hd, L.ptr(stats), L.ptr(o), B, H, S, da, temper, L.ptr(dt),
+                                        L.ptr(dh), L.ptr(dw), block[0], block[1], block[2], 1 if masked else 0, fill,
+                                        L.ptr(dqkv[0]), L.ptr(dqkv[1]), L.ptr(dqkv[2]), L.ptr(ddt), L.ptr(ddh), L.ptr(ddw),
+                                        L.out_amax(dqkv), L.ptr(ws), nws, L.stream_ptr()), "lvt_attn_bwd_flash_qkvp")
+    if t0 is not None:
+        L.TIMER.end("attn_bwd", 8.0 * B * H * S * S * da, t0)
+    return dqkv, ddt, ddh, ddw
 
 
 def attn_bwd_flash(qkv, do, stats, B, H, S, da, temper, dt, dh, dw, block, masked, fill=-1e4, o=None):
diff --git a/lvt_amd/modeling/autoregressive/vt_attention.py b/lvt_amd/modeling/autoregressive/vt_attention.py
--- a/lvt_amd/modeling/autoregressive/vt_attention.py
+++ b/lvt_amd/modeling/autoregressive/vt_attention.py
@@ -198,18 +198,26 @@
                    sB=(na * d * da, d * da), sC=(3 * M * hd, da), flags=L.EPI_PLANES, c_plane=M * hd)
             P, o = tx.attn_fwd_planes(qkv, b, na, S, da, temper, dt, dh, dw, block, masked)
         else:
-            qkv = torch.empty(3, M, hd, dtype=torch.float32, device=dev)
+            qkv = torch.empty(3, M, hd, dtype=torch.float32, device=dev) if (p2 is not None or not flash) else None
             if p2 is not None:
                 G.gemm_p2(G.P2Image(xn_img, L.amax_of(xn)) if p2_full else xn, p2[0], qkv, M, hd, d, lda=d, ldb=d, ldc=hd,
                           batch_outer=3, batch_inner=1, sB=(hd * d, 0), sC=(M * hd, 0))
                 if p2_full:
                     del xn_img
+            elif flash:
+                qkv_buf, qkv, qkve, c_plane = tx.qkv_rowplanes(M, na, da, dev)
+                G.gemm(xn, wqkv, qkv_buf, M, da, d, ta=0, tb=1, lda=d, ldb=da, ldc=hd, batch_outer=3, batch_inner=na,
+                       sB=(na * d * da, d * da), sC=(M * hd, da), flags=L.EPI_ROWPLANES, c_plane=c_plane)
             else:
                 G.gemm(xn, wqkv, qkv, M, da, d, ta=0, tb=1, lda=d, ldb=da, ldc=hd, batch_outer=3, batch_inner=na,
                        sB=(na * d * da, d * da), sC=(M * hd, da))
             q, k, v = qkv[0], qkv[1], qkv[2]
+        rowplanes = flash and p2 is None
         if planes:
             pass
+        elif rowplanes:
+            o, P = tx.attn_fwd_flash_qkvp(qkv, qkve, b, na, S, da, temper, dt, dh, dw, block, masked)
+            qkv = qkv_buf
         elif flash:
             o, P = tx.attn_fwd_flash(qkv, b, na, S, da, temper, dt, dh, dw, block, masked)
         elif FUSED_ATTENTION and tx.attn_fwd_supported(S, da):
@@ -239,6 +247,7 @@
         ctx.save_for_backward(x, mean1, rstd1, xn, qkv, P, o, y1, mean2, rstd2, fn, h1,
                               ln_w, wqkv, proj_w, f0w, f1w, f3w, dt, dh, dw)
         ctx.block, ctx.dims, ctx.masked, ctx.planes, ctx.flash = block, (M, d, S, b, na, da), bool(masked), bool(planes), bool(flash)
+        ctx.rowplanes = bool(rowplanes)
         return y2
 
     @staticmethod
@@ -273,7 +282,12 @@
         G.gemm(dy1, proj_w, do, M, hd, d, ta=0, tb=1, ldb=hd)
         dproj = linear_wgrad(dy1, o, d, hd, M)
         if ctx.flash:
-            dqkv, ddt, ddh, ddw = tx.attn_bwd_flash(qkv, do, P, b, na, S, da, temper, dt, dh, dw, ctx.block, ctx.masked, o=o)
+            if ctx.rowplanes:
+                qkvp, qkve = qkv[:3 * M * hd].view(3, M, hd), qkv[3 * M * hd:].view(3, na, M)
+                dqkv, ddt, ddh, ddw = tx.attn_bwd_flash_qkvp(qkvp, qkve, do, P, o, b, na, S, da, temper, dt, dh, dw, ctx.block,
+                                                             ctx.masked)
+            else:
+                dqkv, ddt, ddh, ddw = tx.attn_bwd_flash(qkv, do, P, b, na, S, da, temper, dt, dh, dw, ctx.block, ctx.masked, o=o)
             return _BlockLocalAttentionFn._finish_backward(ctx, dqkv, ddt, ddh, ddw, dy1, dproj, df0w, df0b, df1w, df1b,
                                                             df3w, df3b)
         q, k, v = qkv[0], qkv[1], qkv[2]
```
